# Tencent/FeatherCNN

Hardware: AMD Instinct MI355X
Metric: images/sec fp32 forward @224x224 (higher is better)
Workload: dtype f32; 1 GPU; vgg16 whole net (40 layers in the model file, 20 after fusion level 3), batch 32 per GPU, 224x224x3, fp32, synthetic ...; net=vgg16, mode=net, per_gpu_batch=32, global_batch=32, parallelism=batch-shard x1, launch=hipGraph replay per step, conv_routing=fhip_conv_select_algo_tuned

## Files before the change

__graft_entry__.py:

```python
from __future__ import annotations

import os
import subprocess
import sys

ROOT = os.path.dirname(os.path.abspath(__file__))
if ROOT not in sys.path:
    sys.path.insert(0, ROOT)


def build() -> None:
    jobs = str(min(8, os.cpu_count() or 1))
    subprocess.run(["make", "-s", "-j", jobs, "-C", os.path.join(ROOT, "feathercnn_amd", "csrc")], check=True)
    subprocess.run(["make", "-s", "-C", os.path.join(ROOT, "oracle"), "port"], check=True)
    subprocess.run(["make", "-s", "-C", os.path.join(ROOT, "oracle"), "ref"], check=True)
    import feathercnn_amd
    feathercnn_amd.load_library()
    from feathercnn_amd import _lib
    _lib.load_gconv_library()
    _lib.load_deconv_library()
    _lib.load_inorm_library()
    _lib.load_shuffle_library()
    from feathercnn_amd import provenance
    provenance.write_stamp()


def smoke() -> None:
    import numpy as np
    import torch

    import oracle
    from feathercnn_amd import ConvLayer, ConvParam
    from oracle import conv_geom, nerr, synth

    if not torch.cuda.is_available():
        raise RuntimeError("smoke() needs a GPU")
    if not os.path.exists(os.path.join(ROOT, "feathercnn_amd", "libfeather_hip.so")):
        build()
    dev = torch.device("cuda:0")
    chk = oracle.best()
    cases = [("winograd_f63", conv_geom(16, 32, 20, 3, 1, 1)), ("im2col_1x1", conv_geom(32, 24, 14, 1, 1, 0)),
             ("im2col_7x7s2", conv_geom(3, 16, 32, 7, 2, 3)), ("depthwise_s1", conv_geom(16, 16, 28, 3, 1, 1, group=16)),
             ("depthwise_s2", conv_geom(16, 16, 28, 3, 2, 1, group=16)), ("depthwise_flat_14px", conv_geom(24, 24, 14, 3, 1, 1, group=24)),
             ("depthwise_flat_7px", conv_geom(40, 40, 7, 3, 1, 1, group=40)), ("depthwise_band_56px", conv_geom(8, 8, 56, 3, 1, 1, group=8)),
             ("depthwise_flat_20px_s2", conv_geom(12, 12, 20, 3, 2, 1, group=12)), ("depthwise_flat_5px", conv_geom(44, 44, 5, 3, 1, 1, group=44))]
    for name, g in cases:
        x, w, b = synth(g, 2)
        p = ConvParam(output_channels=g.oc, input_channels=g.ic, input_h=g.ih, input_w=g.iw, kernel_h=g.kh, kernel_w=g.kw,
                      stride_h=g.sh, stride_w=g.sw, pad_left=g.pl, pad_right=g.pr, pad_top=g.pt, pad_bottom=g.pb,
                      group=g.group, bias_term=True, activation=1, batch=2)
        layer = ConvLayer(p, torch.from_numpy(w).to(dev), torch.from_numpy(b).to(dev))
        y = layer.Forward(torch.from_numpy(x).to(dev))
        torch.cuda.synchronize()
        e = nerr(y.cpu().numpy(), chk.forward(g, x, w, b))
        print(f"smoke {name}: algo={layer.booster.algo} normalised error vs {type(chk).__name__} = {e:.2e}")
        if not (e <= 1e-4) or not np.isfinite(e):
            raise AssertionError(f"smoke {name}: parity failed ({e})")
    from feathercnn_amd.booster import WINOGRADF63, forward_chained
    g1, g2 = conv_geom(16, 24, 28, 3, 1, 1), conv_geom(24, 8, 28, 3, 1, 1)
    (x, w1, b1), (_, w2, b2) = synth(g1, 2, seed=3), synth(g2, 2, seed=4)
    run = []
    for g, w, b in ((g1, w1, b1), (g2, w2, b2)):
        p = ConvParam(output_channels=g.oc, input_channels=g.ic, input_h=g.ih, input_w=g.iw, kernel_h=3, kernel_w=3, stride_h=1, stride_w=1,
                      pad_left=1, pad_right=1, pad_top=1, pad_bottom=1, group=1, bias_term=True, activation=1, batch=2)
        run.append(ConvLayer(p, torch.from_numpy(w).to(dev), torch.from_numpy(b).to(dev), algo=WINOGRADF63))
    y = forward_chained(run, torch.from_numpy(x).to(dev))
    torch.cuda.synchronize()
    e = nerr(y.cpu().numpy(), chk.forward(g2, chk.forward(g1, x, w1, b1), w2, b2))
    print(f"smoke chained winograd pair: normalised error = {e:.2e}")
    if not (e <= 1e-4):
        raise AssertionError(f"smoke chained pair: parity failed ({e})")
    g0, g1 = conv_geom(3, 16, 28, 3, 1, 1), conv_geom(16, 8, 28, 3, 1, 1)
    (x, w0, b0), (_, w1, b1) = synth(g0, 2, seed=6), synth(g1, 2, seed=7)
    p0 = ConvParam(output_channels=16, input_channels=3, input_h=28, input_w=28, kernel_h=3, kernel_w=3, stride_h=1, stride_w=1, pad_left=1,
                   pad_right=1, pad_top=1, pad_bottom=1, group=1, bias_term=True, activation=1, batch=2)
    p0.AssignOutputDim()
    p1 = ConvParam(output_channels=8, input_channels=16, input_h=28, input_w=28, kernel_h=3, kernel_w=3, stride_h=1, stride_w=1, pad_left=1,
                   pad_right=1, pad_top=1, pad_bottom=1, group=1, bias_term=True, activation=1, batch=2)
    l1 = ConvLayer(p1, torch.from_numpy(w1).to(dev), torch.from_numpy(b1).to(dev), algo=WINOGRADF63)
    y = forward_chained([l1], torch.from_numpy(x).to(dev), first=(p0, torch.from_numpy(w0).to(dev), torch.from_numpy(b0).to(dev)))
    torch.cuda.synchronize()
    e = nerr(y.cpu().numpy(), chk.forward(g1, chk.forward(g0, x, w0, b0), w1, b1))
    print(f"smoke first layer inside the Winograd input transform: normalised error = {e:.2e}")
    if not (e <= 1e-4):
        raise AssertionError(f"smoke first-layer fusion: parity failed ({e})")
    from feathercnn_amd import model_zoo
    from feathercnn_amd.net import Net
    from oracle import netcheck
    p, b, i, o = model_zoo.tiny_allsorts()
    x = np.random.default_rng(5).uniform(-1, 1, (2, 3, 20, 20)).astype(np.float32)
    want = (netcheck.RefNet(p, b) if netcheck.have_ref_net() else netcheck.PortNet(p, b)).run(i, x, o)
    for level in (1, 3):
        net = Net(fusion=level, tuned=(level == 3), graph=(level == 3))
        net.LoadParam(p)
        net.LoadWeights(b)
        net.FeedInput(i, x)
        net.Forward()
        e = nerr(net.Extract(o), want)
        print(f"smoke tiny net, fusion level {level} ({len(net.layers())} layers after fusion): normalised error = {e:.2e}")
        if not (e <= 1e-4):
            raise AssertionError(f"smoke net: parity failed ({e})")
    sys.path.insert(0, os.path.join(ROOT, "tests"))
    import gconv_ref
    p, b, i, o = model_zoo.tiny_grouped()
    x = np.random.default_rng(6).uniform(-1, 1, (2, 3, 21, 21)).astype(np.float32)
    net = Net(fusion=2)
    net.LoadParam(p)
    net.LoadWeights(b)
    net.FeedInput(i, x)
    net.Forward()
    e = gconv_ref.nerr(net.Extract(o), gconv_ref.Net(p, b).run(i, x, o))
    print(f"smoke grouped net ({sum(a == 'GCONV' for _, _, a in net.layers())} grouped layers): normalised error = {e:.2e}")
    if not (e <= 1e-4):
        raise AssertionError(f"smoke grouped net: parity failed ({e})")
    import deconv_ref
    p, b, i, o = model_zoo.tiny_deconv()
    x = np.random.default_rng(7).uniform(-1, 1, (2, 3, 16, 16)).astype(np.float32)
    net = Net(fusion=2)
    net.LoadParam(p)
    net.LoadWeights(b)
    net.FeedInput(i, x)
    net.Forward()
    e = deconv_ref.nerr(net.Extract(o), deconv_ref.Net(p, b).run(i, x, o))
    print(f"smoke tiny_deconv ({sum(a == 'DECONV' for _, _, a in net.layers())} deconvolution layers): normalised error = {e:.2e}")
    if not (e <= 1e-4):
        raise AssertionError(f"smoke tiny_deconv: parity failed ({e})")
    import inorm_ref
    p, b, i, o = model_zoo.tiny_generative()
    x = np.random.default_rng(8).uniform(-1, 1, (2, 3, 24, 24)).astype(np.float32)
    net = Net(fusion=2)
    net.LoadParam(p)
    net.LoadWeights(b)
    net.FeedInput(i, x)
    net.Forward()
    e = inorm_ref.nerr(net.Extract(o), inorm_ref.Net(p, b).run(i, x, o))
    print(f"smoke tiny_generative ({sum(a == 'INORM' for _, _, a in net.layers())} InstanceNorm layers): normalised error = {e:.2e}")
    if not (e <= 1e-4):
        raise AssertionError(f"smoke tiny_generative: parity failed ({e})")
    import shuffle_ref
    p, b, i, o = model_zoo.tiny_shuffle()
    x = np.random.default_rng(9).uniform(-1, 1, (2, 3, 28, 28)).astype(np.float32)
    net = Net(fusion=2)
    net.LoadParam(p)
    net.LoadWeights(b)
    net.FeedInput(i, x)
    net.Forward()
    e = shuffle_ref.nerr(net.Extract(o), shuffle_ref.Net(p, b).run(i, x, o))
    print(f"smoke tiny_shuffle ({sum(a == 'SHUFFLE' for _, _, a in net.layers())} channel-map launches): normalised error = {e:.2e}")
    if not (e <= 1e-4):
        raise AssertionError(f"smoke tiny_shuffle: parity failed ({e})")
    print("smoke OK")


if __name__ == "__main__":
    build()
    if len(sys.argv) > 1 and sys.argv[1] == "smoke":
        smoke()
```

feathercnn_amd/_lib.py:

```python
from __future__ import annotations

import ctypes
import os

_HERE = os.path.dirname(os.path.abspath(__file__))
_LIB = None
_PIXOUT = None
_GCONV = None
_DECONV = None
_INORM = None
_SHUFFLE = None

STAGE_NAMES = ("wino_input", "wino_gemm", "wino_output", "igemm", "depthwise", "init", "wino_chain")


class fhip_conv_param(ctypes.Structure):
    _fields_ = [(n, ctypes.c_int) for n in (
        "output_channels", "input_channels", "input_h", "input_w", "kernel_h", "kernel_w", "output_h", "output_w",
        "stride_h", "stride_w", "pad_left", "pad_bottom", "pad_right", "pad_top", "group", "bias_term", "activation")]


class fhip_winograd_plan(ctypes.Structure):
    _fields_ = [("tiles_x", ctypes.c_int), ("tiles_y", ctypes.c_int), ("tiles_per_image", ctypes.c_int),
                ("columns", ctypes.c_int), ("columns_padded", ctypes.c_int), ("column_block", ctypes.c_int), ("frequency_points", ctypes.c_int), ("tile_outputs", ctypes.c_int),
                ("in_channels_padded", ctypes.c_int),
                ("out_channels_padded", ctypes.c_int), ("v_offset_bytes", ctypes.c_size_t), ("v_bytes", ctypes.c_size_t),
                ("m_offset_bytes", ctypes.c_size_t), ("m_bytes", ctypes.c_size_t), ("u_bytes", ctypes.c_size_t)]


class fhip_pool_param(ctypes.Structure):
    _fields_ = [(n, ctypes.c_int) for n in (
        "channels", "input_h", "input_w", "kernel_h", "kernel_w", "stride_h", "stride_w", "pad_left", "pad_right",
        "pad_top", "pad_bottom", "pooling_type", "global_pooling")]


class fhip_pixel_image(ctypes.Structure):
    _fields_ = [("data", ctypes.c_void_p)] + [(n, ctypes.c_int) for n in ("w", "h", "stride", "roi_x", "roi_y", "roi_w", "roi_h")]


_P = ctypes.POINTER(fhip_conv_param)
_Q = ctypes.POINTER(fhip_pool_param)
_PI = ctypes.POINTER(ctypes.c_int)
_SZ = ctypes.c_size_t
_V = ctypes.c_void_p
_I = ctypes.c_int

SIGNATURES = {
    "fhip_conv_assign_output_dim": (_I, [_P]),
    "fhip_conv_flops": (ctypes.c_double, [_P]),
    "fhip_conv_select_algo": (_I, [_P, ctypes.POINTER(_I)]),
    "fhip_conv_select_algo_tuned": (_I, [_P, ctypes.POINTER(_I)]),
    "fhip_conv_get_buffer_size": (_I, [_P, _I, _I, ctypes.POINTER(ctypes.c_size_t), ctypes.POINTER(ctypes.c_size_t)]),
    "fhip_conv_init": (_I, [_P, _I, _V, _V, _V]),
    "fhip_conv_forward": (_I, [_P, _I, _I, _V, _V, _V, _V, _V, _V]),
    "fhip_winograd_f63_plan": (_I, [_P, _I, ctypes.POINTER(fhip_winograd_plan)]),
    "fhip_winograd_f63_transform_kernel": (_I, [_P, _V, _V, _V]),
    "fhip_winograd_f63_input_transform": (_I, [_P, _I, _V, _V, _V]),
    "fhip_winograd_f63_tile_gemm": (_I, [_P, _I, _V, _V, _V, _V]),
    "fhip_winograd_f63_output_transform": (_I, [_P, _I, _V, _V, _V, _V]),
    "fhip_stage_timing_enable": (_I, [_I]),
    "fhip_stage_timing_collect": (_I, [ctypes.POINTER(ctypes.c_double), ctypes.POINTER(ctypes.c_longlong)]),
    "fhip_last_error": (ctypes.c_char_p, []),
    "fhip_version": (ctypes.c_char_p, []),
    "fhip_device_info": (_I, [ctypes.c_char_p, _I, ctypes.POINTER(_I), ctypes.POINTER(_I)]),
    "fhip_conv_streams_1x1": (_I, [_P, _I, _I]),
    "fhip_calibrate_mfma_f32": (_I, [ctypes.POINTER(ctypes.c_double), ctypes.POINTER(ctypes.c_double), _V]),
    "fhip_relu": (_I, [_V, _V, _SZ, _V]),
    "fhip_add": (_I, [_V, _V, _V, _SZ, _I, _V]),
    "fhip_affine": (_I, [_V, _V, _V, _V, _I, _I, _I, _I, _V]),
    "fhip_conv_can_fuse_residual": (_I, [_P, _I]),
    "fhip_conv_forward_residual": (_I, [_P, _I, _I, _V, _V, _V, _V, _V, _V, _V]),
    "fhip_conv_can_fuse_dw_pw": (_I, [_P, _P, _I]),
    "fhip_conv_forward_dw_pw": (_I, [_P, _P, _I, _V, _V, _V, _V, _V, _V, _V]),
    "fhip_conv_can_chain_winograd": (_I, [_P, _I, _P, _I, _I]),
    "fhip_conv_forward_chained": (_I, [_P, _I, _V, _V, _V, _V, _V, _V, _P, _V, _I, _V]),
    "fhip_winograd_f63_output_to_next_input": (_I, [_P, _P, _I, _V, _V, _V, _I, _V]),
    "fhip_conv_can_fuse_siblings": (_I, [_P, _I, _P, _I, _I]),
    "fhip_conv_siblings_geometry": (_I, [_P, _P, _P]),
    "fhip_conv_forward_siblings": (_I, [_P, _P, _I, _V, _V, _V, _V, _V, _V]),
    "fhip_conv_can_fuse_first_winograd": (_I, [_P, _P, _I, _I]),
    "fhip_winograd_f63_input_from_first": (_I, [_P, _P, _I, _V, _V, _V, _V, _V]),
    "fhip_conv_can_fuse_maxpool2": (_I, [_P, _I]),
    "fhip_conv_forward_maxpool2": (_I, [_P, _I, _I, _V, _V, _V, _V, _V, _V]),
    "fhip_pixels_to_float": (_I, [_V, _V, _I, _I, _I, _I, _I, _I, _V, _V, _V]),
    "fhip_yuv420sp_to_float": (_I, [_V, _V, _I, _I, _I, _I, _I, _I, _I, _V, _V, _V]),
    "fhip_pixel_images_plan": (_I, [_V, _I, _I, _I, _I, _V, ctypes.POINTER(_SZ)]),
    "fhip_pixels_to_float_images": (_I, [_V, _V, _V, _V, _V, _V]),
    "fhip_pooling_output_dim": (_I, [_Q, _PI, _PI]),
    "fhip_pooling": (_I, [_Q, _I, _V, _V, _V]),
    "fhip_softmax": (_I, [_V, _V, _I, _I, _V]),
    "fhip_net_create": (_I, [ctypes.POINTER(_V)]),
    "fhip_net_destroy": (_I, [_V]),
    "fhip_net_set_stream": (_I, [_V, _V]),
    "fhip_net_get_stream": (_I, [_V, ctypes.POINTER(_V)]),
    "fhip_net_set_fusion": (_I, [_V, _I]),
    "fhip_net_set_graph": (_I, [_V, _I]),
    "fhip_net_set_tuned_selection": (_I, [_V, _I]),
    "fhip_net_set_concurrency": (_I, [_V, _I]),
    "fhip_net_set_sub_batches": (_I, [_V, _I]),
    "fhip_net_load_param": (_I, [_V, ctypes.c_char_p]),
    "fhip_net_load_param_mem": (_I, [_V, ctypes.c_char_p, _SZ]),
    "fhip_net_load_weights": (_I, [_V, ctypes.c_char_p]),
    "fhip_net_load_weights_mem": (_I, [_V, _V, _SZ]),
    "fhip_net_load_weights_device": (_I, [_V, _V, _SZ]),
    "fhip_net_feed_input": (_I, [_V, ctypes.c_char_p, _I, _I, _I, _I, _V, _I]),
    "fhip_net_feed_pixels": (_I, [_V, ctypes.c_char_p, _I, _V, _I, _I, _I, _I, _I, _V, _V, _I]),
    "fhip_net_feed_yuv420sp": (_I, [_V, ctypes.c_char_p, _I, _V, _I, _I, _I, _I, _I, _I, _V, _V, _I]),
    "fhip_net_feed_pixel_images": (_I, [_V, ctypes.c_char_p, _I, _V, _I, _I, _I, _V, _V, _I]),
    "fhip_net_forward": (_I, [_V]),
    "fhip_net_extract": (_I, [_V, ctypes.c_char_p, ctypes.POINTER(_V), _PI, _PI, _PI, _PI]),
    "fhip_net_extract_host": (_I, [_V, ctypes.c_char_p, _V, _SZ]),
    "fhip_net_layer_count": (_I, [_V]),
    "fhip_net_layer_info": (_I, [_V, _I, ctypes.c_char_p, ctypes.c_char_p, _I, _PI]),
    "fhip_net_layer_conv_param": (_I, [_V, _I, _P, _PI]),
    "fhip_net_layer_fused_pointwise": (_I, [_V, _I, _P, _PI]),
    "fhip_net_layer_chain": (_I, [_V, _I, _PI, _PI]),
    "fhip_net_layer_sibling": (_I, [_V, _I, _PI]),
    "fhip_net_layer_residual": (_I, [_V, _I, _PI]),
    "fhip_net_forward_timed": (_I, [_V, ctypes.POINTER(ctypes.c_float)]),
    "fhip_net_memory": (_I, [_V, ctypes.POINTER(_SZ), ctypes.POINTER(_SZ), ctypes.POINTER(_SZ)]),
}

PIXOUT_SIGNATURES = {
    "fhip_pixout_channels": (_I, [_I]),
    "fhip_float_to_pixels": (_I, [_V, _SZ, _V, _I, _I, _I, _I, _I, _I, _V, _V, _V]),
    "fhip_float_to_pixels_host": (_I, [_V, _SZ, _V, _I, _I, _I, _I, _I, _I, _V, _V, _V]),
    "fhip_pixout_last_error": (ctypes.c_char_p, []),
}

GCONV_SIGNATURES = {
    "fhip_gconv_supported": (_I, [_P]),
    "fhip_gconv_get_buffer_size": (_I, [_P, _I, ctypes.POINTER(_SZ), ctypes.POINTER(_SZ)]),
    "fhip_gconv_init": (_I, [_P, _V, _V, _V]),
    "fhip_gconv_forward": (_I, [_P, _I, _V, _V, _V, _V, _V, _V]),
    "fhip_gconv_route": (_I, [_P, _V, _V, ctypes.c_char_p, _I]),
    "fhip_gconv_last_error": (ctypes.c_char_p, []),
}

class fhip_deconv_param(ctypes.Structure):
    _fields_ = [(n, ctypes.c_int) for n in ("output_channels", "input_channels", "input_h", "input_w", "kernel_h", "kernel_w", "output_h", "output_w",
                                            "stride_h", "stride_w", "pad_left", "pad_bottom", "pad_right", "pad_top", "group", "bias_term",
                                            "activation", "output_pad_right", "output_pad_bottom")]


_DP = ctypes.POINTER(fhip_deconv_param)
DECONV_SIGNATURES = {
    "fhip_deconv_assign_output_dim": (_I, [_DP]),
    "fhip_deconv_supported": (_I, [_DP]),
    "fhip_deconv_get_buffer_size": (_I, [_DP, _I, ctypes.POINTER(_SZ), ctypes.POINTER(_SZ)]),
    "fhip_deconv_init": (_I, [_DP, _V, _V, _V]),
    "fhip_deconv_forward": (_I, [_DP, _I, _V, _V, _V, _V, _V, _V]),
    "fhip_deconv_route": (_I, [_DP, ctypes.c_char_p, _I]),
    "fhip_deconv_last_error": (ctypes.c_char_p, []),
}

_FL = ctypes.c_float
INORM_SIGNATURES = {
    "fhip_instance_norm_get_buffer_size": (_I, [_I, _I, _I, _I, ctypes.POINTER(_SZ)]),
    "fhip_instance_norm_forward": (_I, [_I, _I, _I, _I, _V, _V, _V, _V, _FL, _I, _FL, _V, _V]),
    "fhip_instance_norm_forward_route": (_I, [_I, _I, _I, _I, _I, _V, _V, _V, _V, _FL, _I, _FL, _V, _V]),
    "fhip_instance_norm_route": (_I, [_I, _I, _I, _I, _V, _V, ctypes.c_char_p, _I]),
    "fhip_activation_forward": (_I, [_I, _V, _V, _I, _I, _I, _FL, _FL, _V, _V]),
    "fhip_inorm_last_error": (ctypes.c_char_p, []),
}

_PP = ctypes.POINTER(ctypes.c_void_p)
_IP = ctypes.POINTER(ctypes.c_int)
SHUFFLE_SIGNATURES = {
    "fhip_channel_map_supported": (_I, [_I, _I, _I, _I]),
    "fhip_channel_slice_resolve": (_I, [_I, _IP, _I, _IP]),
    "fhip_channel_shuffle_forward": (_I, [_V, _V, _I, _I, _I, _I, _I, _I, _V]),
    "fhip_channel_slice_forward": (_I, [_PP, _V, _I, _I, _I, _I, _IP, _I, _V]),
    "fhip_channel_map_create": (_I, [_PP, _IP, _I, _IP, _I, _IP]),
    "fhip_channel_map_destroy": (_I, [_V]),
    "fhip_channel_map_forward": (_I, [_V, _PP, _PP, _I, _I, _I, _V]),
    "fhip_channel_map_forward_route": (_I, [_I, _V, _PP, _PP, _I, _I, _I, _V]),
    "fhip_channel_map_route": (_I, [_I, _I, _I, _PP, _I, ctypes.c_char_p, _I]),
    "fhip_shuffle_last_error": (ctypes.c_char_p, []),
}


def lib_path() -> str:
    return os.environ.get("FEATHER_HIP_LIB", os.path.join(_HERE, "libfeather_hip.so"))


def load_library():
    global _LIB
    if _LIB is None:
        import torch
        path = lib_path()
        if not os.path.exists(path):
            raise RuntimeError(f"feathercnn_amd: HIP library {path} is missing -- run `python -c 'import __graft_entry__ as g; "
                               "g.build()'` (or `make -C feathercnn_amd/csrc`). There is no CPU fallback.")
        lib = ctypes.CDLL(path)
        for name, (res, args) in SIGNATURES.items():
            fn = getattr(lib, name)
            fn.restype = res
            fn.argtypes = args
        _LIB = lib
    return _LIB


def pixout_path() -> str:
    return os.path.join(_HERE, "libfeather_pixout.so")


def load_pixout_library():
    global _PIXOUT
    if _PIXOUT is None:
        import torch
        path = pixout_path()
        if not os.path.exists(path):
            raise RuntimeError(f"feathercnn_amd: HIP library {path} is missing -- run `python -c 'import __graft_entry__ as g; "
                               "g.build()'` (or `make -C feathercnn_amd/csrc`). There is no CPU fallback.")
        lib = ctypes.CDLL(path)
        for name, (res, args) in PIXOUT_SIGNATURES.items():
            fn = getattr(lib, name)
            fn.restype = res
            fn.argtypes = args
        _PIXOUT = lib
    return _PIXOUT


def gconv_path() -> str:
    return os.path.join(_HERE, "libfeather_gconv.so")


def load_gconv_library():
    global _GCONV
    if _GCONV is None:
        import torch
        path = gconv_path()
        if not os.path.exists(path):
            raise RuntimeError(f"feathercnn_amd: HIP library {path} is missing -- run `python -c 'import __graft_entry__ as g; "
                               "g.build()'` (or `make -C feathercnn_amd/csrc`). There is no CPU fallback.")
        lib = ctypes.CDLL(path)
        for name, (res, args) in GCONV_SIGNATURES.items():
            fn = getattr(lib, name)
            fn.restype = res
            fn.argtypes = args
        _GCONV = lib
    return _GCONV


def deconv_path() -> str:
    return os.path.join(_HERE, "libfeather_deconv.so")


def load_deconv_library():
    global _DECONV
    if _DECONV is None:
        import torch
        path = deconv_path()
        if not os.path.exists(path):
            raise RuntimeError(f"feathercnn_amd: HIP library {path} is missing -- run `python -c 'import __graft_entry__ as g; "
                               "g.build()'` (or `make -C feathercnn_amd/csrc`). There is no CPU fallback.")
        lib = ctypes.CDLL(path)
        for name, (res, args) in DECONV_SIGNATURES.items():
            fn = getattr(lib, name)
            fn.restype = res
            fn.argtypes = args
        _DECONV = lib
    return _DECONV


def inorm_path() -> str:
    return os.path.join(_HERE, "libfeather_inorm.so")


def load_inorm_library():
    global _INORM
    if _INORM is None:
        import torch
        path = inorm_path()
        if not os.path.exists(path):
            raise RuntimeError(f"feathercnn_amd: HIP library {path} is missing -- run `python -c 'import __graft_entry__ as g; "
                               "g.build()'` (or `make -C feathercnn_amd/csrc`). There is no CPU fallback.")
        lib = ctypes.CDLL(path)
        for name, (res, args) in INORM_SIGNATURES.items():
            fn = getattr(lib, name)
            fn.restype = res
            fn.argtypes = args
        _INORM = lib
    return _INORM


def shuffle_path() -> str:
    return os.path.join(_HERE, "libfeather_shuffle.so")


def load_shuffle_library():
    global _SHUFFLE
    if _SHUFFLE is None:
        import torch
        path = shuffle_path()
        if not os.path.exists(path):
            raise RuntimeError(f"feathercnn_amd: HIP library {path} is missing -- run `python -c 'import __graft_entry__ as g; "
                               "g.build()'` (or `make -C feathercnn_amd/csrc`). There is no CPU fallback.")
        lib = ctypes.CDLL(path)
        for name, (res, args) in SHUFFLE_SIGNATURES.items():
            fn = getattr(lib, name)
            fn.restype = res
            fn.argtypes = args
        _SHUFFLE = lib
    return _SHUFFLE
```

feathercnn_amd/csrc/capi.hip:

```cpp
#include <string.h>
#include <stdlib.h>

#include <algorithm>
#include <mutex>
#include <string>
#include <vector>

#include "common.h"
#include "feather_hip/feather_net.h"

namespace fhip
{
int winograd_plan(const fhip_conv_param& p, int batch, fhip_winograd_plan* plan);
int winograd_transform_kernel(const fhip_conv_param& p, float* u, const float* kernel, hipStream_t s);
int winograd_input_transform(const fhip_conv_param& p, int batch, float* v, const float* input, hipStream_t s);
int winograd_tile_gemm(const fhip_conv_param& p, int batch, float* m, const float* u, const float* v, hipStream_t s);
int winograd_output_transform(const fhip_conv_param& p, int batch, float* output, const float* m, const float* bias,
                              hipStream_t s, int pool = 0);
bool winograd_can_pool(const fhip_conv_param& p);
bool winograd_can_chain(const fhip_conv_param& p, const fhip_conv_param& next, int pool);
bool winograd_can_fuse_first(const fhip_conv_param& first, const fhip_conv_param& next, int batch);
fhip_conv_param igemm_twin_geometry(const fhip_conv_param& a, const fhip_conv_param& b);
bool igemm_twin_applicable(const fhip_conv_param& a, const fhip_conv_param& b, int batch);
int igemm_twin_forward(const fhip_conv_param& a, const fhip_conv_param& b, int batch, float* out_a, float* out_b, const float* in, const float* packed,
// ... 168 lines not shown
{
    if (!valid_param(p) || !buffer_bytes || !packed_bytes || batch < 1) return fail(FHIP_E_BADARG, "bad argument");
    switch (algo)
    {
        case FHIP_NAIVE:
        case FHIP_IM2COL:
        {
            if (p->group > 1) return fail(FHIP_E_UNSUPPORTED, "implicit GEMM handles group == 1 only");
            *buffer_bytes = igemm_buffer_bytes(*p, batch);
            *packed_bytes = igemm_packed_floats(*p) * sizeof(float);
            return FHIP_OK;
        }
        case FHIP_DEPTHWISE:
            *buffer_bytes = 0;
            *packed_bytes = depthwise_packed_floats(*p, nullptr) * sizeof(float);
            return FHIP_OK;
        case FHIP_WINOGRADF63:
        {
            fhip_winograd_plan pl;
            int rc = winograd_plan(*p, batch, &pl);
            if (rc) return rc;
            *buffer_bytes = pl.v_bytes + pl.m_bytes;
            *packed_bytes = pl.u_bytes;
            return FHIP_OK;
        }
        default: return fail(FHIP_E_UNSUPPORTED, "This algo is not supported on gfx950 (nor on AVX2, avx/booster.cpp:348-354)");
    }
}

int fhip_conv_init(const fhip_conv_param* p, int algo, float* packed, const float* kernel, void* stream)
{
    if (!valid_param(p) || !packed || !kernel) return fail(FHIP_E_BADARG, "bad argument");
    hipStream_t s = (hipStream_t)stream;
    switch (algo)
    {
        case FHIP_NAIVE:
        case FHIP_IM2COL: return igemm_init(*p, packed, kernel, s);
        case FHIP_DEPTHWISE: return depthwise_init(*p, packed, kernel, s);
        case FHIP_WINOGRADF63: return winograd_transform_kernel(*p, packed, kernel, s);
        default: return fail(FHIP_E_UNSUPPORTED, "This algo is not supported on gfx950");
    }
}

static int conv_forward_impl(const fhip_conv_param* p, int algo, int batch, float* output, const float* input, const float* packed,
                             float* buffer, const float* bias, void* stream, int pool, const float* residual = nullptr)
{
    if (!valid_param(p) || !output || !input || !packed || batch < 1) return fail(FHIP_E_BADARG, "bad argument");
    hipStream_t s = (hipStream_t)stream;
    if (pool && (algo != FHIP_WINOGRADF63 || !winograd_can_pool(*p)))
        return fail(FHIP_E_UNSUPPORTED, "fused max pooling is available on the Winograd route with even output dims only");
    if (residual && algo != FHIP_IM2COL) return fail(FHIP_E_UNSUPPORTED, "the fused residual add is available on the IM2COL route only");
    switch (algo)
    {
        case FHIP_NAIVE: return igemm_forward(*p, batch, output, input, packed, bias, buffer, true, s);
        case FHIP_IM2COL: return igemm_forward(*p, batch, output, input, packed, bias, buffer, false, s, residual);
        case FHIP_DEPTHWISE: return depthwise_forward(*p, batch, output, input, packed, bias, s);
        case FHIP_WINOGRADF63:
        {
            if (!buffer) return fail(FHIP_E_BADARG, "Winograd needs the scratch buffer");
            fhip_winograd_plan pl;
            int rc = winograd_plan(*p, batch, &pl);
            if (rc) return rc;
            float* v = reinterpret_cast<float*>(reinterpret_cast<char*>(buffer) + pl.v_offset_bytes);
            float* m = reinterpret_cast<float*>(reinterpret_cast<char*>(buffer) + pl.m_offset_bytes);
            if ((rc = winograd_input_transform(*p, batch, v, input, s))) return rc;
            if ((rc = winograd_tile_gemm(*p, batch, m, packed, v, s))) return rc;
            return winograd_output_transform(*p, batch, output, m, bias, s, pool);
        }
        default: return fail(FHIP_E_UNSUPPORTED, "This algo is not supported on gfx950");
    }
}

int fhip_conv_forward(const fhip_conv_param* p, int algo, int batch, float* output, const float* input, const float* packed,
                      float* buffer, const float* bias, void* stream)
{
    return conv_forward_impl(p, algo, batch, output, input, packed, buffer, bias, stream, 0);
}

int fhip_conv_forward_maxpool2(const fhip_conv_param* p, int algo, int batch, float* pooled_output, const float* input, const float* packed,
                               float* buffer, const float* bias, void* stream)
{
    return conv_forward_impl(p, algo, batch, pooled_output, input, packed, buffer, bias, stream, 1);
}

int fhip_conv_forward_residual(const fhip_conv_param* p, int algo, int batch, float* output, const float* input, const float* packed,
                               float* buffer, const float* bias, const float* residual, void* stream)
{
    if (!residual) return fail(FHIP_E_BADARG, "null residual");
    return conv_forward_impl(p, algo, batch, output, input, packed, buffer, bias, stream, 0, residual);
}

int fhip_conv_streams_1x1(const fhip_conv_param* p, int algo, int batch)
{
    return valid_param(p) && (algo == FHIP_IM2COL || algo == FHIP_NAIVE) && batch >= 1 && igemm_streams(*p, batch) ? 1 : 0;
}

int fhip_conv_can_fuse_residual(const fhip_conv_param* p, int algo) { return valid_param(p) && algo == FHIP_IM2COL ? 1 : 0; }

int fhip_conv_can_fuse_maxpool2(const fhip_conv_param* p, int algo)
{
    return valid_param(p) && algo == FHIP_WINOGRADF63 && winograd_can_pool(*p) ? 1 : 0;
}

int fhip_conv_can_fuse_dw_pw(const fhip_conv_param* dw, const fhip_conv_param* pw, int batch)
{
    return valid_param(dw) && valid_param(pw) && dwpw_applicable(*dw, *pw, batch) ? 1 : 0;
}

int fhip_conv_forward_dw_pw(const fhip_conv_param* dw, const fhip_conv_param* pw, int batch, float* output, const float* input,
                            const float* dw_packed, const float* dw_bias, const float* pw_packed, const float* pw_bias, void* stream)
{
    if (!valid_param(dw) || !valid_param(pw) || !output || !input || !dw_packed || !pw_packed || batch < 1) return fail(FHIP_E_BADARG, "bad argument");
    return dwpw_forward(*dw, *pw, batch, output, input, dw_packed, dw_bias, pw_packed, pw_bias, (hipStream_t)stream);
}

int fhip_conv_can_fuse_siblings(const fhip_conv_param* a, int algo_a, const fhip_conv_param* b, int algo_b, int batch)
{
    return valid_param(a) && valid_param(b) && algo_a == FHIP_IM2COL && algo_b == FHIP_IM2COL && igemm_twin_applicable(*a, *b, batch) ? 1 : 0;
}

int fhip_conv_siblings_geometry(const fhip_conv_param* a, const fhip_conv_param* b, fhip_conv_param* both)
{
    if (!valid_param(a) || !valid_param(b) || !both) return fail(FHIP_E_BADARG, "bad argument");
    *both = igemm_twin_geometry(*a, *b);
    return FHIP_OK;
}

int fhip_conv_forward_siblings(const fhip_conv_param* a, const fhip_conv_param* b, int batch, float* output_a, float* output_b, const float* input,
                               const float* packed_both, const float* bias_both, void* stream)
{
    if (!valid_param(a) || !valid_param(b) || !output_a || !output_b || !input || !packed_both || batch < 1) return fail(FHIP_E_BADARG, "bad argument");
    return igemm_twin_forward(*a, *b, batch, output_a, output_b, input, packed_both, bias_both, (hipStream_t)stream);
}

int fhip_conv_can_chain_winograd(const fhip_conv_param* p, int algo, const fhip_conv_param* next, int next_algo, int pool)
{
    return valid_param(p) && valid_param(next) && algo == FHIP_WINOGRADF63 && next_algo == FHIP_WINOGRADF63 && winograd_can_chain(*p, *next, pool) ? 1 : 0;
}

int fhip_conv_forward_chained(const fhip_conv_param* p, int batch, float* output, const float* input, const float* packed, float* v, float* m,
                              const float* bias, const fhip_conv_param* next, float* v_next, int pool, void* stream)
{
    if (!valid_param(p) || !packed || !v || !m || batch < 1) return fail(FHIP_E_BADARG, "bad argument");
    if (next ? (!valid_param(next) || !v_next) : !output) return fail(FHIP_E_BADARG, "a chained layer needs `next` and `v_next`, the last one `output`");
    hipStream_t s = (hipStream_t)stream;
    int rc;
    if (input && (rc = winograd_input_transform(*p, batch, v, input, s))) return rc;
    if ((rc = winograd_tile_gemm(*p, batch, m, packed, v, s))) return rc;
    if (next) return winograd_output_to_next_input(*p, *next, batch, v_next, m, bias, s, pool);
    if (pool && !winograd_can_pool(*p)) return fail(FHIP_E_UNSUPPORTED, "fused max pooling needs even output dims");
    return winograd_output_transform(*p, batch, output, m, bias, s, pool);
}

int fhip_winograd_f63_output_to_next_input(const fhip_conv_param* p, const fhip_conv_param* next, int batch, float* v_next, const float* m,
                                           const float* bias, int pool, void* stream)
{
    if (!valid_param(p) || !valid_param(next) || !v_next || !m || batch < 1) return fail(FHIP_E_BADARG, "bad argument");
    return winograd_output_to_next_input(*p, *next, batch, v_next, m, bias, (hipStream_t)stream, pool);
}

int fhip_conv_can_fuse_first_winograd(const fhip_conv_param* first, const fhip_conv_param* next, int next_algo, int batch)
{
    return valid_param(first) && valid_param(next) && next_algo == FHIP_WINOGRADF63 && winograd_can_fuse_first(*first, *next, batch) ? 1 : 0;
}

int fhip_winograd_f63_input_from_first(const fhip_conv_param* first, const fhip_conv_param* next, int batch, float* v_next, const float* input,
                                       const float* first_kernel, const float* first_bias, void* stream)
{
    if (!valid_param(first) || !valid_param(next) || !v_next || !input || !first_kernel || batch < 1) return fail(FHIP_E_BADARG, "bad argument");
    return winograd_input_from_first(*first, *next, batch, v_next, input, first_kernel, first_bias, (hipStream_t)stream);
}

int fhip_winograd_f63_transform_kernel(const fhip_conv_param* p, float* u, const float* kernel, void* stream)
{
    if (!valid_param(p) || !u || !kernel) return fail(FHIP_E_BADARG, "bad argument");
    return winograd_transform_kernel(*p, u, kernel, (hipStream_t)stream);
}

int fhip_winograd_f63_input_transform(const fhip_conv_param* p, int batch, float* v, const float* input, void* stream)
{
    if (!valid_param(p) || !v || !input) return fail(FHIP_E_BADARG, "bad argument");
    return winograd_input_transform(*p, batch, v, input, (hipStream_t)stream);
}

int fhip_winograd_f63_tile_gemm(const fhip_conv_param* p, int batch, float* m, const float* u, const float* v, void* stream)
{
    if (!valid_param(p) || !m || !u || !v) return fail(FHIP_E_BADARG, "bad argument");
    return winograd_tile_gemm(*p, batch, m, u, v, (hipStream_t)stream);
}

int fhip_winograd_f63_output_transform(const fhip_conv_param* p, int batch, float* output, const float* m, const float* bias,
                                       void* stream)
{
    if (!valid_param(p) || !output || !m) return fail(FHIP_E_BADARG, "bad argument");
    return winograd_output_transform(*p, batch, output, m, bias, (hipStream_t)stream);
}

int fhip_stage_timing_enable(int on)
{
    std::lock_guard<std::mutex> lk(g_tm_mu);
    g_tm_on = on != 0;
    return FHIP_OK;
}

int fhip_stage_timing_collect(double* ms, long long* launches)
{
    if (!ms || !launches) return fail(FHIP_E_BADARG, "null argument");
    std::lock_guard<std::mutex> lk(g_tm_mu);
    for (int i = 0; i < FHIP_STAGE_COUNT; ++i)
    {
        ms[i] = 0.0;
        launches[i] = 0;
    }
    int rc = FHIP_OK;
    for (auto& t : g_tm_pending)
    {
        float dt = 0.f;
        hipError_t e = hipEventSynchronize(t.b);
        if (e == hipSuccess) e = hipEventElapsedTime(&dt, t.a, t.b);
        if (e != hipSuccess)
            rc = fail_hip(e, "stage timing");
        else if (t.stage >= 0 && t.stage < FHIP_STAGE_COUNT)
        {
            ms[t.stage] += dt;
            launches[t.stage] += 1;
        }
        g_tm_pool.emplace_back(t.a, t.b);
    }
    g_tm_pending.clear();
    return rc;
}

const char* fhip_last_error(void) { return g_last_error.c_str(); }

const char* fhip_version(void) { return "feather_hip 0.1 (gfx950)"; }

int fhip_device_info(char* name, int name_len, int* cus, int* lds_bytes)
{
    int n = 0;
    if (hipGetDeviceCount(&n) != hipSuccess || n < 1) return fail(FHIP_E_NODEVICE, "no HIP device");
    int dev = 0;
    FHIP_CHECK_HIP(hipGetDevice(&dev));
    hipDeviceProp_t prop;
    FHIP_CHECK_HIP(hipGetDeviceProperties(&prop, dev));
    if (name && name_len > 0)
    {
        snprintf(name, name_len, "%s (%s)", prop.name, prop.gcnArchName);
    }
    if (cus) *cus = prop.multiProcessorCount;
    if (lds_bytes) *lds_bytes = (int)prop.maxSharedMemoryPerMultiProcessor;
    return FHIP_OK;
}

namespace
{
typedef float cal_f32x16 __attribute__((ext_vector_type(16)));
__device__ unsigned long long g_cal_ticks[2];

__global__ __launch_bounds__(256) void mfma_calibration_kernel(float* sink, const float* noise, int steps)
{
    const long long c0 = clock64(), w0 = wall_clock64();
    cal_f32x16 acc[4];
#pragma unroll
    for (int t = 0; t < 4; ++t)
#pragma unroll
        for (int r = 0; r < 16; ++r) acc[t][r] = 0.f;
    float a[8], b[8];
#pragma unroll
    for (int u = 0; u < 8; ++u)
    {
        a[u] = noise[(threadIdx.x * 16 + u + blockIdx.x) & 4095];
        b[u] = noise[(threadIdx.x * 16 + 8 + u + 3 * blockIdx.x) & 4095];
    }
    for (int s = 0; s < steps; ++s)
    {
#pragma unroll
        for (int u = 0; u < 8; ++u)
        {
            acc[0] = __builtin_amdgcn_mfma_f32_32x32x2f32(a[u], b[u], acc[0], 0, 0, 0);
            acc[1] = __builtin_amdgcn_mfma_f32_32x32x2f32(a[(u + 3) & 7], b[(u + 5) & 7], acc[1], 0, 0, 0);
            acc[2] = __builtin_amdgcn_mfma_f32_32x32x2f32(a[(u + 1) & 7], b[(u + 2) & 7], acc[2], 0, 0, 0);
            acc[3] = __builtin_amdgcn_mfma_f32_32x32x2f32(a[(u + 6) & 7], b[(u + 7) & 7], acc[3], 0, 0, 0);
        }
#pragma unroll
        for (int u = 0; u < 8; ++u) asm volatile("" : "+v"(a[u]), "+v"(b[u]));
    }
    float sum = 0.f;
#pragma unroll
    for (int t = 0; t < 4; ++t)
#pragma unroll
        for (int r = 0; r < 16; ++r) sum += acc[t][r];
    if (sum == 123.456f) sink[0] = sum;
    if (threadIdx.x == 0 && (blockIdx.x & 15) == 0)
    {
        atomicAdd(&g_cal_ticks[0], (unsigned long long)(clock64() - c0));
        atomicAdd(&g_cal_ticks[1], (unsigned long long)(wall_clock64() - w0));
    }
}
}

static int calibrate_mfma_f32_run(float* sink, float* noise, hipEvent_t e0, hipEvent_t e1, int blocks, int steps, hipStream_t s, double* tflops,
                                  double* shader_mhz)
{
    {
        std::vector<float> h(4096);
        unsigned x = 2463534242u;
// ... 61 lines not shown
```

feathercnn_amd/csrc/net.hip:

```cpp
#include <ctype.h>
#include <dlfcn.h>
#include <float.h>
#include <math.h>
#include <stdarg.h>
#include <stdio.h>
#include <string.h>

#include <algorithm>
#include <map>
#include <memory>
#include <mutex>
#include <string>
#include <vector>

#include "common.h"
#include "feather_hip/feather_deconv.h"
#include "feather_hip/feather_gconv.h"
#include "feather_hip/feather_inorm.h"
#include "feather_hip/feather_net.h"
#include "feather_hip/feather_shuffle.h"

namespace fhip
{
namespace net
{

static int failf(int code, const char* fmt, ...)
{
    char buf[512];
    va_list ap;
    va_start(ap, fmt);
    vsnprintf(buf, sizeof(buf), fmt, ap);
    va_end(ap);
    return fail(code, buf);
}

enum
{
    NET_E_IO = -1,
    NET_E_SHAPE = -100,
    NET_E_UNKNOWN_LAYER = -200,
    NET_E_TOPOLOGY = -300,
    NET_E_BASE_RESHAPE = -400
};

struct GconvApi
{
    decltype(&fhip_gconv_supported) supported = nullptr;
    decltype(&fhip_gconv_get_buffer_size) get_buffer_size = nullptr;
    decltype(&fhip_gconv_init) init = nullptr;
    decltype(&fhip_gconv_forward) forward = nullptr;
    decltype(&fhip_gconv_last_error) last_error = nullptr;
};

static const GconvApi* gconv_api()
{
    static std::mutex mu;
    static GconvApi api;
    static bool loaded = false;
    std::lock_guard<std::mutex> lk(mu);
    if (loaded) return &api;
    std::string tried;
    void* h = nullptr;
    Dl_info self;
    if (dladdr((void*)&gconv_api, &self) && self.dli_fname)
    {
        std::string path = self.dli_fname;
        const size_t slash = path.rfind('/');
        path = (slash == std::string::npos ? std::string() : path.substr(0, slash + 1)) + "libfeather_gconv.so";
        h = dlopen(path.c_str(), RTLD_NOW | RTLD_LOCAL);
        tried = path;
    }
    if (!h) h = dlopen("libfeather_gconv.so", RTLD_NOW | RTLD_LOCAL);
    if (!h)
    {
        failf(FHIP_E_UNSUPPORTED, "a convolution with 1 < group < input_channels needs libfeather_gconv.so next to libfeather_hip.so (%s): %s",
              tried.c_str(), dlerror());
        return nullptr;
    }
    GconvApi a;
    a.supported = (decltype(a.supported))dlsym(h, "fhip_gconv_supported");
    a.get_buffer_size = (decltype(a.get_buffer_size))dlsym(h, "fhip_gconv_get_buffer_size");
    a.init = (decltype(a.init))dlsym(h, "fhip_gconv_init");
    a.forward = (decltype(a.forward))dlsym(h, "fhip_gconv_forward");
    a.last_error = (decltype(a.last_error))dlsym(h, "fhip_gconv_last_error");
    if (!a.supported || !a.get_buffer_size || !a.init || !a.forward || !a.last_error)
    {
        failf(FHIP_E_UNSUPPORTED, "libfeather_gconv.so (%s) does not export the entry points of feather_gconv.h", tried.c_str());
        dlclose(h);
        return nullptr;
    }
    api = a;
    loaded = true;
    return &api;
}

struct DeconvApi
{
    decltype(&fhip_deconv_assign_output_dim) assign_output_dim = nullptr;
    decltype(&fhip_deconv_supported) supported = nullptr;
    decltype(&fhip_deconv_get_buffer_size) get_buffer_size = nullptr;
    decltype(&fhip_deconv_init) init = nullptr;
    decltype(&fhip_deconv_forward) forward = nullptr;
    decltype(&fhip_deconv_last_error) last_error = nullptr;
};

static const DeconvApi* deconv_api()
{
    static std::mutex mu;
    static DeconvApi api;
    static bool loaded = false;
    std::lock_guard<std::mutex> lk(mu);
    if (loaded) return &api;
    std::string tried;
    void* h = nullptr;
    Dl_info self;
    if (dladdr((void*)&deconv_api, &self) && self.dli_fname)
    {
        std::string path = self.dli_fname;
        const size_t slash = path.rfind('/');
        path = (slash == std::string::npos ? std::string() : path.substr(0, slash + 1)) + "libfeather_deconv.so";
        h = dlopen(path.c_str(), RTLD_NOW | RTLD_LOCAL);
        tried = path;
    }
    if (!h) h = dlopen("libfeather_deconv.so", RTLD_NOW | RTLD_LOCAL);
    if (!h)
    {
        failf(FHIP_E_UNSUPPORTED, "a Deconvolution layer needs libfeather_deconv.so next to libfeather_hip.so (%s): %s", tried.c_str(), dlerror());
        return nullptr;
    }
    DeconvApi a;
    a.assign_output_dim = (decltype(a.assign_output_dim))dlsym(h, "fhip_deconv_assign_output_dim");
    a.supported = (decltype(a.supported))dlsym(h, "fhip_deconv_supported");
    a.get_buffer_size = (decltype(a.get_buffer_size))dlsym(h, "fhip_deconv_get_buffer_size");
    a.init = (decltype(a.init))dlsym(h, "fhip_deconv_init");
    a.forward = (decltype(a.forward))dlsym(h, "fhip_deconv_forward");
    a.last_error = (decltype(a.last_error))dlsym(h, "fhip_deconv_last_error");
    if (!a.assign_output_dim || !a.supported || !a.get_buffer_size || !a.init || !a.forward || !a.last_error)
    {
        failf(FHIP_E_UNSUPPORTED, "libfeather_deconv.so (%s) does not export the entry points of feather_deconv.h", tried.c_str());
        dlclose(h);
        return nullptr;
    }
    api = a;
    loaded = true;
    return &api;
}

struct InormApi
{
    decltype(&fhip_instance_norm_get_buffer_size) get_buffer_size = nullptr;
    decltype(&fhip_instance_norm_forward) forward = nullptr;
    decltype(&fhip_activation_forward) activation = nullptr;
    decltype(&fhip_inorm_last_error) last_error = nullptr;
};

static const InormApi* inorm_api()
{
    static std::mutex mu;
    static InormApi api;
    static bool loaded = false;
    std::lock_guard<std::mutex> lk(mu);
    if (loaded) return &api;
    std::string tried;
    void* h = nullptr;
    Dl_info self;
    if (dladdr((void*)&inorm_api, &self) && self.dli_fname)
    {
        std::string path = self.dli_fname;
        const size_t slash = path.rfind('/');
        path = (slash == std::string::npos ? std::string() : path.substr(0, slash + 1)) + "libfeather_inorm.so";
        h = dlopen(path.c_str(), RTLD_NOW | RTLD_LOCAL);
        tried = path;
    }
    if (!h) h = dlopen("libfeather_inorm.so", RTLD_NOW | RTLD_LOCAL);
    if (!h)
    {
        failf(FHIP_E_UNSUPPORTED, "an InstanceNorm / activation layer needs libfeather_inorm.so next to libfeather_hip.so (%s): %s", tried.c_str(), dlerror());
        return nullptr;
    }
    InormApi a;
    a.get_buffer_size = (decltype(a.get_buffer_size))dlsym(h, "fhip_instance_norm_get_buffer_size");
    a.forward = (decltype(a.forward))dlsym(h, "fhip_instance_norm_forward");
    a.activation = (decltype(a.activation))dlsym(h, "fhip_activation_forward");
    a.last_error = (decltype(a.last_error))dlsym(h, "fhip_inorm_last_error");
    if (!a.get_buffer_size || !a.forward || !a.activation || !a.last_error)
    {
        failf(FHIP_E_UNSUPPORTED, "libfeather_inorm.so (%s) does not export the entry points of feather_inorm.h", tried.c_str());
        dlclose(h);
        return nullptr;
    }
    api = a;
    loaded = true;
    return &api;
}

struct ShuffleApi
{
    decltype(&fhip_channel_slice_resolve) resolve = nullptr;
    decltype(&fhip_channel_map_create) create = nullptr;
    decltype(&fhip_channel_map_destroy) destroy = nullptr;
    decltype(&fhip_channel_map_forward) forward = nullptr;
    decltype(&fhip_shuffle_last_error) last_error = nullptr;
};

static const ShuffleApi* shuffle_api()
{
    static std::mutex mu;
    static ShuffleApi api;
    static bool loaded = false;
    std::lock_guard<std::mutex> lk(mu);
    if (loaded) return &api;
    std::string tried;
    void* h = nullptr;
    Dl_info self;
    if (dladdr((void*)&shuffle_api, &self) && self.dli_fname)
    {
        std::string path = self.dli_fname;
        const size_t slash = path.rfind('/');
        path = (slash == std::string::npos ? std::string() : path.substr(0, slash + 1)) + "libfeather_shuffle.so";
        h = dlopen(path.c_str(), RTLD_NOW | RTLD_LOCAL);
        tried = path;
    }
    if (!h) h = dlopen("libfeather_shuffle.so", RTLD_NOW | RTLD_LOCAL);
    if (!h)
    {
        failf(FHIP_E_UNSUPPORTED, "a ShuffleChannel / Slice layer needs libfeather_shuffle.so next to libfeather_hip.so (%s): %s", tried.c_str(), dlerror());
        return nullptr;
    }
    ShuffleApi a;
    a.resolve = (decltype(a.resolve))dlsym(h, "fhip_channel_slice_resolve");
    a.create = (decltype(a.create))dlsym(h, "fhip_channel_map_create");
    a.destroy = (decltype(a.destroy))dlsym(h, "fhip_channel_map_destroy");
    a.forward = (decltype(a.forward))dlsym(h, "fhip_channel_map_forward");
    a.last_error = (decltype(a.last_error))dlsym(h, "fhip_shuffle_last_error");
    if (!a.resolve || !a.create || !a.destroy || !a.forward || !a.last_error)
    {
        failf(FHIP_E_UNSUPPORTED, "libfeather_shuffle.so (%s) does not export the entry points of feather_shuffle.h", tried.c_str());
        dlclose(h);
        return nullptr;
    }
    api = a;
    loaded = true;
    return &api;
}

struct ParamDict
{
    static const int kMax = 32;
    struct Entry
    {
        bool loaded = false;
        uint32_t bits = 0;
        std::vector<float> array;
    } e[kMax];

    void clear()
    {
        for (auto& x : e) x = Entry();
    }
    int get(int id, int def) const
    {
        if (id < 0 || id >= kMax || !e[id].loaded) return def;
        int v;
        memcpy(&v, &e[id].bits, 4);
        return v;
    }
    float get(int id, float def) const
    {
        if (id < 0 || id >= kMax || !e[id].loaded) return def;
        float v;
        memcpy(&v, &e[id].bits, 4);
        return v;
    }
    bool has_array(int id) const { return id >= 0 && id < kMax && e[id].loaded && !e[id].array.empty(); }

    static bool is_float(const std::string& s)
    {
        for (char ch : s)
            if (ch == '.' || ch == 'e' || ch == 'E') return true;
        return false;
    }
    static bool looks_like_pair(const std::string& tok)
    {
        size_t i = 0;
        if (i < tok.size() && tok[i] == '-') ++i;
        const size_t d0 = i;
        while (i < tok.size() && isdigit((unsigned char)tok[i])) ++i;
        return i > d0 && i < tok.size() && tok[i] == '=';
    }
    int parse(const std::string& tok)
    {
        const size_t eq = tok.find('=');
        int id = atoi(tok.substr(0, eq).c_str());
        const std::string val = tok.substr(eq + 1);
        const bool is_array = id <= -23300;
        if (is_array) id = -id - 23300;
        if (id < 0 || id >= kMax) return failf(FHIP_E_BADARG, "param id %d out of range", id);
        if (is_array)
        {
            std::vector<std::string> parts;
            size_t a = 0;
            while (a <= val.size())
            {
                const size_t b = val.find(',', a);
                parts.push_back(val.substr(a, b == std::string::npos ? std::string::npos : b - a));
                if (b == std::string::npos) break;
                a = b + 1;
            }
            const int len = atoi(parts[0].c_str());
            if (len < 0 || (int)parts.size() != len + 1) return failf(FHIP_E_BADARG, "ParamDict read array element fail");
            e[id].array.resize(len);
            for (int j = 0; j < len; ++j) e[id].array[j] = (float)atof(parts[j + 1].c_str());
        }
        else
        {
            if (val.empty()) return failf(FHIP_E_BADARG, "ParamDict read value fail");
            if (is_float(val))
            {
                const float f = (float)atof(val.c_str());
                memcpy(&e[id].bits, &f, 4);
            }
            else
            {
                const int i = atoi(val.c_str());
                memcpy(&e[id].bits, &i, 4);
            }
        }
        e[id].loaded = true;
        return 0;
    }
};

struct ModelBin
{
    const unsigned char* p;
    const unsigned char* end;

    static float half_to_float(uint16_t h)
    {
        const uint32_t sign = (uint32_t)(h >> 15) << 31;
        int exp = (h >> 10) & 0x1f;
        uint32_t man = h & 0x3ff;
        uint32_t bits;
        if (exp == 0)
        {
            if (man == 0)
                bits = sign;
            else
            {
                exp = 1;
                while (!(man & 0x400))
                {
                    man <<= 1;
                    --exp;
                }
                man &= 0x3ff;
                bits = sign | ((uint32_t)(exp + 112) << 23) | (man << 13);
            }
        }
        else if (exp == 31)
            bits = sign | 0x7f800000u | (man << 13);
        else
            bits = sign | ((uint32_t)(exp + 112) << 23) | (man << 13);
        float f;
        memcpy(&f, &bits, 4);
        return f;
    }
    bool take(void* dst, size_t bytes)
    {
        if ((size_t)(end - p) < bytes) return false;
        if (dst) memcpy(dst, p, bytes);
        p += bytes;
        return true;
    }
    int load(size_t w, int type, std::vector<float>& out)
    {
        out.assign(w, 0.f);
        if (type == 1)
        {
            if (!take(out.data(), w * 4)) return failf(NET_E_SHAPE, "ModelBin read weight_data failed (file too short)");
            return 0;
        }
        if (type != 0) return failf(NET_E_SHAPE, "ModelBin load type %d not implemented", type);
        unsigned char f[4];
        if (!take(f, 4)) return failf(NET_E_SHAPE, "ModelBin read flag_struct failed");
        uint32_t tag;
        memcpy(&tag, f, 4);
        const unsigned flag = f[0] + f[1] + f[2] + f[3];
        if (tag == 0x01306B47u)
        {
            const size_t bytes = (w * 2 + 3) / 4 * 4;
            if ((size_t)(end - p) < bytes) return failf(NET_E_SHAPE, "ModelBin read float16_weights failed");
            for (size_t i = 0; i < w; ++i)
            {
                uint16_t h;
                memcpy(&h, p + 2 * i, 2);
                out[i] = half_to_float(h);
            }
            p += bytes;
            return 0;
        }
        if (tag == 0x000D4B38u) return failf(FHIP_E_UNSUPPORTED, "int8 weights are not supported (conv_layer.h:50-55 rejects them too)");
        if (tag == 0x0002C056u)
        {
            if (!take(out.data(), w * 4)) return failf(NET_E_SHAPE, "ModelBin read weight_data failed");
            return 0;
        }
        if (flag != 0)
        {
            float table[256];
            if (!take(table, sizeof(table))) return failf(NET_E_SHAPE, "ModelBin read quantization_value failed");
            const size_t bytes = (w + 3) / 4 * 4;
            if ((size_t)(end - p) < bytes) return failf(NET_E_SHAPE, "ModelBin read index_array failed");
            for (size_t i = 0; i < w; ++i) out[i] = table[p[i]];
            p += bytes;
            return 0;
        }
        if (!take(out.data(), w * 4)) return failf(NET_E_SHAPE, "ModelBin read weight_data failed (file too short)");
        return 0;
    }
};

struct Blob
{
    std::string name;
    int n = 0, c = 0, h = 0, w = 0;
    float* data = nullptr;
    size_t capacity = 0;
    Blob* alias = nullptr;
    bool fused_away = false;
    bool chained = false;

    size_t count() const { return (size_t)n * c * h * w; }
    int reshape(int n_, int c_, int h_, int w_)
    {
        n = n_;
        c = c_;
        h = h_;
        w = w_;
        alias = nullptr;
        if (chained && !data) return 0;
        if (count() > capacity)
        {
            if (data && capacity) (void)hipFree(data);
            data = nullptr;
            capacity = 0;
            FHIP_CHECK_HIP(hipMalloc((void**)&data, count() * sizeof(float)));
            capacity = count();
        }
        return 0;
    }
    void drop_storage()
    {
        if (data && capacity) (void)hipFree(data);
        data = nullptr;
        capacity = 0;
    }
    void share(Blob* src)
    {
        n = src->n;
        c = src->c;
        h = src->h;
        w = src->w;
        if (data && capacity) (void)hipFree(data);
        capacity = 0;
        alias = src;
        data = src->data;
    }
    ~Blob()
    {
        if (data && capacity) (void)hipFree(data);
    }
};

struct DeviceVec
{
    float* d = nullptr;
    size_t bytes = 0;
    int upload(const float* h, size_t count, hipStream_t s)
    {
        if (bytes != count * 4)
        {
            release();
            FHIP_CHECK_HIP(hipMalloc((void**)&d, std::max<size_t>(count, 1) * 4));
            bytes = count * 4;
        }
        if (count) FHIP_CHECK_HIP(hipMemcpyAsync(d, h, count * 4, hipMemcpyHostToDevice, s));
        return 0;
    }
    int resize(size_t nbytes)
    {
        if (bytes != nbytes)
        {
            release();
            FHIP_CHECK_HIP(hipMalloc((void**)&d, std::max<size_t>(nbytes, 4)));
            bytes = nbytes;
        }
        return 0;
    }
    void release()
    {
        if (d) (void)hipFree(d);
        d = nullptr;
        bytes = 0;
    }
    ~DeviceVec() { release(); }
};

struct Net;

struct Layer
{
    std::string type, name;
    std::vector<Blob*> bottoms, tops;
    Net* net = nullptr;

    virtual ~Layer() {}
    virtual int LoadParam(const ParamDict&) { return 0; }
    virtual int LoadWeights(ModelBin&) { return 0; }
    virtual int Reshape()
    {
        if (tops.size() != 1 || bottoms.size() != 1) return failf(NET_E_BASE_RESHAPE, "layer %s: base Reshape needs 1 bottom and 1 top", name.c_str());
        return tops[0]->reshape(bottoms[0]->n, bottoms[0]->c, bottoms[0]->h, bottoms[0]->w);
    }
    virtual int Init(hipStream_t) { return 0; }
    virtual int Forward(hipStream_t) = 0;
    virtual int Fuse(Layer*, int ) { return 0; }
    virtual size_t weight_bytes() const { return 0; }
    virtual size_t arena_bytes() const { return 0; }
    virtual int algo() const { return -1; }
    virtual const fhip_conv_param* conv_param() const { return nullptr; }
    virtual const fhip_conv_param* fused_pointwise(int*) const { return nullptr; }
    virtual void chain_state(int* v_from_previous, int* writes_next_v) const { *v_from_previous = *writes_next_v = 0; }
    virtual int sibling_state() const { return 0; }
    virtual int residual_state() const { return 0; }
};

static bool is_plain_relu(const Layer* l);

struct Net
{
    std::vector<std::unique_ptr<Layer>> layers;
    std::map<std::string, std::unique_ptr<Blob>> blobs;
    std::vector<std::unique_ptr<Blob>> shadowed;
    hipStream_t stream = nullptr;
    int fusion = 1;
    bool use_graph = false;
    bool tuned_selection = false;
    bool param_loaded = false, weights_loaded = false, fused = false, initialized = false, shapes_dirty = true;
    DeviceVec arena;
    size_t chain_slot[2] = {0, 0}, chain_m = 0;
    hipGraphExec_t graph_exec = nullptr;
    hipStream_t owned_stream = nullptr;
    bool concurrency = false;
    hipStream_t side_stream = nullptr;
    std::vector<hipEvent_t> events;
    std::vector<int> side;
    std::vector<std::vector<int>> waits;

    ~Net()
    {
        drop_graph();
        for (hipEvent_t e : events) (void)hipEventDestroy(e);
        if (side_stream) (void)hipStreamDestroy(side_stream);
        if (owned_stream) (void)hipStreamDestroy(owned_stream);
    }
    void drop_graph()
    {
        if (graph_exec) (void)hipGraphExecDestroy(graph_exec);
        graph_exec = nullptr;
    }
    Blob* find(const std::string& n)
    {
        auto it = blobs.find(n);
        return it == blobs.end() ? nullptr : it->second.get();
    }
};

struct InputLayer : Layer
{
    int Reshape() override { return 0; }
    int Forward(hipStream_t) override { return 0; }
};

struct ConvLayer : Layer
{
    fhip_conv_param p;
    int algo_ = -1, inited_algo = -2;
    bool gconv = false;
    std::vector<float> w_host, b_host;
    std::vector<float> post_mul, post_add;
    DeviceVec packed, bias;
    size_t buffer_bytes = 0, packed_bytes = 0;
    bool fuse_pool = false, pool_fast = false;
    fhip_pool_param poolq;
    DeviceVec pre_pool;
    Blob* residual = nullptr;
    bool res_fast = false;
    std::unique_ptr<ConvLayer> pw;
    bool pair_fast = false;
    DeviceVec mid;
    ConvLayer* chain_next = nullptr;
    bool chain_in = false;
    int chain_pos = 0;
    size_t chain_bytes = 0;
    ConvLayer* head_of = nullptr;
    ConvLayer* head = nullptr;
    DeviceVec first_raw;
    ConvLayer* sib = nullptr;
    ConvLayer* sib_of = nullptr;
    ConvLayer* sib_packed_for = nullptr;
    DeviceVec sib_packed, sib_bias;
    bool sib_has_bias = false;
    bool first_candidate() const
    {
        return p.kernel_h == 3 && p.kernel_w == 3 && p.stride_h == 1 && p.stride_w == 1 && p.group == 1 && p.input_channels >= 2 && p.input_channels <= 4 && p.pad_left == 1 &&
               p.pad_right == 1 && p.pad_top == 1 && p.pad_bottom == 1;
    }

    ConvLayer()
    {
        memset(&p, 0, sizeof(p));
        memset(&poolq, 0, sizeof(poolq));
    }

    int LoadParam(const ParamDict& pd) override
    {
        const int dilation_w = pd.get(2, 1), dilation_h = pd.get(12, dilation_w);
        if (dilation_w > 1 || dilation_h > 1) return failf(NET_E_UNKNOWN_LAYER, "layer %s: dilated convolution is not supported", name.c_str());
        if (pd.get(8, 0)) return failf(NET_E_UNKNOWN_LAYER, "layer %s: int8 convolution is not supported", name.c_str());
        p.kernel_w = pd.get(1, 0);
        p.kernel_h = pd.get(11, p.kernel_w);
        p.stride_w = pd.get(3, 1);
        p.stride_h = pd.get(13, p.stride_w);
        p.pad_left = pd.get(4, 0);
        p.pad_bottom = pd.get(14, p.pad_left);
        p.pad_right = pd.get(4, 0);
        p.pad_top = pd.get(14, p.pad_left);
        p.group = pd.get(7, 1);
        p.output_channels = pd.get(0, 0);
        p.bias_term = pd.get(5, 0);
        p.activation = FHIP_ACT_NONE;
        const int weight_data_size = pd.get(6, 0);
        if (p.group == 0 || p.output_channels % p.group) return failf(NET_E_SHAPE, "layer %s: output_channels is not divisible by its group", name.c_str());
        p.output_channels /= p.group;
        if (p.output_channels <= 0 || p.kernel_h <= 0 || p.kernel_w <= 0) return failf(NET_E_SHAPE, "layer %s: bad convolution geometry", name.c_str());
        p.input_channels = weight_data_size / p.output_channels / p.kernel_h / p.kernel_w;
        gconv = p.group > 1 && p.group < p.input_channels;
        if (gconv) p.output_channels *= p.group;
        return 0;
    }
    int LoadWeights(ModelBin& mb) override
    {
        const size_t wsize = (size_t)p.input_channels * p.output_channels * p.kernel_h * p.kernel_w / (gconv ? p.group : 1);
        inited_algo = -2;
        sib_packed_for = nullptr;
        int rc = mb.load(wsize, 0, w_host);
        if (rc) return rc;
        if (p.bias_term)
        {
            const int k = p.group == p.input_channels ? p.input_channels : p.output_channels;
            rc = mb.load(k, 1, b_host);
        }
        return rc;
    }
    int Reshape() override
    {
        const Blob* b = bottoms[0];
        p.input_w = b->w;
        p.input_h = b->h;
        if (p.input_channels != b->c)
            return failf(NET_E_TOPOLOGY, "convolution layer %s has %d input channels while bottom blob has %d channels", name.c_str(), p.input_channels, b->c);
        fhip_conv_assign_output_dim(&p);
        if (p.output_h < 1 || p.output_w < 1) return failf(NET_E_SHAPE, "layer %s: empty output", name.c_str());
        if (gconv)
        {
            const GconvApi* api = gconv_api();
            if (!api) return FHIP_E_UNSUPPORTED;
            if (api->supported(&p) != 1) return failf(FHIP_E_UNSUPPORTED, "layer %s: grouped convolution refused: %s", name.c_str(), api->last_error());
            algo_ = FHIP_NET_ROUTE_GCONV;
            int rc = tops[0]->reshape(b->n, p.output_channels, p.output_h, p.output_w);
            if (rc) return rc;
            if ((rc = api->get_buffer_size(&p, b->n, &buffer_bytes, &packed_bytes))) return failf(rc, "layer %s: %s", name.c_str(), api->last_error());
            return 0;
        }
        int rc = net->tuned_selection ? fhip_conv_select_algo_tuned(&p, &algo_) : fhip_conv_select_algo(&p, &algo_);
        if (rc) return rc;
        if (pw)
        {
            Blob dwout;
            dwout.n = b->n;
            dwout.c = p.output_channels;
            dwout.h = p.output_h;
            dwout.w = p.output_w;
            pw->bottoms.assign(1, &dwout);
            pw->tops = tops;
            pw->net = net;
            rc = pw->Reshape();
            pw->bottoms.clear();
            if (rc) return rc;
            pair_fast = fhip_conv_can_fuse_dw_pw(&p, &pw->p, b->n) != 0 && !pw->fuse_pool && !pw->residual && pw->algo_ == FHIP_IM2COL;
            if (!pair_fast && (rc = mid.resize((size_t)b->n * p.output_channels * p.output_h * p.output_w * sizeof(float)))) return rc;
            size_t bb = 0;
            if ((rc = fhip_conv_get_buffer_size(&p, algo_, b->n, &bb, &packed_bytes))) return rc;
            buffer_bytes = std::max(bb, pw->buffer_bytes);
            return 0;
        }
        res_fast = residual && fhip_conv_can_fuse_residual(&p, algo_) != 0;
        if (residual && (residual->n != b->n || residual->c != p.output_channels || residual->h != p.output_h || residual->w != p.output_w))
            return failf(NET_E_SHAPE, "Shape mismatch among bottoms of layer %s.", name.c_str());
        if (fuse_pool)
        {
            poolq.channels = p.output_channels;
            poolq.input_h = p.output_h;
            poolq.input_w = p.output_w;
            int ph, pw;
            if ((rc = fhip_pooling_output_dim(&poolq, &ph, &pw))) return rc;
            pool_fast = fhip_conv_can_fuse_maxpool2(&p, algo_) != 0;
            if (!pool_fast && (rc = pre_pool.resize((size_t)b->n * p.output_channels * p.output_h * p.output_w * sizeof(float)))) return rc;
            rc = tops[0]->reshape(b->n, p.output_channels, ph, pw);
        }
        else
            rc = tops[0]->reshape(b->n, p.output_channels, p.output_h, p.output_w);
        if (rc) return rc;
        return fhip_conv_get_buffer_size(&p, algo_, b->n, &buffer_bytes, &packed_bytes);
    }
    void folded(std::vector<float>& w, std::vector<float>& b) const
    {
        w = w_host;
        b = b_host;
        if (post_mul.empty()) return;
        const int K = p.output_channels;
        const size_t per = w.size() / K;
        if (b.empty()) b.assign(K, 0.f);
        for (int k = 0; k < K; ++k)
        {
            for (size_t i = 0; i < per; ++i) w[k * per + i] *= post_mul[k];
            b[k] = b[k] * post_mul[k] + post_add[k];
        }
    }
    int init_siblings(hipStream_t s)
    {
        std::vector<float> wa, ba, wb, bb;
        folded(wa, ba);
        sib->folded(wb, bb);
        fhip_conv_param pa = p, pb = sib->p, both;
        pa.bias_term = ba.empty() ? 0 : 1;
        pb.bias_term = bb.empty() ? 0 : 1;
        int rc = fhip_conv_siblings_geometry(&pa, &pb, &both);
        if (rc) return rc;
        wa.insert(wa.end(), wb.begin(), wb.end());
        sib_has_bias = both.bias_term != 0;
        if (sib_has_bias)
        {
            if (ba.empty()) ba.assign(p.output_channels, 0.f);
            if (bb.empty()) bb.assign(sib->p.output_channels, 0.f);
            ba.insert(ba.end(), bb.begin(), bb.end());
            if ((rc = sib_bias.upload(ba.data(), ba.size(), s))) return rc;
        }
        size_t bytes = 0, pk = 0;
        if ((rc = fhip_conv_get_buffer_size(&both, FHIP_IM2COL, bottoms[0]->n, &bytes, &pk))) return rc;
        DeviceVec raw;
        if ((rc = raw.upload(wa.data(), wa.size(), s))) return rc;
        if ((rc = sib_packed.resize(pk))) return rc;
        if ((rc = fhip_conv_init(&both, FHIP_IM2COL, sib_packed.d, raw.d, s))) return rc;
        FHIP_CHECK_HIP(hipStreamSynchronize(s));
        sib_packed_for = sib;
        return 0;
    }
    int Init(hipStream_t s) override
    {
        if (pw)
        {
            const int rc = pw->Init(s);
            if (rc) return rc;
        }
        if (sib && sib_packed_for != sib)
        {
            const int rc = init_siblings(s);
            if (rc) return rc;
        }
        if (inited_algo == algo_ && packed.bytes == packed_bytes) return 0;
        std::vector<float> w, b;
        folded(w, b);
        if (!post_mul.empty()) p.bias_term = 1;
        DeviceVec raw;
        int rc = raw.upload(w.data(), w.size(), s);
        if (rc) return rc;
        if (first_candidate() && (rc = first_raw.upload(w.data(), w.size(), s))) return rc;
        rc = packed.resize(packed_bytes);
        if (rc) return rc;
        if (gconv)
        {
            const GconvApi* api = gconv_api();
            if (!api) return FHIP_E_UNSUPPORTED;
            if ((rc = api->init(&p, (float*)packed.d, (const float*)raw.d, s))) return failf(rc, "layer %s: %s", name.c_str(), api->last_error());
        }
        else
            rc = fhip_conv_init(&p, algo_, packed.d, raw.d, s);
        if (rc) return rc;
        if (p.bias_term)
        {
            rc = bias.upload(b.data(), b.size(), s);
            if (rc) return rc;
        }
        FHIP_CHECK_HIP(hipStreamSynchronize(s));
        inited_algo = algo_;
        return 0;
    }
    int Forward(hipStream_t s) override
    {
        const float* b = p.bias_term ? bias.d : nullptr;
        if (gconv)
        {
            const GconvApi* api = gconv_api();
            if (!api) return FHIP_E_UNSUPPORTED;
            const int rc = api->forward(&p, bottoms[0]->n, tops[0]->data, bottoms[0]->data, (const float*)packed.d, nullptr, b, s);
            return rc ? failf(rc, "layer %s: %s", name.c_str(), api->last_error()) : 0;
        }
        if (head_of) return 0;
        if (sib_of) return 0;
        if (sib)
            return fhip_conv_forward_siblings(&p, &sib->p, bottoms[0]->n, tops[0]->data, sib->tops[0]->data, bottoms[0]->data, sib_packed.d,
                                              sib_has_bias ? sib_bias.d : nullptr, s);
        if (pw)
        {
            const float* pb = pw->p.bias_term ? pw->bias.d : nullptr;
            if (pair_fast)
                return fhip_conv_forward_dw_pw(&p, &pw->p, bottoms[0]->n, tops[0]->data, bottoms[0]->data, packed.d, b, pw->packed.d, pb, s);
            int rc = fhip_conv_forward(&p, algo_, bottoms[0]->n, mid.d, bottoms[0]->data, packed.d, (float*)net->arena.d, b, s);
            if (rc) return rc;
            Blob dwout;
            dwout.n = bottoms[0]->n;
            dwout.c = p.output_channels;
            dwout.h = p.output_h;
            dwout.w = p.output_w;
            dwout.data = mid.d;
            pw->bottoms.assign(1, &dwout);
            pw->tops = tops;
            rc = pw->Forward(s);
            pw->bottoms.clear();
            dwout.data = nullptr;
            return rc;
        }
        if (chain_in || chain_next || head)
        {
            char* base = reinterpret_cast<char*>(net->arena.d);
            float* v = reinterpret_cast<float*>(base + net->chain_slot[chain_pos & 1]);
            float* vn = reinterpret_cast<float*>(base + net->chain_slot[(chain_pos + 1) & 1]);
            float* m = reinterpret_cast<float*>(base + net->chain_m);
            const float* in = chain_in || head ? nullptr : bottoms[0]->data;
            const int n = bottoms[0]->n;
            if (head)
            {
                const int rc = fhip_winograd_f63_input_from_first(&head->p, &p, n, v, head->bottoms[0]->data, head->first_raw.d,
                                                                  head->p.bias_term ? head->bias.d : nullptr, s);
                if (rc) return rc;
            }
            if (chain_next) return fhip_conv_forward_chained(&p, n, nullptr, in, packed.d, v, m, b, &chain_next->p, vn, fuse_pool ? 1 : 0, s);
            if (!fuse_pool || pool_fast) return fhip_conv_forward_chained(&p, n, tops[0]->data, in, packed.d, v, m, b, nullptr, nullptr, fuse_pool ? 1 : 0, s);
            const int rc = fhip_conv_forward_chained(&p, n, pre_pool.d, in, packed.d, v, m, b, nullptr, nullptr, 0, s);
            if (rc) return rc;
            return fhip_pooling(&poolq, n, tops[0]->data, pre_pool.d, s);
        }
        if (residual)
        {
            if (residual->alias) residual->data = residual->alias->data;
            if (res_fast)
                return fhip_conv_forward_residual(&p, algo_, bottoms[0]->n, tops[0]->data, bottoms[0]->data, packed.d, (float*)net->arena.d, b,
                                                  residual->data, s);
            fhip_conv_param q = p;
            q.activation = FHIP_ACT_NONE;
            const int rc = fhip_conv_forward(&q, algo_, bottoms[0]->n, tops[0]->data, bottoms[0]->data, packed.d, (float*)net->arena.d, b, s);
            if (rc) return rc;
            return fhip_add(tops[0]->data, tops[0]->data, residual->data, tops[0]->count(), p.activation == FHIP_ACT_RELU, s);
        }
        if (!fuse_pool) return fhip_conv_forward(&p, algo_, bottoms[0]->n, tops[0]->data, bottoms[0]->data, packed.d, (float*)net->arena.d, b, s);
        if (pool_fast)
            return fhip_conv_forward_maxpool2(&p, algo_, bottoms[0]->n, tops[0]->data, bottoms[0]->data, packed.d, (float*)net->arena.d, b, s);
        const int rc = fhip_conv_forward(&p, algo_, bottoms[0]->n, pre_pool.d, bottoms[0]->data, packed.d, (float*)net->arena.d, b, s);
        if (rc) return rc;
        return fhip_pooling(&poolq, bottoms[0]->n, tops[0]->data, pre_pool.d, s);
    }
    int Fuse(Layer* next, int level) override;
    bool FuseResidual(Blob* other)
    {
        if (pw)
        {
            if (fuse_pool || residual || !pw->FuseResidual(other)) return false;
            pw->bottoms.pop_back();
            bottoms.push_back(other);
            return true;
        }
        if (gconv || fuse_pool || residual || p.activation != FHIP_ACT_NONE) return false;
        residual = other;
        bottoms.push_back(other);
        return true;
    }
    size_t weight_bytes() const override
    {
        return packed.bytes + bias.bytes + pre_pool.bytes + mid.bytes + first_raw.bytes + sib_packed.bytes + sib_bias.bytes + (pw ? pw->weight_bytes() : 0);
    }
    const fhip_conv_param* fused_pointwise(int* one_kernel) const override
    {
        if (one_kernel) *one_kernel = pair_fast ? 1 : 0;
        return pw ? &pw->p : nullptr;
    }
    size_t arena_bytes() const override { return std::max(buffer_bytes, chain_bytes); }
    const fhip_conv_param* conv_param() const override { return &p; }
    int algo() const override { return gconv ? FHIP_NET_ROUTE_GCONV : algo_; }
    int sibling_state() const override { return sib ? 1 : sib_of ? 2 : 0; }
    int residual_state() const override { return !residual ? 0 : res_fast ? 1 : 2; }
    void chain_state(int* v_from_previous, int* writes_next_v) const override
    {
        *v_from_previous = head ? 2 : chain_in ? 1 : 0;
        *writes_next_v = head_of ? 2 : chain_next ? 1 : 0;
    }
};

struct InnerProductLayer : Layer
{
    fhip_conv_param p;
    size_t input_size = 0, output_size = 0, weight_data_size = 0;
    std::vector<float> w_host, b_host;
    DeviceVec packed, bias;
    size_t buffer_bytes = 0, packed_bytes = 0;
    bool inited = false;

    InnerProductLayer() { memset(&p, 0, sizeof(p)); }
    int LoadParam(const ParamDict& pd) override
    {
        output_size = pd.get(0, 0);
        p.bias_term = pd.get(1, 0);
        weight_data_size = pd.get(2, 0);
        if (output_size == 0) return failf(NET_E_SHAPE, "layer %s: num_output is 0", name.c_str());
        input_size = weight_data_size / output_size;
        p.input_channels = (int)input_size;
        p.output_channels = (int)output_size;
        p.input_h = p.input_w = p.kernel_h = p.kernel_w = p.stride_h = p.stride_w = p.group = 1;
        fhip_conv_assign_output_dim(&p);
        return 0;
    }
    int LoadWeights(ModelBin& mb) override
    {
        int rc = mb.load(weight_data_size, 0, w_host);
        if (rc) return rc;
        if (p.bias_term) rc = mb.load(output_size, 1, b_host);
        return rc;
    }
    int Reshape() override
    {
        const Blob* b = bottoms[0];
        const size_t per_image = (size_t)b->c * b->h * b->w;
        if (input_size != per_image)
            return failf(NET_E_SHAPE, "In Layer %s: Bottom %s data size %zu is inconsistant with expected input size %zu.", name.c_str(), b->name.c_str(), per_image, input_size);
        int rc = tops[0]->reshape(b->n, (int)output_size, 1, 1);
        if (rc) return rc;
        return fhip_conv_get_buffer_size(&p, FHIP_IM2COL, b->n, &buffer_bytes, &packed_bytes);
    }
    int Init(hipStream_t s) override
    {
        if (inited) return 0;
        DeviceVec raw;
        int rc = raw.upload(w_host.data(), w_host.size(), s);
        if (rc) return rc;
        rc = packed.resize(packed_bytes);
        if (rc) return rc;
        rc = fhip_conv_init(&p, FHIP_IM2COL, packed.d, raw.d, s);
        if (rc) return rc;
        if (p.bias_term)
        {
            rc = bias.upload(b_host.data(), b_host.size(), s);
            if (rc) return rc;
        }
        FHIP_CHECK_HIP(hipStreamSynchronize(s));
        std::vector<float>().swap(w_host);
        inited = true;
        return 0;
    }
    int Forward(hipStream_t s) override
    {
        return fhip_conv_forward(&p, FHIP_IM2COL, bottoms[0]->n, tops[0]->data, bottoms[0]->data, packed.d, (float*)net->arena.d,
                                 p.bias_term ? bias.d : nullptr, s);
    }
    int Fuse(Layer* next, int) override
    {
        if (is_plain_relu(next))
        {
            p.activation = FHIP_ACT_RELU;
            return 1;
        }
        return 0;
    }
    size_t weight_bytes() const override { return packed.bytes + bias.bytes; }
    size_t arena_bytes() const override { return buffer_bytes; }
    int algo() const override { return FHIP_IM2COL; }
};

struct ReluLayer : Layer
{
    float slope = 0.f;
    int LoadParam(const ParamDict& pd) override
    {
        slope = pd.get(0, 0.f);
        return 0;
    }
    int Reshape() override
    {
        if (slope != 0.f && !inorm_api()) return FHIP_E_UNSUPPORTED;
        return Layer::Reshape();
    }
    int Forward(hipStream_t s) override
    {
        if (slope == 0.f) return fhip_relu(tops[0]->data, bottoms[0]->data, bottoms[0]->count(), s);
        const InormApi* api = inorm_api();
        if (!api) return FHIP_E_UNSUPPORTED;
        const Blob* b = bottoms[0];
        const int rc = api->activation(FHIP_ACTIVATION_LEAKY_RELU, tops[0]->data, b->data, b->n, b->c, b->h * b->w, slope, 0.f, nullptr, s);
        return rc ? failf(rc, "layer %s: %s", name.c_str(), api->last_error()) : 0;
    }
};

static bool is_plain_relu(const Layer* l) { return l->type == "ReLU" && static_cast<const ReluLayer*>(l)->slope == 0.f; }

struct InstanceNormLayer : Layer
{
    int channels = 0, affine = 1, act = FHIP_INORM_ACT_NONE;
    float eps = 0.001f, slope = 0.f;
    std::vector<float> gamma, beta;
    DeviceVec d_gamma, d_beta;
    size_t scratch_bytes = 0;
    bool inited = false;

    int LoadParam(const ParamDict& pd) override
    {
        channels = pd.get(0, 0);
        eps = pd.get(1, 0.001f);
        affine = pd.get(2, 1);
        if (channels < 1) return failf(NET_E_SHAPE, "layer %s: InstanceNorm needs at least one channel", name.c_str());
        if (!(eps >= 0.f)) return failf(NET_E_SHAPE, "layer %s: InstanceNorm eps must not be negative", name.c_str());
        return 0;
    }
    int LoadWeights(ModelBin& mb) override
    {
        inited = false;
        if (!affine) return 0;
        const int rc = mb.load(channels, 1, gamma);
        return rc ? rc : mb.load(channels, 1, beta);
    }
    int Reshape() override
    {
        const Blob* b = bottoms[0];
        if (b->c != channels)
            return failf(NET_E_TOPOLOGY, "InstanceNorm layer %s has %d channels while bottom blob %s has %d", name.c_str(), channels, b->name.c_str(), b->c);
        const InormApi* api = inorm_api();
        if (!api) return FHIP_E_UNSUPPORTED;
        int rc = api->get_buffer_size(b->n, b->c, b->h, b->w, &scratch_bytes);
        if (rc) return failf(rc, "layer %s: %s", name.c_str(), api->last_error());
        return Layer::Reshape();
    }
    int Init(hipStream_t s) override
    {
        if (inited || !affine) return 0;
        int rc = d_gamma.upload(gamma.data(), gamma.size(), s);
        if (rc) return rc;
        if ((rc = d_beta.upload(beta.data(), beta.size(), s))) return rc;
        FHIP_CHECK_HIP(hipStreamSynchronize(s));
        inited = true;
        return 0;
    }
// ... 849 lines not shown
            if (!next(tn)) return failf(NET_E_IO, "param file truncated in layer %s", name.c_str());
            std::unique_ptr<Blob> blob(new Blob);
            blob->name = tn;
            layer->tops.push_back(blob.get());
            auto& slot = net.blobs[tn];
            if (slot) net.shadowed.push_back(std::move(slot));
            slot = std::move(blob);
        }
        pd.clear();
        while (t < tok.size() && ParamDict::looks_like_pair(tok[t]))
        {
            const int rc = pd.parse(tok[t++]);
            if (rc) return rc;
        }
        const int rc = layer->LoadParam(pd);
        if (rc) return rc;
        net.layers.push_back(std::move(layer));
    }
    net.param_loaded = true;
    return 0;
}

static int load_weights_mem(Net& net, const void* data, size_t len)
{
    if (net.initialized) return failf(NET_E_IO, "Net is already initialized. Are you repeatedly loading models?");
    if (net.layers.empty()) return failf(NET_E_IO, "Network has not been loaded. Please load the param file first.");
    ModelBin mb{(const unsigned char*)data, (const unsigned char*)data + len};
    for (auto& l : net.layers)
    {
        const int rc = l->LoadWeights(mb);
        if (rc)
        {
            const std::string why = fhip_last_error();
            return failf(NET_E_IO, "Layer %s loading weights failed: %s", l->name.c_str(), why.c_str());
        }
    }
    net.weights_loaded = true;
    return 0;
}

static int read_file(const char* path, std::vector<char>& out)
{
    FILE* fp = fopen(path, "rb");
    if (!fp) return failf(NET_E_IO, "Cannot open file, path: %s", path);
    fseek(fp, 0, SEEK_END);
    const long sz = ftell(fp);
    fseek(fp, 0, SEEK_SET);
    out.resize(sz > 0 ? (size_t)sz : 0);
    const size_t got = out.empty() ? 0 : fread(out.data(), 1, out.size(), fp);
    fclose(fp);
    if (got != out.size()) return failf(NET_E_IO, "short read on %s", path);
    return 0;
}

static void fuse_layers(Net& net)
{
    if (net.fused) return;
    net.fused = true;
    if (net.fusion <= 0) return;
    if (net.fusion >= 2) collapse_channel_maps(net);
    for (size_t i = 0; i < net.layers.size(); ++i)
    {
        for (;;)
        {
            Layer* cur = net.layers[i].get();
            if (cur->tops.size() != 1) break;
            Blob* top = cur->tops[0];
            size_t consumer = 0;
            int uses = 0;
            for (size_t j = i + 1; j < net.layers.size(); ++j)
                for (Blob* b : net.layers[j]->bottoms)
                    if (b == top)
                    {
                        ++uses;
                        consumer = j;
                    }
            if (uses != 1) break;
            Layer* nx = net.layers[consumer].get();
            if (net.fusion >= 2 && nx->type == "Eltwise" && nx->bottoms.size() == 2 && nx->tops.size() == 1 && nx->bottoms[0] != nx->bottoms[1] &&
                (cur->type == "Convolution" || cur->type == "ConvolutionDepthWise"))
            {
                Blob* other = nx->bottoms[0] == top ? nx->bottoms[1] : nx->bottoms[0];
                bool earlier = false;
                for (size_t j = 0; j < i; ++j)
                    for (Blob* t : net.layers[j]->tops) earlier = earlier || t == other;
                if (!earlier || !static_cast<ConvLayer*>(cur)->FuseResidual(other)) break;
                top->fused_away = true;
                cur->tops[0] = nx->tops[0];
                net.layers.erase(net.layers.begin() + consumer);
                continue;
            }
            if (nx->bottoms.size() != 1 || nx->tops.size() != 1) break;
            const int fr = cur->Fuse(nx, net.fusion);
            if (fr != 1 && fr != 2) break;
            if (fr == 2) static_cast<ConvLayer*>(cur)->pw.reset(static_cast<ConvLayer*>(net.layers[consumer].release()));
            top->fused_away = true;
            cur->tops[0] = nx->tops[0];
            net.layers.erase(net.layers.begin() + consumer);
        }
    }
}

static int plan_concurrency(Net& net)
{
    const size_t L = net.layers.size();
    net.side.assign(L, -1);
    net.waits.assign(L, std::vector<int>());
    if (!net.concurrency) return 0;
    int pairs = 0;
    for (size_t i = 0; i < L; ++i)
    {
        Layer* l = net.layers[i].get();
        if ((l->type != "Convolution" && l->type != "ConvolutionDepthWise") || l->arena_bytes() != 0 || l->tops.size() != 1) continue;
        if (l->sibling_state()) continue;
        size_t consumer = 0;
        int uses = 0;
        for (size_t j = i + 1; j < L; ++j)
            for (Blob* b : net.layers[j]->bottoms)
                if (b == l->tops[0] || b->alias == l->tops[0])
                {
                    ++uses;
                    consumer = j;
                }
        if (uses != 1 || consumer <= i + 1) continue;
        bool work_between = false;
        for (size_t j = i + 1; j < consumer; ++j) work_between = work_between || net.layers[j]->algo() >= 0;
        if (!work_between) continue;
        net.side[i] = pairs;
        net.waits[consumer].push_back(pairs);
        ++pairs;
    }
    if (pairs && !net.side_stream) FHIP_CHECK_HIP(hipStreamCreateWithFlags(&net.side_stream, hipStreamNonBlocking));
    while (net.events.size() < (size_t)2 * pairs)
    {
        hipEvent_t e;
        FHIP_CHECK_HIP(hipEventCreateWithFlags(&e, hipEventDisableTiming));
        net.events.push_back(e);
    }
    return 0;
}

static int plan_chains(Net& net)
{
    const size_t L = net.layers.size();
    std::vector<ConvLayer*> conv(L, nullptr);
    for (size_t i = 0; i < L; ++i)
        if (net.layers[i]->type == "Convolution" || net.layers[i]->type == "ConvolutionDepthWise")
        {
            conv[i] = static_cast<ConvLayer*>(net.layers[i].get());
            conv[i]->chain_next = nullptr;
            conv[i]->chain_in = false;
            conv[i]->chain_pos = 0;
            conv[i]->chain_bytes = 0;
            conv[i]->head = conv[i]->head_of = nullptr;
        }
    for (auto& kv : net.blobs) kv.second->chained = false;
    for (auto& b : net.shadowed) b->chained = false;
    net.chain_slot[0] = net.chain_slot[1] = net.chain_m = 0;
    if (net.fusion < 3) return 0;
    auto plain = [](const ConvLayer* c) { return c && !c->pw && !c->residual && c->algo_ == FHIP_WINOGRADF63 && c->tops.size() == 1 && c->bottoms.size() == 1; };
    for (size_t i = 0; i + 1 < L; ++i)
    {
        ConvLayer *a = conv[i], *b = conv[i + 1];
        if (!plain(a) || !plain(b) || b->bottoms[0] != a->tops[0]) continue;
        if (a->fuse_pool && !a->pool_fast) continue;
        int uses = 0;
        for (size_t j = 0; j < L; ++j)
            for (Blob* x : net.layers[j]->bottoms) uses += (x == a->tops[0] || x->alias == a->tops[0]) ? 1 : 0;
        if (uses != 1) continue;
        if (!fhip_conv_can_chain_winograd(&a->p, a->algo_, &b->p, b->algo_, a->fuse_pool ? 1 : 0)) continue;
        a->chain_next = b;
        b->chain_in = true;
        b->chain_pos = a->chain_pos + 1;
        a->tops[0]->chained = true;
        a->tops[0]->drop_storage();
    }
    for (size_t i = 0; i + 1 < L; ++i)
    {
        ConvLayer *a = conv[i], *b = conv[i + 1];
        if (!a || a->pw || a->residual || a->fuse_pool || a->chain_in || a->chain_next || a->tops.size() != 1 || a->bottoms.size() != 1) continue;
        if (!a->first_candidate() || !plain(b) || b->chain_in || b->bottoms[0] != a->tops[0]) continue;
        int uses = 0;
        for (size_t j = 0; j < L; ++j)
            for (Blob* x : net.layers[j]->bottoms) uses += (x == a->tops[0] || x->alias == a->tops[0]) ? 1 : 0;
        if (uses != 1) continue;
        if (!fhip_conv_can_fuse_first_winograd(&a->p, &b->p, b->algo_, a->bottoms[0]->n)) continue;
        a->head_of = b;
        b->head = a;
        a->tops[0]->chained = true;
        a->tops[0]->drop_storage();
    }
    auto restore = [](Blob* b) -> int {
        if (b->chained || b->data || b->alias || b->fused_away || b->count() == 0) return 0;
        FHIP_CHECK_HIP(hipMalloc((void**)&b->data, b->count() * sizeof(float)));
        b->capacity = b->count();
        return 0;
    };
    for (auto& kv : net.blobs)
        if (const int rc = restore(kv.second.get())) return rc;
    for (auto& b : net.shadowed)
        if (const int rc = restore(b.get())) return rc;
    auto up = [](size_t x) { return (x + 255) / 256 * 256; };
    size_t slot[2] = {0, 0}, msz = 0;
    for (size_t i = 0; i < L; ++i)
    {
        ConvLayer* c = conv[i];
        if (!c || (!c->chain_in && !c->chain_next && !c->head)) continue;
        fhip_winograd_plan pl;
        const int rc = fhip_winograd_f63_plan(&c->p, c->bottoms[0]->n, &pl);
        if (rc) return rc;
        slot[c->chain_pos & 1] = std::max(slot[c->chain_pos & 1], up(pl.v_bytes));
        msz = std::max(msz, up(pl.m_bytes));
    }
    net.chain_slot[0] = 0;
    net.chain_slot[1] = slot[0];
    net.chain_m = slot[0] + slot[1];
    for (size_t i = 0; i < L; ++i)
        if (conv[i] && (conv[i]->chain_in || conv[i]->chain_next || conv[i]->head)) conv[i]->chain_bytes = slot[0] + slot[1] + msz;
    return 0;
}

static int plan_siblings(Net& net)
{
    const size_t L = net.layers.size();
    std::vector<ConvLayer*> conv(L, nullptr);
    for (size_t i = 0; i < L; ++i)
        if (net.layers[i]->type == "Convolution")
        {
            conv[i] = static_cast<ConvLayer*>(net.layers[i].get());
            conv[i]->sib = conv[i]->sib_of = nullptr;
        }
    if (net.fusion < 2) return 0;
    auto root = [](const Blob* b) { return b->alias ? b->alias : b; };
    auto plain = [](const ConvLayer* c) {
        return c && !c->pw && !c->residual && !c->fuse_pool && !c->chain_in && !c->chain_next && !c->head && !c->head_of && !c->sib && !c->sib_of &&
               c->algo_ == FHIP_IM2COL && c->tops.size() == 1 && c->bottoms.size() == 1;
    };
    for (size_t i = 0; i + 1 < L; ++i)
    {
        ConvLayer *a = conv[i], *b = conv[i + 1];
        if (!plain(a) || !plain(b) || root(a->bottoms[0]) != root(b->bottoms[0]) || a->tops[0] == b->tops[0]) continue;
        if (a->p.output_channels <= 64 || b->p.output_channels <= 64) continue;
        if (!fhip_conv_can_fuse_siblings(&a->p, a->algo_, &b->p, b->algo_, a->bottoms[0]->n)) continue;
        a->sib = b;
        b->sib_of = a;
    }
    for (size_t i = 0; i < L; ++i)
        if (conv[i] && !conv[i]->sib && conv[i]->sib_packed.bytes)
        {
            conv[i]->sib_packed.release();
            conv[i]->sib_bias.release();
            conv[i]->sib_packed_for = nullptr;
        }
    return 0;
}

static int reshape_all(Net& net)
{
    net.drop_graph();
    size_t need = 0;
    for (auto& l : net.layers)
    {
        const int rc = l->Reshape();
        if (rc) return rc;
    }
    {
        int rc = plan_chains(net);
        if (rc) return rc;
        if ((rc = plan_siblings(net))) return rc;
    }
    for (auto& l : net.layers) need = std::max(need, l->arena_bytes());
    if (need > net.arena.bytes)
    {
        const int rc = net.arena.resize(need);
        if (rc) return rc;
    }
    net.shapes_dirty = false;
    return plan_concurrency(net);
}

static int prepare(Net& net)
{
    if (!net.param_loaded) return failf(NET_E_IO, "Network has not been loaded. Please load the param file first.");
    if (!net.weights_loaded)
    {
        bool needs = false;
        for (auto& l : net.layers) needs = needs || (l->type != "Input" && l->type != "ReLU" && l->type != "Pooling" && l->type != "Softmax" &&
                                                     l->type != "Split" && l->type != "Eltwise" && l->type != "Concat" && l->type != "Dropout" &&
                                                     l->type != "Sigmoid" && l->type != "TanH" && l->type != "Clip" && l->type != "ShuffleChannel" &&
                                                     l->type != "Slice");
        if (needs) return failf(NET_E_IO, "weights have not been loaded");
    }
    fuse_layers(net);
    for (auto& kv : net.blobs)
        if (!kv.second->fused_away && kv.second->count() == 0)
        {
            bool is_input = false;
            for (auto& l : net.layers)
                if (l->type == "Input")
                    for (Blob* tb : l->tops) is_input = is_input || tb == kv.second.get();
            if (is_input) return failf(NET_E_SHAPE, "input blob %s has not been fed", kv.first.c_str());
        }
    if (net.shapes_dirty)
    {
        const int rc = reshape_all(net);
        if (rc) return rc;
    }
    for (auto& l : net.layers)
    {
        const int rc = l->Init(net.stream);
        if (rc) return rc;
    }
    net.initialized = true;
    return 0;
}

static int run_layers(Net& net)
{
    for (size_t i = 0; i < net.layers.size(); ++i)
    {
        Layer* l = net.layers[i].get();
        if (i < net.side.size() && net.side[i] >= 0)
        {
            hipEvent_t fork = net.events[2 * net.side[i]], join = net.events[2 * net.side[i] + 1];
            FHIP_CHECK_HIP(hipEventRecord(fork, net.stream));
            FHIP_CHECK_HIP(hipStreamWaitEvent(net.side_stream, fork, 0));
            const int rc = l->Forward(net.side_stream);
            if (rc) return rc;
            FHIP_CHECK_HIP(hipEventRecord(join, net.side_stream));
            continue;
        }
        if (i < net.waits.size())
            for (int pair : net.waits[i]) FHIP_CHECK_HIP(hipStreamWaitEvent(net.stream, net.events[2 * pair + 1], 0));
        const int rc = l->Forward(net.stream);
        if (rc) return rc;
    }
    return 0;
}

static int forward(Net& net)
{
    int rc = prepare(net);
    if (rc) return rc;
    if (!net.use_graph) return run_layers(net);
    if (!net.graph_exec)
    {
        hipGraph_t graph = nullptr;
        FHIP_CHECK_HIP(hipStreamBeginCapture(net.stream, hipStreamCaptureModeThreadLocal));
        rc = run_layers(net);
        const hipError_t e = hipStreamEndCapture(net.stream, &graph);
        if (rc)
        {
            if (graph) (void)hipGraphDestroy(graph);
            return rc;
        }
        FHIP_CHECK_HIP(e);
        const hipError_t ei = hipGraphInstantiate(&net.graph_exec, graph, nullptr, nullptr, 0);
        (void)hipGraphDestroy(graph);
        FHIP_CHECK_HIP(ei);
    }
    FHIP_CHECK_HIP(hipGraphLaunch(net.graph_exec, net.stream));
    return 0;
}
// ... 392 lines not shown
        return fhip_pixels_to_float_images(out, n->plans.data() + plan_at[r], n->staging + plan_at[r], mean, norm, s);
    });
}

int fhip_net_forward(fhip_net* n)
{
    NET_GUARD(n);
    if (n->more.empty()) return forward(n->impl);
    if (n->share.empty()) return failf(NET_E_SHAPE, "no input has been fed");
    FHIP_CHECK_HIP(hipEventRecord(n->fork, n->impl.stream));
    for (size_t r = 0; r < n->more.size(); ++r)
    {
        if (n->share[r + 1] < 1) continue;
        Net& m = n->more[r]->impl;
        FHIP_CHECK_HIP(hipStreamWaitEvent(m.stream, n->fork, 0));
        const int rc = forward(m);
        if (rc) return rc;
        FHIP_CHECK_HIP(hipEventRecord(n->joins[r], m.stream));
    }
    const int rc = forward(n->impl);
    if (rc) return rc;
    for (size_t r = 0; r < n->more.size(); ++r)
        if (n->share[r + 1] > 0) FHIP_CHECK_HIP(hipStreamWaitEvent(n->impl.stream, n->joins[r], 0));
    return FHIP_OK;
}

int fhip_net_extract(fhip_net* n, const char* blob_name, float** ptr, int* num, int* c, int* h, int* w)
{
    NET_GUARD(n);
    if (!blob_name || !ptr) return fail(FHIP_E_BADARG, "null argument");
    Blob* b = n->impl.find(blob_name);
    if (!b) return failf(NET_E_IO, "Cannot find output blob %s", blob_name);
    if (b->fused_away) return failf(NET_E_IO, "blob %s was fused into its consumer; disable fusion to extract it", blob_name);
    if (b->chained)
        return failf(NET_E_IO, "blob %s exists only as the next layer's transformed input at fusion level 3; use level 2 to extract it", blob_name);
    if (b->alias) b->data = b->alias->data;
    *ptr = b->data;
    if (num) *num = b->n;
    if (c) *c = b->c;
    if (h) *h = b->h;
    if (w) *w = b->w;
    if (n->more.empty() || n->share.size() < 2 || n->share[1] < 1) return FHIP_OK;
    size_t total = b->count();
    int images = b->n;
    std::vector<std::pair<float*, size_t>> pieces(1, std::make_pair(b->data, b->count()));
    for (size_t r = 0; r < n->more.size(); ++r)
    {
        if (n->share[r + 1] < 1) continue;
        float* d = nullptr;
        int pn, pc, ph, pw;
        const int rc = fhip_net_extract(n->more[r].get(), blob_name, &d, &pn, &pc, &ph, &pw);
        if (rc) return rc;
        if (pc != b->c || ph != b->h || pw != b->w) return failf(NET_E_SHAPE, "blob %s has different shapes in the sub-batch replicas", blob_name);
        pieces.push_back(std::make_pair(d, (size_t)pn * pc * ph * pw));
        total += pieces.back().second;
        images += pn;
    }
    DeviceVec& g = n->gathered[blob_name];
    if (g.bytes < total * sizeof(float))
    {
        FHIP_CHECK_HIP(hipStreamSynchronize(n->impl.stream));
        const int rc = g.resize(total * sizeof(float));
        if (rc) return rc;
    }
    size_t at = 0;
    for (auto& pc_ : pieces)
    {
        if (pc_.first && pc_.second)
            FHIP_CHECK_HIP(hipMemcpyAsync(g.d + at, pc_.first, pc_.second * sizeof(float), hipMemcpyDeviceToDevice, n->impl.stream));
        at += pc_.second;
    }
    *ptr = g.d;
    if (num) *num = images;
    return FHIP_OK;
}

int fhip_net_extract_host(fhip_net* n, const char* blob_name, float* host, size_t capacity)
{
    float* d = nullptr;
    int num, c, h, w;
    const int rc = fhip_net_extract(n, blob_name, &d, &num, &c, &h, &w);
    if (rc) return rc;
    const size_t count = (size_t)num * c * h * w;
    if (!host || capacity < count) return fail(FHIP_E_BADARG, "host buffer too small");
    if (!d) return fail(FHIP_E_BADARG, "blob has no data yet (run Forward first)");
    FHIP_CHECK_HIP(hipMemcpyAsync(host, d, count * sizeof(float), hipMemcpyDeviceToHost, n->impl.stream));
    FHIP_CHECK_HIP(hipStreamSynchronize(n->impl.stream));
    return FHIP_OK;
}

int fhip_net_layer_count(fhip_net* n)
{
    NET_GUARD(n);
    return (int)n->impl.layers.size();
}

int fhip_net_layer_info(fhip_net* n, int index, char* type, char* name, int len, int* algo)
{
    NET_GUARD(n);
    if (index < 0 || index >= (int)n->impl.layers.size()) return fail(FHIP_E_BADARG, "layer index out of range");
    Layer* l = n->impl.layers[index].get();
    if (type && len > 0) snprintf(type, len, "%s", l->type.c_str());
    if (name && len > 0) snprintf(name, len, "%s", l->name.c_str());
    if (algo) *algo = l->algo();
    return FHIP_OK;
}

int fhip_net_layer_conv_param(fhip_net* n, int index, fhip_conv_param* param, int* batch)
{
    NET_GUARD(n);
    if (index < 0 || index >= (int)n->impl.layers.size() || !param) return fail(FHIP_E_BADARG, "layer index out of range");
    Layer* l = n->impl.layers[index].get();
    const fhip_conv_param* cp = l->conv_param();
    if (!cp) return fail(FHIP_E_BADARG, "not a convolution layer");
    *param = *cp;
    if (batch) *batch = l->bottoms.empty() ? 0 : l->bottoms[0]->n;
    return FHIP_OK;
}

int fhip_net_layer_fused_pointwise(fhip_net* n, int index, fhip_conv_param* param, int* one_kernel)
{
    NET_GUARD(n);
    if (index < 0 || index >= (int)n->impl.layers.size() || !param) return fail(FHIP_E_BADARG, "layer index out of range");
    const fhip_conv_param* cp = n->impl.layers[index]->fused_pointwise(one_kernel);
    if (!cp) return fail(FHIP_E_BADARG, "no pointwise convolution was absorbed into this layer");
    *param = *cp;
    return FHIP_OK;
}

int fhip_net_layer_sibling(fhip_net* n, int index, int* state)
{
    NET_GUARD(n);
    if (index < 0 || index >= (int)n->impl.layers.size() || !state) return fail(FHIP_E_BADARG, "layer index out of range");
    *state = n->impl.layers[index]->sibling_state();
    return FHIP_OK;
}

int fhip_net_layer_residual(fhip_net* n, int index, int* state)
{
    NET_GUARD(n);
    if (index < 0 || index >= (int)n->impl.layers.size() || !state) return fail(FHIP_E_BADARG, "layer index out of range");
    *state = n->impl.layers[index]->residual_state();
    return FHIP_OK;
}

int fhip_net_layer_chain(fhip_net* n, int index, int* v_from_previous, int* writes_next_v)
{
    NET_GUARD(n);
    if (index < 0 || index >= (int)n->impl.layers.size() || !v_from_previous || !writes_next_v) return fail(FHIP_E_BADARG, "layer index out of range");
    n->impl.layers[index]->chain_state(v_from_previous, writes_next_v);
    return FHIP_OK;
}

int fhip_net_forward_timed(fhip_net* n, float* ms)
{
    NET_GUARD(n);
    if (!ms) return fail(FHIP_E_BADARG, "null argument");
    if (!n->more.empty())
        return fail(FHIP_E_UNSUPPORTED, "per-layer timing of a net with sub-batch replicas: kernels of concurrent replicas share the chip, "
                                        "so their durations are not layer times -- time a net created without fhip_net_set_sub_batches");
    Net& net = n->impl;
    int rc = prepare(net);
    if (rc) return rc;
    const size_t L = net.layers.size();
    std::vector<hipEvent_t> ev(L + 1);
    for (auto& e : ev) FHIP_CHECK_HIP(hipEventCreate(&e));
    FHIP_CHECK_HIP(hipEventRecord(ev[0], net.stream));
    for (size_t i = 0; i < L && rc == 0; ++i)
    {
        rc = net.layers[i]->Forward(net.stream);
        (void)hipEventRecord(ev[i + 1], net.stream);
    }
    (void)hipStreamSynchronize(net.stream);
    if (rc == 0)
        for (size_t i = 0; i < L; ++i) (void)hipEventElapsedTime(&ms[i], ev[i], ev[i + 1]);
    for (auto& e : ev) (void)hipEventDestroy(e);
    return rc;
}

int fhip_net_memory(fhip_net* n, size_t* blob_bytes, size_t* weight_bytes, size_t* arena_bytes)
{
    NET_GUARD(n);
    size_t bb = 0, wb = 0;
    for (auto& kv : n->impl.blobs) bb += kv.second->capacity * sizeof(float);
    for (auto& b : n->impl.shadowed) bb += b->capacity * sizeof(float);
    for (auto& l : n->impl.layers) wb += l->weight_bytes();
    size_t ab = n->impl.arena.bytes;
    for (auto& m : n->more)
    {
        size_t b2 = 0, w2 = 0, a2 = 0;
        (void)fhip_net_memory(m.get(), &b2, &w2, &a2);
        bb += b2;
        wb += w2;
        ab += a2;
    }
    for (auto& kv : n->gathered) bb += kv.second.bytes;
    if (blob_bytes) *blob_bytes = bb;
    if (weight_bytes) *weight_bytes = wb;
    if (arena_bytes) *arena_bytes = ab;
    return FHIP_OK;
}

}
```

feathercnn_amd/csrc/winograd_f63.hip:

```cpp
#include <algorithm>

#include "gemm_core.h"
#include "wino_gemm_policy.h"
#include "wino_gemm_glds.h"

namespace fhip
{

__device__ __forceinline__ void bt8(float& r0, float& r1, float& r2, float& r3, float& r4, float& r5, float& r6, float& r7)
{
    const float o0 = (r0 - r6) + 5.25f * (r4 - r2);
    const float o7 = (r7 - r1) + 5.25f * (r3 - r5);
    const float t1 = (r2 + r6) - 4.25f * r4;
    const float t2 = (r1 + r5) - 4.25f * r3;
    const float p1 = r6 + (0.25f * r2 - 1.25f * r4);
    const float p2 = (0.5f * r1 - 2.5f * r3) + 2.f * r5;
    const float q1 = r6 + 4.f * (r2 - 1.25f * r4);
    const float q2 = (2.f * r1 - 2.5f * r3) + 0.5f * r5;
    r0 = o0;
    r1 = t1 + t2;
    r2 = t1 - t2;
    r3 = p1 + p2;
    r4 = p1 - p2;
    r5 = q1 + q2;
    r6 = q1 - q2;
    r7 = o7;
}

__device__ __forceinline__ void at6(float m0, float m1, float m2, float m3, float m4, float m5, float m6, float m7,
                                    float& s0, float& s1, float& s2, float& s3, float& s4, float& s5)
{
    const float a12 = m1 + m2, d12 = m1 - m2;
    const float a34 = m3 + m4, d34 = m3 - m4;
    const float a56 = m5 + m6, d56 = m5 - m6;
    s0 = (m0 + a12) + (a34 + 32.f * a56);
    s1 = (d12 + 2.f * d34) + 16.f * d56;
    s2 = (a12 + 4.f * a34) + 8.f * a56;
    s3 = (d12 + 8.f * d34) + 4.f * d56;
    s4 = (a12 + 16.f * a34) + 2.f * a56;
    s5 = ((d12 + 32.f * d34) + d56) + m7;
}

__global__ __launch_bounds__(256) void wino_filter_transform_kernel(float* __restrict__ U, const float* __restrict__ w,
                                                                   int C, int K, int Cp, int Kp)
{
    const int k = blockIdx.x * blockDim.x + threadIdx.x;
    const int c = blockIdx.y;
    if (k >= K) return;
    const float* g = w + ((size_t)k * C + c) * 9;
    float gg[3][3];
#pragma unroll
    for (int i = 0; i < 3; ++i)
#pragma unroll
        for (int j = 0; j < 3; ++j) gg[i][j] = g[i * 3 + j];
    const float G[8][3] = {{1.0f, 0.0f, 0.0f},
                           {-2.0f / 9, -2.0f / 9, -2.0f / 9},
                           {-2.0f / 9, 2.0f / 9, -2.0f / 9},
                           {1.0f / 90, 1.0f / 45, 2.0f / 45},
                           {1.0f / 90, -1.0f / 45, 2.0f / 45},
                           {1.0f / 45, 1.0f / 90, 1.0f / 180},
                           {1.0f / 45, -1.0f / 90, 1.0f / 180},
                           {0.0f, 0.0f, 1.0f}};
    float mid[8][3];
#pragma unroll
    for (int i = 0; i < 8; ++i)
#pragma unroll
        for (int j = 0; j < 3; ++j) mid[i][j] = G[i][0] * gg[0][j] + G[i][1] * gg[1][j] + G[i][2] * gg[2][j];
    const size_t xi_stride = (size_t)Cp * Kp;
    float* up = U + (size_t)c * Kp + k;
#pragma unroll
    for (int i = 0; i < 8; ++i)
#pragma unroll
        for (int j = 0; j < 8; ++j)
            up[(size_t)(i * 8 + j) * xi_stride] = mid[i][0] * G[j][0] + mid[i][1] * G[j][1] + mid[i][2] * G[j][2];
}

struct WinoXformParams
{
    int C, K, H, W, OH, OW, PL, PT;
    int TX, T;
    int P, Pp;
    int N;
    WinoLayout Lv, Lm;
};

__global__ __launch_bounds__(256) void wino_input_transform_kernel(float* __restrict__ V, const float* __restrict__ in,
                                                                  const WinoXformParams q)
{
    const long long idx = (long long)blockIdx.x * blockDim.x + threadIdx.x;
    if (idx >= (long long)q.C * q.P) return;
    const int c = (int)(idx / q.P);
    const int p = (int)(idx - (long long)c * q.P);
    const int n = p / q.T, t = p - n * q.T;
    const int ty = t / q.TX, tx = t - ty * q.TX;
    const int y0 = ty * 6 - q.PT, x0 = tx * 6 - q.PL;
    const float* ip = in + ((size_t)n * q.C + c) * q.H * q.W;

    float d[8][8];
    const bool interior = (y0 >= 0) && (x0 >= 0) && (y0 + 8 <= q.H) && (x0 + 8 <= q.W);
    if (interior)
    {
#pragma unroll
        for (int i = 0; i < 8; ++i)
#pragma unroll
            for (int j = 0; j < 8; ++j) d[i][j] = ip[(size_t)(y0 + i) * q.W + x0 + j];
    }
    else
    {
#pragma unroll
        for (int i = 0; i < 8; ++i)
        {
            const int y = y0 + i;
            const bool yok = (unsigned)y < (unsigned)q.H;
#pragma unroll
            for (int j = 0; j < 8; ++j)
            {
                const int x = x0 + j;
                const bool ok = yok && ((unsigned)x < (unsigned)q.W);
                d[i][j] = ok ? ip[(size_t)y * q.W + x] : 0.f;
            }
        }
    }
#pragma unroll
    for (int j = 0; j < 8; ++j) bt8(d[0][j], d[1][j], d[2][j], d[3][j], d[4][j], d[5][j], d[6][j], d[7][j]);
#pragma unroll
    for (int i = 0; i < 8; ++i) bt8(d[i][0], d[i][1], d[i][2], d[i][3], d[i][4], d[i][5], d[i][6], d[i][7]);

    const size_t xi_stride = q.Lv.xis;
    float* vp = V + (size_t)c * q.Lv.bp + q.Lv.col(p);
#pragma unroll
    for (int i = 0; i < 8; ++i)
#pragma unroll
        for (int j = 0; j < 8; ++j) st_scratch(vp + (size_t)(i * 8 + j) * xi_stride, d[i][j]);
}

}
#include "wino_first.h"
namespace fhip
{

struct WinoStaged
{
    int UB;
    int LDW;
    int units;
    int TY;
    int R;
};

template <bool HAS_BIAS, bool RELU>
__global__ __launch_bounds__(256) void wino_output_transform_kernel(float* __restrict__ out, const float* __restrict__ M,
                                                                   const float* __restrict__ bias, const WinoXformParams q)
{
    const int p = blockIdx.x * blockDim.x + threadIdx.x;
    const int k = blockIdx.y;
    if (p >= q.P) return;
    const int n = p / q.T, t = p - n * q.T;
    const int ty = t / q.TX, tx = t - ty * q.TX;

    const size_t xi_stride = q.Lm.xis;
    const float* mp = M + (size_t)k * q.Lm.bp + q.Lm.col(p);
    float m[8][8];
#pragma unroll
    for (int i = 0; i < 8; ++i)
#pragma unroll
        for (int j = 0; j < 8; ++j) m[i][j] = ld_scratch(mp + (size_t)(i * 8 + j) * xi_stride);

    float tmp[6][8];
#pragma unroll
    for (int j = 0; j < 8; ++j)
        at6(m[0][j], m[1][j], m[2][j], m[3][j], m[4][j], m[5][j], m[6][j], m[7][j], tmp[0][j], tmp[1][j], tmp[2][j],
            tmp[3][j], tmp[4][j], tmp[5][j]);
    const float b = HAS_BIAS ? bias[k] : 0.f;
    const int oy0 = ty * 6, ox0 = tx * 6;
    float* op = out + (((size_t)n * q.K + k) * q.OH + oy0) * q.OW + ox0;
#pragma unroll
    for (int a = 0; a < 6; ++a)
    {
        float y[6];
        at6(tmp[a][0], tmp[a][1], tmp[a][2], tmp[a][3], tmp[a][4], tmp[a][5], tmp[a][6], tmp[a][7], y[0], y[1], y[2], y[3],
            y[4], y[5]);
        if (oy0 + a < q.OH)
        {
#pragma unroll
            for (int bb = 0; bb < 6; ++bb)
                if (ox0 + bb < q.OW)
                {
                    float v = y[bb] + b;
                    if (RELU) v = fmaxf(v, 0.f);
                    op[(size_t)a * q.OW + bb] = v;
                }
        }
    }
}
// ... 1132 lines not shown
```

feathercnn_amd/net.py:

```python
from __future__ import annotations

import ctypes

import numpy as np

from . import _lib
from .booster import ALGO_NAMES, FeatherHipError, _check, _stream


ROUTE_GCONV = 100
ROUTE_NAMES = dict(ALGO_NAMES)
ROUTE_NAMES[ROUTE_GCONV] = "GCONV"
ROUTE_DECONV = 101
ROUTE_NAMES[ROUTE_DECONV] = "DECONV"
ROUTE_INORM = 102
ROUTE_NAMES[ROUTE_INORM] = "INORM"
ROUTE_SHUFFLE = 103
ROUTE_NAMES[ROUTE_SHUFFLE] = "SHUFFLE"

class Net:
    def __init__(self, fusion: int = 1, graph: bool = False, stream=None, tuned: bool = False, concurrency: bool = False,
                 sub_batches: int = 1):
        self._lib = _lib.load_library()
        h = ctypes.c_void_p()
# ... 48 lines not shown
            shape, ptr, dev = a.shape, a.ctypes.data_as(ctypes.c_void_p), 0
            keep = a
        if len(shape) == 3:
            shape = (1,) + tuple(shape)
        if len(shape) != 4:
            raise FeatherHipError("FeedInput wants [N][C][H][W] or [C][H][W]")
        n, c, h, w = (int(v) for v in shape)
        _check(self._lib.fhip_net_feed_input(self._h, input_name.encode(), n, c, h, w, ptr, dev), "fhip_net_feed_input")
        self.synchronize()
        del keep
        return 0

    def FeedPixels(self, input_name: str, pixels, ptype: int, target=None, mean=None, norm=None) -> int:
        from .pixels import _images, _per_channel, pixel_channels
        import torch
        n, h, w, ptr, dev, keep = _images(pixels, ptype)
        tw, th = (w, h) if target is None else (int(target[0]), int(target[1]))
        _, cout = pixel_channels(ptype)
        m, mp = _per_channel(mean, cout, "mean")
        s, sp = _per_channel(norm, cout, "norm")
        if dev:
            torch.cuda.current_stream().synchronize()
        _check(self._lib.fhip_net_feed_pixels(self._h, input_name.encode(), n, ptr, int(ptype), w, h, tw, th, mp, sp, dev),
               "fhip_net_feed_pixels")
        self.synchronize()
        del keep, m, s
        return 0

    def FeedPixelImages(self, input_name: str, images, ptype: int, target, rois=None, mean=None, norm=None) -> int:
        from .pixels import _image_descs, _per_channel, pixel_channels
        import torch
        descs, dev, keep = _image_descs(images, ptype, rois)
        tw, th = int(target[0]), int(target[1])
        _, cout = pixel_channels(ptype)
        m, mp = _per_channel(mean, cout, "mean")
        s, sp = _per_channel(norm, cout, "norm")
        if dev:
            torch.cuda.current_stream().synchronize()
        _check(self._lib.fhip_net_feed_pixel_images(self._h, input_name.encode(), len(descs), descs, int(ptype), tw, th, mp, sp, dev),
               "fhip_net_feed_pixel_images")
        self.synchronize()
        del keep, m, s
        return 0

    def FeedYUV420sp(self, input_name: str, frames, ptype: int = 1, target=None, resize_first: bool = True, mean=None, norm=None) -> int:
        from .pixels import _frames, _per_channel
        import torch
        n, w, h, cout, ptr, dev, keep = _frames(frames, ptype)
        tw, th = (w, h) if target is None else (int(target[0]), int(target[1]))
        m, mp = _per_channel(mean, cout, "mean")
        s, sp = _per_channel(norm, cout, "norm")
        if dev:
            torch.cuda.current_stream().synchronize()
        _check(self._lib.fhip_net_feed_yuv420sp(self._h, input_name.encode(), n, ptr, w, h, tw, th, int(ptype), int(bool(resize_first)), mp,
                                                sp, dev), "fhip_net_feed_yuv420sp")
        self.synchronize()
        del keep, m, s
        return 0

    def Forward(self) -> int:
        _check(self._lib.fhip_net_forward(self._h), "fhip_net_forward")
        return 0

    def Extract(self, blob_name: str) -> np.ndarray:
        ptr, shape = self.ExtractDevice(blob_name)
        out = np.empty(shape, dtype=np.float32)
        _check(self._lib.fhip_net_extract_host(self._h, blob_name.encode(), out.ctypes.data_as(ctypes.c_void_p), out.size),
               "fhip_net_extract_host")
        return out

    def ExtractPixels(self, blob_name: str, ptype: int, target=None, mean=None, norm=None) -> np.ndarray:
        from .pixels import _check_pixout, _per_channel, output_channels
        cn = output_channels(ptype)
        ptr, (n, c, h, w) = self.ExtractDevice(blob_name)
        if c != cn:
            raise FeatherHipError(f"blob {blob_name} has {c} channels, pixel type {ptype:#x} needs {cn}")
        if not ptr:
            raise FeatherHipError(f"blob {blob_name} has no data yet (run Forward first)")
        tw, th = (w, h) if target is None else (int(target[0]), int(target[1]))
        m, mp = _per_channel(mean, cn, "mean")
        s, sp = _per_channel(norm, cn, "norm")
        stream = ctypes.c_void_p()
        _check(self._lib.fhip_net_get_stream(self._h, ctypes.byref(stream)), "fhip_net_get_stream")
        out = np.empty((n, th, tw, cn), dtype=np.uint8)
        _check_pixout(_lib.load_pixout_library().fhip_float_to_pixels_host(out.ctypes.data_as(ctypes.c_void_p), 0, ctypes.c_void_p(ptr), n,
                                                                           int(ptype), w, h, tw, th, mp, sp, stream),
                      "fhip_float_to_pixels_host")
        del m, s
        return out

    def ExtractDevice(self, blob_name: str):
        p = ctypes.c_void_p()
        dims = [ctypes.c_int() for _ in range(4)]
        _check(self._lib.fhip_net_extract(self._h, blob_name.encode(), ctypes.byref(p), *[ctypes.byref(d) for d in dims]),
               "fhip_net_extract")
        return p.value, tuple(d.value for d in dims)

    def synchronize(self):
        import torch
        torch.cuda.synchronize()

    def layers(self):
        out = []
        n = self._lib.fhip_net_layer_count(self._h)
        for i in range(n):
            t, nm, algo = ctypes.create_string_buffer(64), ctypes.create_string_buffer(256), ctypes.c_int()
            _check(self._lib.fhip_net_layer_info(self._h, i, t, nm, 64, ctypes.byref(algo)), "fhip_net_layer_info")
            out.append((t.value.decode(), nm.value.decode(), ROUTE_NAMES.get(algo.value)))
        return out

    def conv_params(self):
        out = {}
        for i in range(self._lib.fhip_net_layer_count(self._h)):
            p, b = _lib.fhip_conv_param(), ctypes.c_int()
            if self._lib.fhip_net_layer_conv_param(self._h, i, ctypes.byref(p), ctypes.byref(b)) == 0:
                out[i] = (p, b.value)
        return out

    def fused_pointwise(self):
        out = {}
        for i in range(self._lib.fhip_net_layer_count(self._h)):
            p, one = _lib.fhip_conv_param(), ctypes.c_int()
            if self._lib.fhip_net_layer_fused_pointwise(self._h, i, ctypes.byref(p), ctypes.byref(one)) == 0:
                out[i] = (p, bool(one.value))
        return out

    def siblings(self):
        out = {}
        for i in range(self._lib.fhip_net_layer_count(self._h)):
            st = ctypes.c_int()
            if self._lib.fhip_net_layer_sibling(self._h, i, ctypes.byref(st)) == 0 and st.value:
                out[i] = st.value
        return out

    def residuals(self):
        out = {}
        for i in range(self._lib.fhip_net_layer_count(self._h)):
            st = ctypes.c_int()
            if self._lib.fhip_net_layer_residual(self._h, i, ctypes.byref(st)) == 0 and st.value:
                out[i] = st.value
        return out

    def chains(self, raw=False):
        out = {}
        for i in range(self._lib.fhip_net_layer_count(self._h)):
            a, b = ctypes.c_int(), ctypes.c_int()
            if self._lib.fhip_net_layer_chain(self._h, i, ctypes.byref(a), ctypes.byref(b)) == 0 and (a.value or b.value):
                if raw:
                    out[i] = (a.value, b.value)
                elif a.value == 1 or b.value == 1:
                    out[i] = (a.value == 1, b.value == 1)
        return out

    def forward_timed(self):
        n = self._lib.fhip_net_layer_count(self._h)
        ms = (ctypes.c_float * max(n, 1))()
        _check(self._lib.fhip_net_forward_timed(self._h, ms), "fhip_net_forward_timed")
        info = self.layers()
        return [(t, nm, a, ms[i]) for i, (t, nm, a) in enumerate(info)]

    def memory(self):
        v = [ctypes.c_size_t() for _ in range(3)]
        _check(self._lib.fhip_net_memory(self._h, *[ctypes.byref(x) for x in v]), "fhip_net_memory")
        return {"blob_bytes": v[0].value, "weight_bytes": v[1].value, "arena_bytes": v[2].value}


def _p(t):
    return ctypes.c_void_p(t.data_ptr()) if t is not None else None


def relu(x):
    import torch
    y = torch.empty_like(x)
    _check(_lib.load_library().fhip_relu(_p(y), _p(x), x.numel(), _stream()), "fhip_relu")
    return y


def add(a, b, relu: bool = False):
    import torch
    y = torch.empty_like(a)
    _check(_lib.load_library().fhip_add(_p(y), _p(a), _p(b), a.numel(), int(relu), _stream()), "fhip_add")
    return y


def affine(x, mul, add_=None, relu: bool = False):
    import torch
    y = torch.empty_like(x)
    n, c, h, w = x.shape
    _check(_lib.load_library().fhip_affine(_p(y), _p(x), _p(mul), _p(add_), n, c, h * w, int(relu), _stream()),
           "fhip_affine")
    return y


def pool_param(c, h, w, kernel, stride=1, pad=(0, 0, 0, 0), pooling_type=0, global_pooling=False):
    kh, kw = (kernel, kernel) if isinstance(kernel, int) else kernel
    sh, sw = (stride, stride) if isinstance(stride, int) else stride
    return _lib.fhip_pool_param(c, h, w, kh, kw, sh, sw, pad[0], pad[1], pad[2], pad[3], pooling_type, int(global_pooling))


def pooling(x, q):
    import torch
    oh, ow = ctypes.c_int(), ctypes.c_int()
    lib = _lib.load_library()
    _check(lib.fhip_pooling_output_dim(ctypes.byref(q), ctypes.byref(oh), ctypes.byref(ow)), "fhip_pooling_output_dim")
    y = torch.empty((x.shape[0], x.shape[1], oh.value, ow.value), device=x.device, dtype=torch.float32)
    _check(lib.fhip_pooling(ctypes.byref(q), x.shape[0], _p(y), _p(x), _stream()), "fhip_pooling")
    return y


def softmax(x):
    import torch
    y = torch.empty_like(x)
    _check(_lib.load_library().fhip_softmax(_p(y), _p(x), x.shape[0], x[0].numel(), _stream()), "fhip_softmax")
    return y
```

include/feather_hip/feather_hip.h:

```cpp
#ifndef FEATHER_HIP_H_
#define FEATHER_HIP_H_

#include <stddef.h>

#ifdef __cplusplus
extern "C" {
#endif

#define FHIP_API __attribute__((visibility("default")))

enum fhip_conv_algo
{
    FHIP_NAIVE = 0,
    FHIP_IM2COL = 1,
    FHIP_SGECONV = 2,
    FHIP_DEPTHWISE = 3,
    FHIP_WINOGRADF63 = 4,
    FHIP_WINOGRADF63FUSED = 5,
    FHIP_WINOGRADF23 = 6
};

enum fhip_activation
{
    FHIP_ACT_NONE = 0,
    FHIP_ACT_RELU = 1
};

enum fhip_error
{
    FHIP_OK = 0,
    FHIP_E_UNSUPPORTED = -1,
    FHIP_E_BADARG = -2,
    FHIP_E_HIP = -3,
    FHIP_E_NODEVICE = -4
};

typedef struct fhip_conv_param
{
    int output_channels;
    int input_channels;
    int input_h;
    int input_w;
    int kernel_h;
    int kernel_w;
    int output_h;
    int output_w;
    int stride_h;
    int stride_w;
    int pad_left;
    int pad_bottom;
    int pad_right;
    int pad_top;
    int group;
    int bias_term;
    int activation;
} fhip_conv_param;

FHIP_API int fhip_conv_assign_output_dim(fhip_conv_param* param);

FHIP_API double fhip_conv_flops(const fhip_conv_param* param);

FHIP_API int fhip_conv_select_algo(const fhip_conv_param* param, int* algo);
FHIP_API int fhip_conv_select_algo_tuned(const fhip_conv_param* param, int* algo);

FHIP_API int fhip_conv_get_buffer_size(const fhip_conv_param* param, int algo, int batch, size_t* buffer_bytes,
                                       size_t* processed_kernel_bytes);

FHIP_API int fhip_conv_init(const fhip_conv_param* param, int algo, float* processed_kernel, const float* kernel,
                            void* stream);

FHIP_API int fhip_conv_forward(const fhip_conv_param* param, int algo, int batch, float* output, const float* input,
                               const float* processed_kernel, float* buffer, const float* bias_arr, void* stream);


typedef struct fhip_winograd_plan
{
    int tiles_x, tiles_y;
    int tiles_per_image;
    int columns;
    int columns_padded;
    int column_block;
    int frequency_points;
    int tile_outputs;
    int in_channels_padded;
    int out_channels_padded;
    size_t v_offset_bytes, v_bytes;
    size_t m_offset_bytes, m_bytes;
    size_t u_bytes;
} fhip_winograd_plan;

FHIP_API int fhip_winograd_f63_plan(const fhip_conv_param* param, int batch, fhip_winograd_plan* plan);

FHIP_API int fhip_winograd_f63_transform_kernel(const fhip_conv_param* param, float* u, const float* kernel,
                                                void* stream);
FHIP_API int fhip_winograd_f63_input_transform(const fhip_conv_param* param, int batch, float* v, const float* input,
                                               void* stream);
FHIP_API int fhip_winograd_f63_tile_gemm(const fhip_conv_param* param, int batch, float* m, const float* u,
                                         const float* v, void* stream);
FHIP_API int fhip_winograd_f63_output_transform(const fhip_conv_param* param, int batch, float* output, const float* m,
                                                const float* bias_arr, void* stream);


enum fhip_stage
{
    FHIP_STAGE_WINO_INPUT = 0,
    FHIP_STAGE_WINO_GEMM = 1,
    FHIP_STAGE_WINO_OUTPUT = 2,
    FHIP_STAGE_IGEMM = 3,
    FHIP_STAGE_DEPTHWISE = 4,
    FHIP_STAGE_INIT = 5,
    FHIP_STAGE_WINO_CHAIN = 6,
    FHIP_STAGE_COUNT = 7
};
FHIP_API int fhip_stage_timing_enable(int on);
FHIP_API int fhip_stage_timing_collect(double* ms, long long* launches);

FHIP_API const char* fhip_last_error(void);
FHIP_API const char* fhip_version(void);
FHIP_API int fhip_conv_streams_1x1(const fhip_conv_param* param, int algo, int batch);

FHIP_API int fhip_device_info(char* name, int name_len, int* compute_units, int* lds_bytes);
FHIP_API int fhip_calibrate_mfma_f32(double* tflops, double* shader_mhz, void* stream);

#ifdef __cplusplus
}
#endif
#endif
```

include/feather_hip/feather_net.h:

```cpp
#ifndef FEATHER_NET_H_
#define FEATHER_NET_H_

#include "feather_hip/feather_hip.h"

#ifdef __cplusplus
extern "C" {
#endif


FHIP_API int fhip_relu(float* y, const float* x, size_t count, void* stream);

FHIP_API int fhip_add(float* y, const float* a, const float* b, size_t count, int relu, void* stream);

FHIP_API int fhip_affine(float* y, const float* x, const float* mul, const float* add, int batch, int channels, int hw,
                         int relu, void* stream);


enum
{
    FHIP_PIXEL_CONVERT_SHIFT = 16,
    FHIP_PIXEL_RGB = 1,
    FHIP_PIXEL_BGR = (1 << 1),
    FHIP_PIXEL_GRAY = (1 << 2),
    FHIP_PIXEL_RGBA = (1 << 3),
    FHIP_PIXEL_RGB2BGR = FHIP_PIXEL_RGB | (FHIP_PIXEL_BGR << FHIP_PIXEL_CONVERT_SHIFT),
    FHIP_PIXEL_RGB2GRAY = FHIP_PIXEL_RGB | (FHIP_PIXEL_GRAY << FHIP_PIXEL_CONVERT_SHIFT),
    FHIP_PIXEL_BGR2RGB = FHIP_PIXEL_BGR | (FHIP_PIXEL_RGB << FHIP_PIXEL_CONVERT_SHIFT),
    FHIP_PIXEL_BGR2GRAY = FHIP_PIXEL_BGR | (FHIP_PIXEL_GRAY << FHIP_PIXEL_CONVERT_SHIFT),
    FHIP_PIXEL_GRAY2RGB = FHIP_PIXEL_GRAY | (FHIP_PIXEL_RGB << FHIP_PIXEL_CONVERT_SHIFT),
    FHIP_PIXEL_GRAY2BGR = FHIP_PIXEL_GRAY | (FHIP_PIXEL_BGR << FHIP_PIXEL_CONVERT_SHIFT),
    FHIP_PIXEL_RGBA2RGB = FHIP_PIXEL_RGBA | (FHIP_PIXEL_RGB << FHIP_PIXEL_CONVERT_SHIFT),
    FHIP_PIXEL_RGBA2BGR = FHIP_PIXEL_RGBA | (FHIP_PIXEL_BGR << FHIP_PIXEL_CONVERT_SHIFT),
    FHIP_PIXEL_RGBA2GRAY = FHIP_PIXEL_RGBA | (FHIP_PIXEL_GRAY << FHIP_PIXEL_CONVERT_SHIFT)
};

FHIP_API int fhip_pixels_to_float(float* output, const unsigned char* pixels, int batch, int type, int w, int h, int target_w, int target_h,
                                  const float* mean, const float* norm, void* stream);

FHIP_API int fhip_yuv420sp_to_float(float* output, const unsigned char* yuv, int batch, int type, int w, int h, int target_w, int target_h,
                                    int resize_first, const float* mean, const float* norm, void* stream);

typedef struct fhip_pixel_image
{
    const unsigned char* data;
    int w, h, stride;
    int roi_x, roi_y, roi_w, roi_h;
} fhip_pixel_image;

FHIP_API int fhip_pixel_images_plan(const fhip_pixel_image* images, int batch, int type, int target_w, int target_h, void* plan,
                                    size_t* plan_bytes);
FHIP_API int fhip_pixels_to_float_images(float* output, const void* plan, const void* plan_device, const float* mean, const float* norm,
                                         void* stream);

FHIP_API int fhip_conv_can_fuse_maxpool2(const fhip_conv_param* param, int algo);
FHIP_API int fhip_conv_forward_maxpool2(const fhip_conv_param* param, int algo, int batch, float* pooled_output, const float* input,
                                        const float* packed, float* buffer, const float* bias, void* stream);

FHIP_API int fhip_conv_can_fuse_residual(const fhip_conv_param* param, int algo);
FHIP_API int fhip_conv_forward_residual(const fhip_conv_param* param, int algo, int batch, float* output, const float* input,
                                        const float* packed, float* buffer, const float* bias, const float* residual, void* stream);

FHIP_API int fhip_conv_can_fuse_dw_pw(const fhip_conv_param* dw, const fhip_conv_param* pw, int batch);
FHIP_API int fhip_conv_forward_dw_pw(const fhip_conv_param* dw, const fhip_conv_param* pw, int batch, float* output, const float* input,
                                     const float* dw_packed, const float* dw_bias, const float* pw_packed, const float* pw_bias, void* stream);

typedef struct fhip_pool_param
{
    int channels, input_h, input_w;
    int kernel_h, kernel_w;
    int stride_h, stride_w;
    int pad_left, pad_right, pad_top, pad_bottom;
    int pooling_type;
    int global_pooling;
} fhip_pool_param;

FHIP_API int fhip_pooling_output_dim(const fhip_pool_param* p, int* out_h, int* out_w);
FHIP_API int fhip_pooling(const fhip_pool_param* p, int batch, float* y, const float* x, void* stream);

FHIP_API int fhip_softmax(float* y, const float* x, int batch, int count_per_image, void* stream);

FHIP_API int fhip_conv_can_chain_winograd(const fhip_conv_param* param, int algo, const fhip_conv_param* next, int next_algo, int pool);
FHIP_API int fhip_conv_forward_chained(const fhip_conv_param* param, int batch, float* output, const float* input, const float* packed, float* v,
                                       float* m, const float* bias, const fhip_conv_param* next, float* v_next, int pool, void* stream);
FHIP_API int fhip_winograd_f63_output_to_next_input(const fhip_conv_param* param, const fhip_conv_param* next, int batch, float* v_next,
                                                    const float* m, const float* bias, int pool, void* stream);

FHIP_API int fhip_conv_can_fuse_siblings(const fhip_conv_param* a, int algo_a, const fhip_conv_param* b, int algo_b, int batch);
FHIP_API int fhip_conv_siblings_geometry(const fhip_conv_param* a, const fhip_conv_param* b, fhip_conv_param* both);
FHIP_API int fhip_conv_forward_siblings(const fhip_conv_param* a, const fhip_conv_param* b, int batch, float* output_a, float* output_b,
                                        const float* input, const float* packed_both, const float* bias_both, void* stream);

FHIP_API int fhip_conv_can_fuse_first_winograd(const fhip_conv_param* first, const fhip_conv_param* next, int next_algo, int batch);
FHIP_API int fhip_winograd_f63_input_from_first(const fhip_conv_param* first, const fhip_conv_param* next, int batch, float* v_next,
                                                const float* input, const float* first_kernel, const float* first_bias, void* stream);


typedef struct fhip_net fhip_net;

FHIP_API int fhip_net_create(fhip_net** net);
FHIP_API int fhip_net_destroy(fhip_net* net);
FHIP_API int fhip_net_set_stream(fhip_net* net, void* stream);
FHIP_API int fhip_net_get_stream(fhip_net* net, void** stream);
FHIP_API int fhip_net_set_fusion(fhip_net* net, int on);
FHIP_API int fhip_net_set_tuned_selection(fhip_net* net, int on);
FHIP_API int fhip_net_set_concurrency(fhip_net* net, int on);
FHIP_API int fhip_net_set_graph(fhip_net* net, int on);

FHIP_API int fhip_net_set_sub_batches(fhip_net* net, int replicas);

FHIP_API int fhip_net_load_param(fhip_net* net, const char* path);
FHIP_API int fhip_net_load_param_mem(fhip_net* net, const char* text, size_t len);
FHIP_API int fhip_net_load_weights(fhip_net* net, const char* path);
FHIP_API int fhip_net_load_weights_mem(fhip_net* net, const void* data, size_t len);
FHIP_API int fhip_net_load_weights_device(fhip_net* net, const void* device_data, size_t len);

FHIP_API int fhip_net_feed_input(fhip_net* net, const char* blob_name, int n, int c, int h, int w, const float* data,
                                 int on_device);
FHIP_API int fhip_net_feed_pixels(fhip_net* net, const char* blob_name, int n, const unsigned char* pixels, int type, int w, int h,
                                  int target_w, int target_h, const float* mean, const float* norm, int on_device);
FHIP_API int fhip_net_feed_yuv420sp(fhip_net* net, const char* blob_name, int n, const unsigned char* yuv, int w, int h, int target_w,
                                    int target_h, int type, int resize_first, const float* mean, const float* norm, int on_device);
FHIP_API int fhip_net_feed_pixel_images(fhip_net* net, const char* blob_name, int n, const fhip_pixel_image* images, int type,
                                        int target_w, int target_h, const float* mean, const float* norm, int on_device);
FHIP_API int fhip_net_forward(fhip_net* net);
FHIP_API int fhip_net_extract(fhip_net* net, const char* blob_name, float** device_ptr, int* n, int* c, int* h, int* w);
FHIP_API int fhip_net_extract_host(fhip_net* net, const char* blob_name, float* host, size_t capacity);

FHIP_API int fhip_net_layer_count(fhip_net* net);
#define FHIP_NET_ROUTE_GCONV 100
#define FHIP_NET_ROUTE_DECONV 101
#define FHIP_NET_ROUTE_INORM 102
#define FHIP_NET_ROUTE_SHUFFLE 103
FHIP_API int fhip_net_layer_info(fhip_net* net, int index, char* type, char* name, int len, int* algo);
FHIP_API int fhip_net_layer_conv_param(fhip_net* net, int index, fhip_conv_param* param, int* batch);
FHIP_API int fhip_net_layer_fused_pointwise(fhip_net* net, int index, fhip_conv_param* param, int* one_kernel);
FHIP_API int fhip_net_layer_chain(fhip_net* net, int index, int* v_from_previous, int* writes_next_v);
FHIP_API int fhip_net_layer_sibling(fhip_net* net, int index, int* state);
FHIP_API int fhip_net_layer_residual(fhip_net* net, int index, int* state);
FHIP_API int fhip_net_forward_timed(fhip_net* net, float* ms);
FHIP_API int fhip_net_memory(fhip_net* net, size_t* blob_bytes, size_t* weight_bytes, size_t* arena_bytes);

#ifdef __cplusplus
}
#endif
#endif
```

Measured before the change: 9849 images/s.

## Run chained Winograd layers on 2x2 image canvases at small spatial sizes

```diff
diff --git a/__graft_entry__.py b/__graft_entry__.py
--- a/__graft_entry__.py
+++ b/__graft_entry__.py
@@ -21,6 +21,7 @@
     _lib.load_deconv_library()
     _lib.load_inorm_library()
     _lib.load_shuffle_library()
+    _lib.load_canvas_library()
     from feathercnn_amd import provenance
     provenance.write_stamp()
 
diff --git a/feathercnn_amd/_lib.py b/feathercnn_amd/_lib.py
--- a/feathercnn_amd/_lib.py
+++ b/feathercnn_amd/_lib.py
@@ -10,6 +10,7 @@
 _DECONV = None
 _INORM = None
 _SHUFFLE = None
+_CANVAS = None
 
 STAGE_NAMES = ("wino_input", "wino_gemm", "wino_output", "igemm", "depthwise", "init", "wino_chain")
 
@@ -54,6 +55,8 @@
     "fhip_conv_init": (_I, [_P, _I, _V, _V, _V]),
     "fhip_conv_forward": (_I, [_P, _I, _I, _V, _V, _V, _V, _V, _V]),
     "fhip_winograd_f63_plan": (_I, [_P, _I, ctypes.POINTER(fhip_winograd_plan)]),
+    "fhip_winograd_f63_plan_canvas": (_I, [_P, _I, _I, ctypes.POINTER(fhip_winograd_plan)]),
+    "fhip_winograd_f63_canvas_param": (_I, [_P, _I, _P]),
     "fhip_winograd_f63_transform_kernel": (_I, [_P, _V, _V, _V]),
     "fhip_winograd_f63_input_transform": (_I, [_P, _I, _V, _V, _V]),
     "fhip_winograd_f63_tile_gemm": (_I, [_P, _I, _V, _V, _V, _V]),
@@ -115,6 +118,7 @@
     "fhip_net_layer_conv_param": (_I, [_V, _I, _P, _PI]),
     "fhip_net_layer_fused_pointwise": (_I, [_V, _I, _P, _PI]),
     "fhip_net_layer_chain": (_I, [_V, _I, _PI, _PI]),
+    "fhip_net_layer_canvas": (_I, [_V, _I, _PI]),
     "fhip_net_layer_sibling": (_I, [_V, _I, _PI]),
     "fhip_net_layer_residual": (_I, [_V, _I, _PI]),
     "fhip_net_forward_timed": (_I, [_V, ctypes.POINTER(ctypes.c_float)]),
@@ -179,6 +183,13 @@
     "fhip_shuffle_last_error": (ctypes.c_char_p, []),
 }
 
+_PL = ctypes.POINTER(fhip_winograd_plan)
+CANVAS_SIGNATURES = {
+    "fhip_canvas_output_to_next_input": (_I, [_I, _P, _P, _I, _PL, _PL, _V, _V, _V, _V]),
+    "fhip_canvas_output_transform": (_I, [_P, _I, _PL, _V, _V, _V, _I, _V]),
+    "fhip_canvas_last_error": (ctypes.c_char_p, []),
+}
+
 
 def lib_path() -> str:
     return os.environ.get("FEATHER_HIP_LIB", os.path.join(_HERE, "libfeather_hip.so"))
@@ -304,3 +315,24 @@
             fn.argtypes = args
         _SHUFFLE = lib
     return _SHUFFLE
+
+
+def canvas_path() -> str:
+    return os.path.join(_HERE, "libfeather_canvas.so")
+
+
+def load_canvas_library():
+    global _CANVAS
+    if _CANVAS is None:
+        import torch
+        path = canvas_path()
+        if not os.path.exists(path):
+            raise RuntimeError(f"feathercnn_amd: HIP library {path} is missing -- run `python -c 'import __graft_entry__ as g; "
+                               "g.build()'` (or `make -C feathercnn_amd/csrc`). There is no CPU fallback.")
+        lib = ctypes.CDLL(path)
+        for name, (res, args) in CANVAS_SIGNATURES.items():
+            fn = getattr(lib, name)
+            fn.restype = res
+            fn.argtypes = args
+        _CANVAS = lib
+    return _CANVAS
diff --git a/feathercnn_amd/canvas.py b/feathercnn_amd/canvas.py
--- /dev/null
+++ b/feathercnn_amd/canvas.py
@@ -0,0 +1,70 @@
+from __future__ import annotations
+
+import ctypes
+
+from . import _lib
+from .booster import FeatherHipError, _check, _ptr, _stream
+
+ENTRY, INSIDE, EXIT = 1, 2, 3
+
+
+def plan_canvas(param, batch: int, canvas: bool):
+    pl, c = _lib.fhip_winograd_plan(), param._c()
+    _check(_lib.load_library().fhip_winograd_f63_plan_canvas(ctypes.byref(c), int(batch), 2 if canvas else 1, ctypes.byref(pl)),
+           "fhip_winograd_f63_plan_canvas")
+    return pl
+
+
+def canvas_param(param, batch: int):
+    q, c = _lib.fhip_conv_param(), param._c()
+    return q if _lib.load_library().fhip_winograd_f63_canvas_param(ctypes.byref(c), int(batch), ctypes.byref(q)) == 0 else None
+
+
+def _check_canvas(rc, what):
+    if rc != 0:
+        raise FeatherHipError(f"{what} failed ({rc}): {_lib.load_canvas_library().fhip_canvas_last_error().decode()}")
+
+
+def forward_chained_canvas(layers, x, pools, canvas, fill=None, keep=False):
+    import torch
+    lib, clib = _lib.load_library(), _lib.load_canvas_library()
+    batch, dev = x.shape[0], x.device
+    assert not canvas[0] and len(layers) == len(pools) == len(canvas)
+    plans = [plan_canvas(l.param, batch, cv) for l, cv in zip(layers, canvas)]
+    new = (lambda n: torch.full((n,), fill, dtype=torch.float32, device=dev)) if fill is not None else (lambda n: torch.empty(n, dtype=torch.float32, device=dev))
+    vbuf = [new(max(pl.v_bytes for pl in plans[k::2]) // 4) if plans[k::2] else None for k in (0, 1)]
+    m = new(max(pl.m_bytes for pl in plans) // 4)
+    last = layers[-1].param
+    oh, ow = (last.output_h // 2, last.output_w // 2) if pools[-1] else (last.output_h, last.output_w)
+    out = new(batch * last.output_channels * oh * ow).reshape(batch, last.output_channels, oh, ow)
+    kept = []
+    for i, l in enumerate(layers):
+        c, v = l.param._c(), vbuf[i & 1]
+        bias = _ptr(l.bias) if l.bias is not None else None
+        if i == 0:
+            _check(lib.fhip_winograd_f63_input_transform(ctypes.byref(c), batch, _ptr(v), _ptr(x), _stream()), "fhip_winograd_f63_input_transform")
+        if canvas[i]:
+            cp = canvas_param(l.param, batch)
+            _check(lib.fhip_winograd_f63_tile_gemm(ctypes.byref(cp), batch // 4, _ptr(m), _ptr(l.packed), _ptr(v), _stream()), "fhip_winograd_f63_tile_gemm")
+        else:
+            _check(lib.fhip_winograd_f63_tile_gemm(ctypes.byref(c), batch, _ptr(m), _ptr(l.packed), _ptr(v), _stream()), "fhip_winograd_f63_tile_gemm")
+        if keep:
+            kept.append((v.clone(), m.clone(), plans[i]))
+        if i + 1 < len(layers):
+            cn, vn = layers[i + 1].param._c(), vbuf[(i + 1) & 1]
+            if canvas[i] or canvas[i + 1]:
+                form = ENTRY if not canvas[i] else INSIDE if canvas[i + 1] else EXIT
+                assert bool(pools[i]) == (form != INSIDE)
+                _check_canvas(clib.fhip_canvas_output_to_next_input(form, ctypes.byref(c), ctypes.byref(cn), batch, ctypes.byref(plans[i]),
+                                                                    ctypes.byref(plans[i + 1]), _ptr(vn), _ptr(m), bias, _stream()),
+                              "fhip_canvas_output_to_next_input")
+            else:
+                _check(lib.fhip_winograd_f63_output_to_next_input(ctypes.byref(c), ctypes.byref(cn), batch, _ptr(vn), _ptr(m), bias, int(pools[i]), _stream()),
+                       "fhip_winograd_f63_output_to_next_input")
+        elif canvas[i]:
+            _check_canvas(clib.fhip_canvas_output_transform(ctypes.byref(c), batch, ctypes.byref(plans[i]), _ptr(out), _ptr(m), bias, int(pools[i]), _stream()),
+                          "fhip_canvas_output_transform")
+        else:
+            _check(lib.fhip_conv_forward_chained(ctypes.byref(c), batch, _ptr(out), None, _ptr(l.packed), _ptr(v), _ptr(m), bias, None, None, int(pools[i]),
+                                                 _stream()), "fhip_conv_forward_chained")
+    return (out, kept) if keep else out
diff --git a/feathercnn_amd/csrc/capi.hip b/feathercnn_amd/csrc/capi.hip
--- a/feathercnn_amd/csrc/capi.hip
+++ b/feathercnn_amd/csrc/capi.hip
@@ -344,6 +344,42 @@
     return winograd_output_transform(*p, batch, output, m, bias, s, pool);
 }
 
+#ifndef FHIP_CANVAS_PLANES
+#define FHIP_CANVAS_PLANES 3
+#endif
+static bool winograd_canvas_param(const fhip_conv_param& p, int batch, fhip_conv_param* canvas)
+{
+    if (p.kernel_h != 3 || p.kernel_w != 3 || p.stride_h > 1 || p.stride_w > 1 || p.group > 1) return false;
+    if (p.pad_left != 1 || p.pad_right != 1 || p.pad_top != 1 || p.pad_bottom != 1) return false;
+    const int h = p.input_h;
+    if (batch < 4 || (batch & 3) || h != p.input_w || h < 2 || (h & 1) || (2 * h + 2) % 6 != 0) return false;
+    if (!((h == 14 && (FHIP_CANVAS_PLANES & 1)) || (h == 56 && (FHIP_CANVAS_PLANES & 2)))) return false;
+    const int side = 2 * h + 2, tiles = side / 6;
+    if (tiles * tiles > 512 || (size_t)(side + 2) * (side + 4) * sizeof(float) > 64 * 1024) return false;
+    fhip_conv_param q = p;
+    q.input_h = q.input_w = q.output_h = q.output_w = side;
+    fhip_winograd_plan own;
+    if (winograd_plan(p, batch, &own) != FHIP_OK || own.frequency_points != 64) return false;
+    if (canvas) *canvas = q;
+    return true;
+}
+
+int fhip_winograd_f63_canvas_param(const fhip_conv_param* p, int batch, fhip_conv_param* canvas)
+{
+    if (!valid_param(p) || !canvas) return fail(FHIP_E_BADARG, "bad argument");
+    if (!winograd_canvas_param(*p, batch, canvas)) return fail(FHIP_E_UNSUPPORTED, "this layer and batch do not run on 2x2 image canvases");
+    return FHIP_OK;
+}
+
+int fhip_winograd_f63_plan_canvas(const fhip_conv_param* p, int batch, int canvas, fhip_winograd_plan* plan)
+{
+    if (!valid_param(p) || !plan || (canvas != 1 && canvas != 2)) return fail(FHIP_E_BADARG, "bad argument");
+    if (canvas == 1) return winograd_plan(*p, batch, plan);
+    fhip_conv_param q;
+    if (!winograd_canvas_param(*p, batch, &q)) return fail(FHIP_E_UNSUPPORTED, "this layer and batch do not run on 2x2 image canvases");
+    return winograd_plan(q, batch / 4, plan);
+}
+
 int fhip_winograd_f63_output_to_next_input(const fhip_conv_param* p, const fhip_conv_param* next, int batch, float* v_next, const float* m,
                                            const float* bias, int pool, void* stream)
 {
diff --git a/feathercnn_amd/csrc/net.hip b/feathercnn_amd/csrc/net.hip
--- a/feathercnn_amd/csrc/net.hip
+++ b/feathercnn_amd/csrc/net.hip
@@ -14,6 +14,7 @@
 #include <vector>
 
 #include "common.h"
+#include "feather_hip/feather_canvas.h"
 #include "feather_hip/feather_deconv.h"
 #include "feather_hip/feather_gconv.h"
 #include "feather_hip/feather_inorm.h"
@@ -237,6 +238,53 @@
     if (!a.resolve || !a.create || !a.destroy || !a.forward || !a.last_error)
     {
         failf(FHIP_E_UNSUPPORTED, "libfeather_shuffle.so (%s) does not export the entry points of feather_shuffle.h", tried.c_str());
+        dlclose(h);
+        return nullptr;
+    }
+    api = a;
+    loaded = true;
+    return &api;
+}
+
+struct CanvasApi
+{
+    decltype(&fhip_canvas_output_to_next_input) chain = nullptr;
+    decltype(&fhip_canvas_output_transform) output = nullptr;
+    decltype(&fhip_canvas_last_error) last_error = nullptr;
+};
+
+static const CanvasApi* canvas_api()
+{
+    static std::mutex mu;
+    static CanvasApi api;
+    static bool loaded = false;
+    std::lock_guard<std::mutex> lk(mu);
+    if (loaded) return &api;
+    std::string tried;
+    void* h = nullptr;
+    Dl_info self;
+    if (dladdr((void*)&canvas_api, &self) && self.dli_fname)
+    {
+        std::string path = self.dli_fname;
+        const size_t slash = path.rfind('/');
+        path = (slash == std::string::npos ? std::string() : path.substr(0, slash + 1)) + "libfeather_canvas.so";
+        h = dlopen(path.c_str(), RTLD_NOW | RTLD_LOCAL);
+        tried = path;
+    }
+    if (!h) h = dlopen("libfeather_canvas.so", RTLD_NOW | RTLD_LOCAL);
+    if (!h)
+    {
+        failf(FHIP_E_UNSUPPORTED, "a chained Winograd run on 2x2 image canvases needs libfeather_canvas.so next to libfeather_hip.so (%s): %s",
+              tried.c_str(), dlerror());
+        return nullptr;
+    }
+    CanvasApi a;
+    a.chain = (decltype(a.chain))dlsym(h, "fhip_canvas_output_to_next_input");
+    a.output = (decltype(a.output))dlsym(h, "fhip_canvas_output_transform");
+    a.last_error = (decltype(a.last_error))dlsym(h, "fhip_canvas_last_error");
+    if (!a.chain || !a.output || !a.last_error)
+    {
+        failf(FHIP_E_UNSUPPORTED, "libfeather_canvas.so (%s) does not export the entry points of feather_canvas.h", tried.c_str());
         dlclose(h);
         return nullptr;
     }
@@ -533,6 +581,7 @@
     virtual const fhip_conv_param* conv_param() const { return nullptr; }
     virtual const fhip_conv_param* fused_pointwise(int*) const { return nullptr; }
     virtual void chain_state(int* v_from_previous, int* writes_next_v) const { *v_from_previous = *writes_next_v = 0; }
+    virtual int canvas_state() const { return 0; }
     virtual int sibling_state() const { return 0; }
     virtual int residual_state() const { return 0; }
 };
@@ -605,6 +654,9 @@
     bool chain_in = false;
     int chain_pos = 0;
     size_t chain_bytes = 0;
+    bool canvas = false;
+    fhip_conv_param canvas_p;
+    fhip_winograd_plan run_plan;
     ConvLayer* head_of = nullptr;
     ConvLayer* head = nullptr;
     DeviceVec first_raw;
@@ -858,6 +910,7 @@
                                                                   head->p.bias_term ? head->bias.d : nullptr, s);
                 if (rc) return rc;
             }
+            if (canvas || (chain_next && chain_next->canvas)) return forward_canvas(n, in, v, m, vn, b, s);
             if (chain_next) return fhip_conv_forward_chained(&p, n, nullptr, in, packed.d, v, m, b, &chain_next->p, vn, fuse_pool ? 1 : 0, s);
             if (!fuse_pool || pool_fast) return fhip_conv_forward_chained(&p, n, tops[0]->data, in, packed.d, v, m, b, nullptr, nullptr, fuse_pool ? 1 : 0, s);
             const int rc = fhip_conv_forward_chained(&p, n, pre_pool.d, in, packed.d, v, m, b, nullptr, nullptr, 0, s);
@@ -883,6 +936,27 @@
         if (rc) return rc;
         return fhip_pooling(&poolq, bottoms[0]->n, tops[0]->data, pre_pool.d, s);
     }
+    int forward_canvas(int n, const float* in, float* v, float* m, float* vn, const float* b, hipStream_t s)
+    {
+        const CanvasApi* api = canvas_api();
+        if (!api) return FHIP_E_UNSUPPORTED;
+        int rc;
+        if (in)
+        {
+            if (canvas) return failf(FHIP_E_UNSUPPORTED, "layer %s: a canvas layer takes its input from the chained transform before it", name.c_str());
+            if ((rc = fhip_winograd_f63_input_transform(&p, n, v, in, s))) return rc;
+        }
+        rc = canvas ? fhip_winograd_f63_tile_gemm(&canvas_p, n / 4, m, packed.d, v, s) : fhip_winograd_f63_tile_gemm(&p, n, m, packed.d, v, s);
+        if (rc) return rc;
+        if (chain_next)
+        {
+            const int form = !canvas ? FHIP_CANVAS_ENTRY : chain_next->canvas ? FHIP_CANVAS_INSIDE : FHIP_CANVAS_EXIT;
+            rc = api->chain(form, &p, &chain_next->p, n, &run_plan, &chain_next->run_plan, vn, m, b, s);
+        }
+        else
+            rc = api->output(&p, n, &run_plan, tops[0]->data, m, b, fuse_pool ? 1 : 0, s);
+        return rc ? failf(rc, "layer %s: %s", name.c_str(), api->last_error()) : 0;
+    }
     int Fuse(Layer* next, int level) override;
     bool FuseResidual(Blob* other)
     {
@@ -917,6 +991,7 @@
         *v_from_previous = head ? 2 : chain_in ? 1 : 0;
         *writes_next_v = head_of ? 2 : chain_next ? 1 : 0;
     }
+    int canvas_state() const override { return canvas ? 1 : 0; }
 };
 
 struct InnerProductLayer : Layer
@@ -2072,6 +2147,7 @@
             conv[i]->chain_in = false;
             conv[i]->chain_pos = 0;
             conv[i]->chain_bytes = 0;
+            conv[i]->canvas = false;
             conv[i]->head = conv[i]->head_of = nullptr;
         }
     for (auto& kv : net.blobs) kv.second->chained = false;
@@ -2095,6 +2171,39 @@
         a->tops[0]->chained = true;
         a->tops[0]->drop_storage();
     }
+    for (size_t i = 0; i < L; ++i)
+    {
+        ConvLayer* c = conv[i];
+        if (!c || !c->chain_in || c->canvas) continue;
+        ConvLayer* prev = nullptr;
+        for (size_t j = 0; j < i; ++j)
+            if (conv[j] && conv[j]->chain_next == c) prev = conv[j];
+        if (!prev || prev->canvas || !prev->fuse_pool || prev->head) continue;
+        const int n = c->bottoms[0]->n;
+        fhip_conv_param q;
+        if (fhip_winograd_f63_canvas_param(&prev->p, n, &q) == FHIP_OK) continue;
+        if (prev->p.kernel_h != 3 || prev->p.pad_left != 1 || prev->p.pad_right != 1 || prev->p.pad_top != 1 || prev->p.pad_bottom != 1 ||
+            prev->p.output_h != prev->p.output_w || prev->p.output_h != prev->p.input_h)
+            continue;
+        std::vector<ConvLayer*> run;
+        for (ConvLayer* x = c; x; x = x->chain_next)
+        {
+            if (x->p.input_h != c->p.input_h || x->p.input_w != c->p.input_w || fhip_winograd_f63_canvas_param(&x->p, n, &q) != FHIP_OK) break;
+            if (x->p.activation != FHIP_ACT_NONE && x->p.activation != FHIP_ACT_RELU) break;
+            run.push_back(x);
+            if (x->fuse_pool) break;
+        }
+        if (run.empty()) continue;
+        ConvLayer* last = run.back();
+        if (last->chain_next && !last->fuse_pool) continue;
+        if (!last->chain_next && last->fuse_pool && !last->pool_fast) continue;
+        if (!canvas_api()) return FHIP_E_UNSUPPORTED;
+        for (ConvLayer* x : run)
+        {
+            x->canvas = true;
+            (void)fhip_winograd_f63_canvas_param(&x->p, n, &x->canvas_p);
+        }
+    }
     for (size_t i = 0; i + 1 < L; ++i)
     {
         ConvLayer *a = conv[i], *b = conv[i + 1];
@@ -2127,8 +2236,9 @@
         ConvLayer* c = conv[i];
         if (!c || (!c->chain_in && !c->chain_next && !c->head)) continue;
         fhip_winograd_plan pl;
-        const int rc = fhip_winograd_f63_plan(&c->p, c->bottoms[0]->n, &pl);
-        if (rc) return rc;
+        const int rc = fhip_winograd_f63_plan_canvas(&c->p, c->bottoms[0]->n, c->canvas ? 2 : 1, &pl);
+        if (rc) return rc;
+        c->run_plan = pl;
         slot[c->chain_pos & 1] = std::max(slot[c->chain_pos & 1], up(pl.v_bytes));
         msz = std::max(msz, up(pl.m_bytes));
     }
@@ -2827,6 +2937,14 @@
     return FHIP_OK;
 }
 
+int fhip_net_layer_canvas(fhip_net* n, int index, int* canvas)
+{
+    NET_GUARD(n);
+    if (index < 0 || index >= (int)n->impl.layers.size() || !canvas) return fail(FHIP_E_BADARG, "layer index out of range");
+    *canvas = n->impl.layers[index]->canvas_state();
+    return FHIP_OK;
+}
+
 int fhip_net_forward_timed(fhip_net* n, float* ms)
 {
     NET_GUARD(n);
diff --git a/feathercnn_amd/csrc/wino_butterfly.h b/feathercnn_amd/csrc/wino_butterfly.h
--- /dev/null
+++ b/feathercnn_amd/csrc/wino_butterfly.h
@@ -0,0 +1,42 @@
+#pragma once
+
+#include <hip/hip_runtime.h>
+
+namespace fhip
+{
+
+__device__ __forceinline__ void bt8(float& r0, float& r1, float& r2, float& r3, float& r4, float& r5, float& r6, float& r7)
+{
+    const float o0 = (r0 - r6) + 5.25f * (r4 - r2);
+    const float o7 = (r7 - r1) + 5.25f * (r3 - r5);
+    const float t1 = (r2 + r6) - 4.25f * r4;
+    const float t2 = (r1 + r5) - 4.25f * r3;
+    const float p1 = r6 + (0.25f * r2 - 1.25f * r4);
+    const float p2 = (0.5f * r1 - 2.5f * r3) + 2.f * r5;
+    const float q1 = r6 + 4.f * (r2 - 1.25f * r4);
+    const float q2 = (2.f * r1 - 2.5f * r3) + 0.5f * r5;
+    r0 = o0;
+    r1 = t1 + t2;
+    r2 = t1 - t2;
+    r3 = p1 + p2;
+    r4 = p1 - p2;
+    r5 = q1 + q2;
+    r6 = q1 - q2;
+    r7 = o7;
+}
+
+__device__ __forceinline__ void at6(float m0, float m1, float m2, float m3, float m4, float m5, float m6, float m7,
+                                    float& s0, float& s1, float& s2, float& s3, float& s4, float& s5)
+{
+    const float a12 = m1 + m2, d12 = m1 - m2;
+    const float a34 = m3 + m4, d34 = m3 - m4;
+    const float a56 = m5 + m6, d56 = m5 - m6;
+    s0 = (m0 + a12) + (a34 + 32.f * a56);
+    s1 = (d12 + 2.f * d34) + 16.f * d56;
+    s2 = (a12 + 4.f * a34) + 8.f * a56;
+    s3 = (d12 + 8.f * d34) + 4.f * d56;
+    s4 = (a12 + 16.f * a34) + 2.f * a56;
+    s5 = ((d12 + 32.f * d34) + d56) + m7;
+}
+
+}
diff --git a/feathercnn_amd/csrc/winograd_f63.hip b/feathercnn_amd/csrc/winograd_f63.hip
--- a/feathercnn_amd/csrc/winograd_f63.hip
+++ b/feathercnn_amd/csrc/winograd_f63.hip
@@ -1,45 +1,12 @@
 #include <algorithm>
 
 #include "gemm_core.h"
+#include "wino_butterfly.h"
 #include "wino_gemm_policy.h"
 #include "wino_gemm_glds.h"
 
 namespace fhip
 {
-
-__device__ __forceinline__ void bt8(float& r0, float& r1, float& r2, float& r3, float& r4, float& r5, float& r6, float& r7)
-{
-    const float o0 = (r0 - r6) + 5.25f * (r4 - r2);
-    const float o7 = (r7 - r1) + 5.25f * (r3 - r5);
-    const float t1 = (r2 + r6) - 4.25f * r4;
-    const float t2 = (r1 + r5) - 4.25f * r3;
-    const float p1 = r6 + (0.25f * r2 - 1.25f * r4);
-    const float p2 = (0.5f * r1 - 2.5f * r3) + 2.f * r5;
-    const float q1 = r6 + 4.f * (r2 - 1.25f * r4);
-    const float q2 = (2.f * r1 - 2.5f * r3) + 0.5f * r5;
-    r0 = o0;
-    r1 = t1 + t2;
-    r2 = t1 - t2;
-    r3 = p1 + p2;
-    r4 = p1 - p2;
-    r5 = q1 + q2;
-    r6 = q1 - q2;
-    r7 = o7;
-}
-
-__device__ __forceinline__ void at6(float m0, float m1, float m2, float m3, float m4, float m5, float m6, float m7,
-                                    float& s0, float& s1, float& s2, float& s3, float& s4, float& s5)
-{
-    const float a12 = m1 + m2, d12 = m1 - m2;
-    const float a34 = m3 + m4, d34 = m3 - m4;
-    const float a56 = m5 + m6, d56 = m5 - m6;
-    s0 = (m0 + a12) + (a34 + 32.f * a56);
-    s1 = (d12 + 2.f * d34) + 16.f * d56;
-    s2 = (a12 + 4.f * a34) + 8.f * a56;
-    s3 = (d12 + 8.f * d34) + 4.f * d56;
-    s4 = (a12 + 16.f * a34) + 2.f * a56;
-    s5 = ((d12 + 32.f * d34) + d56) + m7;
-}
 
 __global__ __launch_bounds__(256) void wino_filter_transform_kernel(float* __restrict__ U, const float* __restrict__ w,
                                                                    int C, int K, int Cp, int Kp)
diff --git a/feathercnn_amd/csrc_canvas/canvas.hip b/feathercnn_amd/csrc_canvas/canvas.hip
--- /dev/null
+++ b/feathercnn_amd/csrc_canvas/canvas.hip
@@ -0,0 +1,429 @@
+#include <hip/hip_runtime.h>
+#include <stdint.h>
+
+#include <algorithm>
+#include <string>
+
+#include "feather_hip/feather_canvas.h"
+#include "wino_butterfly.h"
+#include "wino_layout.h"
+
+namespace fhip
+{
+
+static thread_local std::string g_error;
+
+static int fail(int code, const char* msg)
+{
+    g_error = msg;
+    return code;
+}
+
+#define FHIP_CANVAS_CHECK_HIP(expr)                                                                               \
+    do                                                                                                            \
+    {                                                                                                             \
+        const hipError_t e_ = (expr);                                                                             \
+        if (e_ != hipSuccess) return fail(FHIP_E_HIP, (std::string(#expr ": ") + hipGetErrorString(e_)).c_str()); \
+    } while (0)
+
+struct CanvasChain
+{
+    int K, NC;
+    int TX, T, Tq;
+    int IH;
+    int QP;
+    int TX2, T2, T2q;
+    int planes, ppb;
+    int LDW, LDH;
+    int sub, pf;
+    WinoLayout Lm, Lv2;
+};
+
+template <bool HAS_BIAS, bool RELU, int FORM, bool MULTI>
+__global__ __launch_bounds__(512, 3) void canvas_chain_kernel(float* __restrict__ Vn, const float* __restrict__ M, const float* __restrict__ bias,
+                                                              const CanvasChain g, const int units)
+{
+    extern __shared__ __attribute__((aligned(16))) float smem[];
+    const int tid = threadIdx.x, nthreads = blockDim.x;
+    for (int i = tid; i < g.ppb * g.pf; i += nthreads) smem[i] = 0.f;
+    const int n1 = MULTI ? (g.T + nthreads - 1) / nthreads : 1;
+    int pl = MULTI ? 0 : tid / g.T, t = tid - pl * g.T;
+    bool lane_on = MULTI ? t < g.T : pl < g.ppb;
+    const int pl2 = tid / g.T2, t2 = tid - pl2 * g.T2;
+    const bool lane_on2 = pl2 < g.ppb;
+    const int q2 = FORM == FHIP_CANVAS_EXIT ? t2 / g.T2q : 0, tt2 = t2 - q2 * g.T2q;
+    const int ty2 = tt2 / g.TX2, tx2 = tt2 - ty2 * g.TX2;
+    const int xcd = blockIdx.x & 7, j = blockIdx.x >> 3, xcd_blocks = (gridDim.x + 7 - xcd) >> 3;
+    const int u_lo = (int)((long long)units * xcd / 8), u_hi = (int)((long long)units * (xcd + 1) / 8);
+    const size_t xi_stride = g.Lm.xis, xi_stride2 = g.Lv2.xis;
+    float* const lp1 = smem + pl * g.pf;
+
+    float m[8][8];
+    auto fetch = [&](int unit, int tile) {
+        const int plane = min(unit * g.ppb + (lane_on ? pl : 0), g.planes - 1);
+        const int k = plane / g.NC, c = plane - k * g.NC;
+        const float* mp = M + (size_t)k * g.Lm.bp + g.Lm.col(c * g.T + min(tile, g.T - 1));
+#pragma unroll
+        for (int i = 0; i < 8; ++i)
+#pragma unroll
+            for (int jj = 0; jj < 8; ++jj) m[i][jj] = mp[(size_t)(i * 8 + jj) * xi_stride];
+    };
+    int unit = u_lo + j;
+    if (unit < u_hi) fetch(unit, t);
+    __syncthreads();
+    for (; unit < u_hi; unit += xcd_blocks)
+    {
+        const int plane = unit * g.ppb + pl;
+        const int k = min(plane, g.planes - 1) / g.NC;
+        for (int it = 0; it < n1; ++it)
+        {
+            if (MULTI)
+            {
+                t = tid + it * nthreads;
+                lane_on = t < g.T;
+            }
+            if (lane_on && plane < g.planes)
+            {
+                const int q = FORM == FHIP_CANVAS_ENTRY ? t / g.Tq : 0, tt = t - q * g.Tq;
+                const int ty = tt / g.TX, tx = tt - ty * g.TX;
+                float tmp[6][8];
+#pragma unroll
+                for (int jj = 0; jj < 8; ++jj)
+                    at6(m[0][jj], m[1][jj], m[2][jj], m[3][jj], m[4][jj], m[5][jj], m[6][jj], m[7][jj], tmp[0][jj], tmp[1][jj], tmp[2][jj], tmp[3][jj],
+                        tmp[4][jj], tmp[5][jj]);
+                const float b = HAS_BIAS ? bias[k] : 0.f;
+                float prev0 = 0.f, prev1 = 0.f, prev2 = 0.f;
+#pragma unroll
+                for (int a = 0; a < 6; ++a)
+                {
+                    float y[6];
+                    at6(tmp[a][0], tmp[a][1], tmp[a][2], tmp[a][3], tmp[a][4], tmp[a][5], tmp[a][6], tmp[a][7], y[0], y[1], y[2], y[3], y[4], y[5]);
+#pragma unroll
+                    for (int bb = 0; bb < 6; ++bb)
+                    {
+                        float v = y[bb] + b;
+                        if (RELU) v = fmaxf(v, 0.f);
+                        y[bb] = v;
+                    }
+                    if (FORM != FHIP_CANVAS_INSIDE)
+                    {
+                        const float h0 = fmaxf(y[0], y[1]), h1 = fmaxf(y[2], y[3]), h2 = fmaxf(y[4], y[5]);
+                        if ((a & 1) == 0)
+                        {
+                            prev0 = h0;
+                            prev1 = h1;
+                            prev2 = h2;
+                            continue;
+                        }
+                        const float pv[3] = {fmaxf(prev0, h0), fmaxf(prev1, h1), fmaxf(prev2, h2)};
+                        const int py = 3 * ty + (a >> 1);
+                        if (FORM == FHIP_CANVAS_ENTRY)
+                        {
+                            if (py < g.IH)
+                            {
+                                float* row = lp1 + (size_t)(py + 1 + (q >> 1) * g.QP) * g.LDW + 2 + 3 * tx + (q & 1) * g.QP;
+#pragma unroll
+                                for (int c = 0; c < 3; ++c) row[c] = (3 * tx + c < g.IH) ? pv[c] : 0.f;
+                            }
+                        }
+                        else
+                        {
+                            const int qy = py >= g.QP ? 1 : 0, yy = py - qy * g.QP;
+                            if (yy < g.IH)
+                            {
+#pragma unroll
+                                for (int c = 0; c < 3; ++c)
+                                {
+                                    const int px = 3 * tx + c, qx = px >= g.QP ? 1 : 0, xx = px - qx * g.QP;
+                                    if (xx < g.IH) lp1[(size_t)(2 * qy + qx) * g.sub + (size_t)(yy + 1) * g.LDW + 2 + xx] = pv[c];
+                                }
+                            }
+                        }
+                        continue;
+                    }
+                    const int ay = 6 * ty + a;
+                    const bool row_seam = (unsigned)(ay - g.IH) < 2u;
+                    float* row = lp1 + (size_t)(ay + 1) * g.LDW + 2 + 6 * tx;
+#pragma unroll
+                    for (int bb = 0; bb < 6; bb += 2)
+                    {
+                        const bool seam = row_seam || (unsigned)(6 * tx + bb - g.IH) < 2u;
+                        *reinterpret_cast<float2*>(row + bb) = seam ? make_float2(0.f, 0.f) : make_float2(y[bb], y[bb + 1]);
+                    }
+                }
+            }
+            if (MULTI && it + 1 < n1) fetch(unit, tid + (it + 1) * nthreads);
+        }
+        __syncthreads();
+        if (unit + xcd_blocks < u_hi) fetch(unit + xcd_blocks, MULTI ? tid : t);
+        __builtin_amdgcn_sched_barrier(0);
+        const int plane2 = unit * g.ppb + pl2;
+        if (lane_on2 && plane2 < g.planes)
+        {
+            const int k2 = plane2 / g.NC, c2 = plane2 - k2 * g.NC;
+            const float* lp = smem + (size_t)pl2 * g.pf + (size_t)q2 * g.sub + (size_t)(6 * ty2) * g.LDW + 6 * tx2 + 1;
+            float d[8][8];
+#pragma unroll
+            for (int i = 0; i < 8; ++i)
+#pragma unroll
+                for (int jj = 0; jj < 8; ++jj) d[i][jj] = lp[(size_t)i * g.LDW + jj];
+#pragma unroll
+            for (int jj = 0; jj < 8; ++jj) bt8(d[0][jj], d[1][jj], d[2][jj], d[3][jj], d[4][jj], d[5][jj], d[6][jj], d[7][jj]);
+#pragma unroll
+            for (int i = 0; i < 8; ++i) bt8(d[i][0], d[i][1], d[i][2], d[i][3], d[i][4], d[i][5], d[i][6], d[i][7]);
+            float* vp = Vn + (size_t)k2 * g.Lv2.bp + g.Lv2.col(c2 * g.T2 + t2);
+#pragma unroll
+            for (int i = 0; i < 8; ++i)
+#pragma unroll
+                for (int jj = 0; jj < 8; ++jj) vp[(size_t)(i * 8 + jj) * xi_stride2] = d[i][jj];
+        }
+        __syncthreads();
+    }
+}
+
+struct CanvasOut
+{
+    int K, T, TX, P;
+    int IH, QP;
+    WinoLayout Lm;
+};
+
+template <bool HAS_BIAS, bool RELU, bool POOL>
+__global__ __launch_bounds__(256) void canvas_output_kernel(float* __restrict__ out, const float* __restrict__ M, const float* __restrict__ bias,
+                                                            const CanvasOut g)
+{
+    const int p = blockIdx.x * blockDim.x + threadIdx.x;
+    const int k = blockIdx.y;
+    if (p >= g.P) return;
+    const int c = p / g.T, t = p - c * g.T;
+    const int ty = t / g.TX, tx = t - ty * g.TX;
+    const size_t xi_stride = g.Lm.xis;
+    const float* mp = M + (size_t)k * g.Lm.bp + g.Lm.col(p);
+    float m[8][8];
+#pragma unroll
+    for (int i = 0; i < 8; ++i)
+#pragma unroll
+        for (int jj = 0; jj < 8; ++jj) m[i][jj] = mp[(size_t)(i * 8 + jj) * xi_stride];
+    float tmp[6][8];
+#pragma unroll
+    for (int jj = 0; jj < 8; ++jj)
+        at6(m[0][jj], m[1][jj], m[2][jj], m[3][jj], m[4][jj], m[5][jj], m[6][jj], m[7][jj], tmp[0][jj], tmp[1][jj], tmp[2][jj], tmp[3][jj], tmp[4][jj],
+            tmp[5][jj]);
+    const float b = HAS_BIAS ? bias[k] : 0.f;
+    const size_t plane = (size_t)g.IH * g.IH;
+    float* const op = out + ((size_t)(4 * c) * g.K + k) * plane;
+    auto put = [&](int y, int x, float v) {
+        const int qy = y >= g.QP ? 1 : 0, yy = y - qy * g.QP, qx = x >= g.QP ? 1 : 0, xx = x - qx * g.QP;
+        if (yy < g.IH && xx < g.IH) op[(size_t)(2 * qy + qx) * g.K * plane + (size_t)yy * g.IH + xx] = v;
+    };
+    float prev0 = 0.f, prev1 = 0.f, prev2 = 0.f;
+#pragma unroll
+    for (int a = 0; a < 6; ++a)
+    {
+        float y[6];
+        at6(tmp[a][0], tmp[a][1], tmp[a][2], tmp[a][3], tmp[a][4], tmp[a][5], tmp[a][6], tmp[a][7], y[0], y[1], y[2], y[3], y[4], y[5]);
+#pragma unroll
+        for (int bb = 0; bb < 6; ++bb)
+        {
+            float v = y[bb] + b;
+            if (RELU) v = fmaxf(v, 0.f);
+            y[bb] = v;
+        }
+        if (POOL)
+        {
+            const float h0 = fmaxf(y[0], y[1]), h1 = fmaxf(y[2], y[3]), h2 = fmaxf(y[4], y[5]);
+            if ((a & 1) == 0)
+            {
+                prev0 = h0;
+                prev1 = h1;
+                prev2 = h2;
+            }
+            else
+            {
+                const int py = 3 * ty + (a >> 1);
+                put(py, 3 * tx, fmaxf(prev0, h0));
+                put(py, 3 * tx + 1, fmaxf(prev1, h1));
+                put(py, 3 * tx + 2, fmaxf(prev2, h2));
+            }
+            continue;
+        }
+#pragma unroll
+        for (int bb = 0; bb < 6; ++bb) put(6 * ty + a, 6 * tx + bb, y[bb]);
+    }
+}
+
+static int device_limits(int* cus, size_t* lds)
+{
+    static thread_local int dev_cached = -1, cus_cached = 0;
+    static thread_local size_t lds_cached = 0;
+    int dev = 0;
+    FHIP_CANVAS_CHECK_HIP(hipGetDevice(&dev));
+    if (dev != dev_cached)
+    {
+        hipDeviceProp_t prop;
+        FHIP_CANVAS_CHECK_HIP(hipGetDeviceProperties(&prop, dev));
+        cus_cached = prop.multiProcessorCount;
+        lds_cached = prop.maxSharedMemoryPerMultiProcessor;
+        dev_cached = dev;
+    }
+    *cus = cus_cached;
+    *lds = lds_cached;
+    return FHIP_OK;
+}
+
+static bool k3s1p1(const fhip_conv_param& c)
+{
+    return c.kernel_h == 3 && c.kernel_w == 3 && c.stride_h <= 1 && c.stride_w <= 1 && c.group <= 1 && c.pad_left == 1 && c.pad_right == 1 &&
+           c.pad_top == 1 && c.pad_bottom == 1 && c.input_h == c.input_w && c.output_h == c.input_h && c.output_w == c.input_w;
+}
+
+static bool plan_is(const fhip_winograd_plan& pl, int side, int images)
+{
+    const int tiles = (side + 2 + 3) / 6;
+    return pl.frequency_points == 64 && pl.tiles_x == tiles && pl.tiles_y == tiles && pl.tiles_per_image == tiles * tiles &&
+           (long long)pl.columns == (long long)tiles * tiles * images && pl.columns_padded >= pl.columns && pl.column_block > 0;
+}
+
+static int canvas_chain(int form, const fhip_conv_param& p, const fhip_conv_param& next, int batch, const fhip_winograd_plan& pp,
+                        const fhip_winograd_plan& pn, float* vn, const float* m, const float* bias, hipStream_t s)
+{
+    if (batch < 4 || (batch & 3)) return fail(FHIP_E_UNSUPPORTED, "canvases hold four images: the batch must be a multiple of 4");
+    if (!k3s1p1(p) || !k3s1p1(next) || next.input_channels != p.output_channels)
+        return fail(FHIP_E_UNSUPPORTED, "canvas layers are square 3x3 / stride-1 / pad-1 convolutions that follow each other");
+    if (p.activation != FHIP_ACT_NONE && p.activation != FHIP_ACT_RELU) return fail(FHIP_E_UNSUPPORTED, "activation other than none / ReLU");
+    const bool has_bias = p.bias_term != 0, relu = p.activation == FHIP_ACT_RELU;
+    if (has_bias && !bias) return fail(FHIP_E_BADARG, "bias_term set but bias is NULL");
+    const int H = p.output_h, IH = next.input_h, nc = batch / 4;
+    if (IH < 2 || (IH & 1)) return fail(FHIP_E_UNSUPPORTED, "canvas images have an even side");
+    CanvasChain g;
+    g.K = p.output_channels;
+    g.NC = nc;
+    g.IH = IH;
+    g.QP = IH + 2;
+    bool ok;
+    switch (form)
+    {
+        case FHIP_CANVAS_ENTRY:
+            ok = H == 2 * IH && (2 * IH + 2) % 6 == 0 && plan_is(pp, H, batch) && plan_is(pn, 2 * IH + 2, nc);
+            g.Tq = pp.tiles_per_image;
+            g.T = 4 * g.Tq;
+            g.T2q = g.T2 = pn.tiles_per_image;
+            break;
+        case FHIP_CANVAS_INSIDE:
+            ok = H == IH && (2 * IH + 2) % 6 == 0 && plan_is(pp, 2 * IH + 2, nc) && plan_is(pn, 2 * IH + 2, nc);
+            g.Tq = g.T = pp.tiles_per_image;
+            g.T2q = g.T2 = pn.tiles_per_image;
+            break;
+        case FHIP_CANVAS_EXIT:
+            ok = H == 2 * IH && (2 * H + 2) % 6 == 0 && plan_is(pp, 2 * H + 2, nc) && plan_is(pn, IH, batch);
+            g.QP = IH + 1;
+            g.Tq = g.T = pp.tiles_per_image;
+            g.T2q = pn.tiles_per_image;
+            g.T2 = 4 * g.T2q;
+            break;
+        default: return fail(FHIP_E_BADARG, "unknown canvas form");
+    }
+    if (!ok) return fail(FHIP_E_BADARG, "the geometries or plans do not belong to this canvas form (fhip_winograd_f63_plan_canvas)");
+    g.TX = pp.tiles_x;
+    g.TX2 = pn.tiles_x;
+    g.Lm = wino_layout(g.K, pp.columns_padded, pp.column_block);
+    g.Lv2 = wino_layout(g.K, pn.columns_padded, pn.column_block);
+    const long long planes = (long long)nc * g.K;
+    if (planes > 0x7fffffffLL) return fail(FHIP_E_BADARG, "N*K too large");
+    g.planes = (int)planes;
+    g.LDH = 6 * pn.tiles_y + 2;
+    g.LDW = 6 * pn.tiles_x + 4;
+    g.sub = g.LDH * g.LDW;
+    g.pf = form == FHIP_CANVAS_EXIT ? 4 * g.sub : g.sub;
+    const size_t plane_bytes = (size_t)g.pf * sizeof(float);
+    if (plane_bytes > 64 * 1024) return fail(FHIP_E_UNSUPPORTED, "the canvas does not fit a block's LDS");
+    const int work = std::max(g.T, g.T2);
+    int ppb = std::max(1, 256 / work);
+    ppb = (int)std::min<size_t>(ppb, std::max<size_t>(1, (48 * 1024) / plane_bytes));
+    g.ppb = (int)std::min<long long>(ppb, planes);
+    const bool multi = work > 512;
+    if (multi && form != FHIP_CANVAS_ENTRY) return fail(FHIP_E_UNSUPPORTED, "a canvas of more than 512 tiles");
+    const unsigned threads = std::max(256u, (unsigned)((multi ? g.T2 : work) + 63) / 64 * 64);
+    if (threads > 512u) return fail(FHIP_E_UNSUPPORTED, "the consumer's canvas has more than 512 tiles");
+    const size_t lds = plane_bytes * g.ppb;
+    const long long units = (planes + g.ppb - 1) / g.ppb;
+    int cus;
+    size_t dev_lds;
+    if (const int rc = device_limits(&cus, &dev_lds)) return rc;
+    const int bpc = std::max(1, std::min((int)(dev_lds / lds), 12 / (int)(threads / 64)));
+    const unsigned grid = ((unsigned)std::min<long long>(units, (long long)cus * bpc) + 7u) & ~7u;
+#define FHIP_CANVAS_LAUNCH(F_, M_)                                                                                                             \
+    do                                                                                                                                         \
+    {                                                                                                                                          \
+        if (has_bias && relu) hipLaunchKernelGGL((canvas_chain_kernel<true, true, F_, M_>), dim3(grid), dim3(threads), lds, s, vn, m, bias, g, (int)units); \
+        else if (has_bias) hipLaunchKernelGGL((canvas_chain_kernel<true, false, F_, M_>), dim3(grid), dim3(threads), lds, s, vn, m, bias, g, (int)units);   \
+        else if (relu) hipLaunchKernelGGL((canvas_chain_kernel<false, true, F_, M_>), dim3(grid), dim3(threads), lds, s, vn, m, bias, g, (int)units);       \
+        else hipLaunchKernelGGL((canvas_chain_kernel<false, false, F_, M_>), dim3(grid), dim3(threads), lds, s, vn, m, bias, g, (int)units);                \
+    } while (0)
+    if (form == FHIP_CANVAS_ENTRY && multi) FHIP_CANVAS_LAUNCH(FHIP_CANVAS_ENTRY, true);
+    else if (form == FHIP_CANVAS_ENTRY) FHIP_CANVAS_LAUNCH(FHIP_CANVAS_ENTRY, false);
+    else if (form == FHIP_CANVAS_INSIDE) FHIP_CANVAS_LAUNCH(FHIP_CANVAS_INSIDE, false);
+    else FHIP_CANVAS_LAUNCH(FHIP_CANVAS_EXIT, false);
+#undef FHIP_CANVAS_LAUNCH
+    FHIP_CANVAS_CHECK_HIP(hipGetLastError());
+    return FHIP_OK;
+}
+
+static int canvas_output(const fhip_conv_param& p, int batch, const fhip_winograd_plan& pl, float* out, const float* m, const float* bias, int pool,
+                         hipStream_t s)
+{
+    if (batch < 4 || (batch & 3)) return fail(FHIP_E_UNSUPPORTED, "canvases hold four images: the batch must be a multiple of 4");
+    if (!k3s1p1(p)) return fail(FHIP_E_UNSUPPORTED, "canvas layers are square 3x3 / stride-1 / pad-1 convolutions");
+    if (p.activation != FHIP_ACT_NONE && p.activation != FHIP_ACT_RELU) return fail(FHIP_E_UNSUPPORTED, "activation other than none / ReLU");
+    const bool has_bias = p.bias_term != 0, relu = p.activation == FHIP_ACT_RELU;
+    if (has_bias && !bias) return fail(FHIP_E_BADARG, "bias_term set but bias is NULL");
+    const int H = p.output_h, nc = batch / 4;
+    if (H < 2 || (H & 1) || (2 * H + 2) % 6 != 0 || !plan_is(pl, 2 * H + 2, nc))
+        return fail(FHIP_E_BADARG, "the geometry or plan is not a canvas layer's (fhip_winograd_f63_plan_canvas)");
+    if (p.output_channels > 65535) return fail(FHIP_E_UNSUPPORTED, "more than 65535 output channels");
+    CanvasOut g;
+    g.K = p.output_channels;
+    g.T = pl.tiles_per_image;
+    g.TX = pl.tiles_x;
+    g.P = pl.columns;
+    g.IH = pool ? H / 2 : H;
+    g.QP = pool ? H / 2 + 1 : H + 2;
+    g.Lm = wino_layout(g.K, pl.columns_padded, pl.column_block);
+    const dim3 grid((unsigned)((g.P + 255) / 256), (unsigned)g.K);
+#define FHIP_CANVAS_OUT(P_)                                                                                                     \
+    do                                                                                                                          \
+    {                                                                                                                           \
+        if (has_bias && relu) hipLaunchKernelGGL((canvas_output_kernel<true, true, P_>), grid, dim3(256), 0, s, out, m, bias, g); \
+        else if (has_bias) hipLaunchKernelGGL((canvas_output_kernel<true, false, P_>), grid, dim3(256), 0, s, out, m, bias, g);   \
+        else if (relu) hipLaunchKernelGGL((canvas_output_kernel<false, true, P_>), grid, dim3(256), 0, s, out, m, bias, g);       \
+        else hipLaunchKernelGGL((canvas_output_kernel<false, false, P_>), grid, dim3(256), 0, s, out, m, bias, g);                \
+    } while (0)
+    if (pool) FHIP_CANVAS_OUT(true);
+    else FHIP_CANVAS_OUT(false);
+#undef FHIP_CANVAS_OUT
+    FHIP_CANVAS_CHECK_HIP(hipGetLastError());
+    return FHIP_OK;
+}
+
+}
+
+extern "C"
+{
+
+int fhip_canvas_output_to_next_input(int form, const fhip_conv_param* param, const fhip_conv_param* next, int batch, const fhip_winograd_plan* plan,
+                                     const fhip_winograd_plan* plan_next, float* v_next, const float* m, const float* bias, void* stream)
+{
+    if (!param || !next || !plan || !plan_next || !v_next || !m) return fhip::fail(FHIP_E_BADARG, "bad argument");
+    return fhip::canvas_chain(form, *param, *next, batch, *plan, *plan_next, v_next, m, bias, (hipStream_t)stream);
+}
+
+int fhip_canvas_output_transform(const fhip_conv_param* param, int batch, const fhip_winograd_plan* plan, float* output, const float* m,
+                                 const float* bias, int pool, void* stream)
+{
+    if (!param || !plan || !output || !m) return fhip::fail(FHIP_E_BADARG, "bad argument");
+    return fhip::canvas_output(*param, batch, *plan, output, m, bias, pool, (hipStream_t)stream);
+}
+
+const char* fhip_canvas_last_error(void) { return fhip::g_error.c_str(); }
+
+}
diff --git a/feathercnn_amd/net.py b/feathercnn_amd/net.py
--- a/feathercnn_amd/net.py
+++ b/feathercnn_amd/net.py
@@ -224,6 +224,14 @@
                     out[i] = (a.value == 1, b.value == 1)
         return out
 
+    def canvases(self):
+        out = []
+        for i in range(self._lib.fhip_net_layer_count(self._h)):
+            c = ctypes.c_int()
+            if self._lib.fhip_net_layer_canvas(self._h, i, ctypes.byref(c)) == 0 and c.value:
+                out.append(i)
+        return out
+
     def forward_timed(self):
         n = self._lib.fhip_net_layer_count(self._h)
         ms = (ctypes.c_float * max(n, 1))()
diff --git a/include/feather_hip/feather_canvas.h b/include/feather_hip/feather_canvas.h
--- /dev/null
+++ b/include/feather_hip/feather_canvas.h
@@ -0,0 +1,35 @@
+#ifndef FEATHER_HIP_FEATHER_CANVAS_H_
+#define FEATHER_HIP_FEATHER_CANVAS_H_
+
+#include <stddef.h>
+
+#include "feather_hip/feather_hip.h"
+
+#ifdef __cplusplus
+extern "C"
+{
+#endif
+
+#define FHIP_CANVAS_API __attribute__((visibility("default")))
+
+enum fhip_canvas_form
+{
+    FHIP_CANVAS_ENTRY = 1,
+    FHIP_CANVAS_INSIDE = 2,
+    FHIP_CANVAS_EXIT = 3
+};
+
+FHIP_CANVAS_API int fhip_canvas_output_to_next_input(int form, const fhip_conv_param* param, const fhip_conv_param* next, int batch,
+                                                     const fhip_winograd_plan* plan, const fhip_winograd_plan* plan_next, float* v_next,
+                                                     const float* m, const float* bias, void* stream);
+
+FHIP_CANVAS_API int fhip_canvas_output_transform(const fhip_conv_param* param, int batch, const fhip_winograd_plan* plan, float* output,
+                                                 const float* m, const float* bias, int pool, void* stream);
+
+FHIP_CANVAS_API const char* fhip_canvas_last_error(void);
+
+#ifdef __cplusplus
+}
+#endif
+
+#endif
diff --git a/include/feather_hip/feather_hip.h b/include/feather_hip/feather_hip.h
--- a/include/feather_hip/feather_hip.h
+++ b/include/feather_hip/feather_hip.h
@@ -90,6 +90,8 @@
 } fhip_winograd_plan;
 
 FHIP_API int fhip_winograd_f63_plan(const fhip_conv_param* param, int batch, fhip_winograd_plan* plan);
+FHIP_API int fhip_winograd_f63_plan_canvas(const fhip_conv_param* param, int batch, int canvas, fhip_winograd_plan* plan);
+FHIP_API int fhip_winograd_f63_canvas_param(const fhip_conv_param* param, int batch, fhip_conv_param* canvas);
 
 FHIP_API int fhip_winograd_f63_transform_kernel(const fhip_conv_param* param, float* u, const float* kernel,
                                                 void* stream);
diff --git a/include/feather_hip/feather_net.h b/include/feather_hip/feather_net.h
--- a/include/feather_hip/feather_net.h
+++ b/include/feather_hip/feather_net.h
@@ -135,6 +135,7 @@
 FHIP_API int fhip_net_layer_conv_param(fhip_net* net, int index, fhip_conv_param* param, int* batch);
 FHIP_API int fhip_net_layer_fused_pointwise(fhip_net* net, int index, fhip_conv_param* param, int* one_kernel);
 FHIP_API int fhip_net_layer_chain(fhip_net* net, int index, int* v_from_previous, int* writes_next_v);
+FHIP_API int fhip_net_layer_canvas(fhip_net* net, int index, int* canvas);
 FHIP_API int fhip_net_layer_sibling(fhip_net* net, int index, int* state);
 FHIP_API int fhip_net_layer_residual(fhip_net* net, int index, int* state);
 FHIP_API int fhip_net_forward_timed(fhip_net* net, float* ms);
```

Result: faster. 10060 images/s (median of 6 runs) (+2.2%).
